# AechPro/rlgym-ppo

Hardware: AMD Instinct MI355X
Metric: ppo_update_samples_per_sec (higher is better)
Workload: dtype f32; 1 GPU; configs[1]: 4096 agents x 128 steps = 524,288-sample buffer, obs 107 f32, 90 discrete actions, 256x3 policy + critic; batch 524,288, minibatch 65,536

## Files before the change

### rlgym_ppo_amd/csrc/api.hip

```cpp
#include "build_id.h"
#include <math.h>
#include <stdarg.h>
#include <string.h>

#include "common.hpp"

namespace rlppo {

static thread_local char g_err[512] = "";

void set_error(const char *fmt, ...) {
    va_list ap;
    va_start(ap, fmt);
    vsnprintf(g_err, sizeof(g_err), fmt, ap);
    va_end(ap);
}

static int64_t padded_width(int64_t d) {
    const int64_t p16 = round_up(d, 16), p64 = round_up(d, 64);
    return (p64 - p16) * 10 >= p64 ? p16 : p64;
}
static int64_t padded_out(int64_t d) {
    if (d <= 32) return 32;
    if (d <= 64) return 64;
    if (d <= 96) return 96;
    return round_up(d, 128);
}

int make_layout(const int32_t *dims, int32_t n_layers, NetLayout *out) {
    RLPPO_CHECK_ARG(dims != nullptr && n_layers >= 1 && n_layers <= RLPPO_MAX_LAYERS, "network: n_layers=%d not in [1,%d]",
                    n_layers, RLPPO_MAX_LAYERS);
    for (int i = 0; i <= n_layers; ++i) RLPPO_CHECK_ARG(dims[i] >= 1, "network: dims[%d]=%d", i, dims[i]);
    out->n_layers = n_layers;
    int64_t off = 0, flat = 0;
    int pin = (int)padded_width(dims[0]);
    for (int l = 0; l < n_layers; ++l) {
        LayerLayout &L = out->L[l];
        L.in = dims[l];
        L.out = dims[l + 1];
        L.pin = pin;
        L.pout = (int)padded_out(dims[l + 1]);
        L.off_w = off;
        off += (int64_t)L.pout * L.pin;
        L.off_wt = off;
        off += (int64_t)L.pin * L.pout;
        L.off_b = off;
        off += L.pout;
        L.off_flat_w = flat;
        flat += (int64_t)L.out * L.in;
        L.off_flat_b = flat;
        flat += L.out;
        pin = L.pout;
    }
    out->packed_floats = off;
    out->flat_floats = flat;
    return 0;
}

static int max_pout(const NetLayout &net) {
    int m = 0;
    for (int l = 0; l < net.n_layers; ++l) m = net.L[l].pout > m ? net.L[l].pout : m;
    return m;
}

struct X3Layout {
    int64_t fwd[RLPPO_MAX_LAYERS], dx[RLPPO_MAX_LAYERS], total;
};
static void x3_layout(const NetLayout &net, X3Layout *o) {
    int64_t off = 0;
    const int last = net.n_layers - 1;
    for (int l = 0; l < net.n_layers; ++l) {
        const LayerLayout &L = net.L[l];
        o->fwd[l] = o->dx[l] = -1;
        if (l >= 1 && l < last && nt_split_ok(L.pout, L.pin)) {
            o->fwd[l] = off;
            off += (int64_t)3 * L.pout * L.pin;
        }
        if (l >= 1 && !(l == last && gemv_head_ok(L.out, L.pin)) && nt_split_ok(L.pin, L.pout)) {
            o->dx[l] = off;
            off += (int64_t)3 * L.pin * L.pout;
        }
    }
    o->total = off;
}

static int g_fold_vhead = 1;

struct RowSource {
    const float *x;
    int64_t ld;
    const unsigned *rowtab = nullptr;
    int64_t src_rows = 0;
};

static int forward(hipStream_t st, const NetLayout &net, const float *packed, const RowSource &in, int64_t n, int out_tanh,
                   float *const *acts, int bf16_operands = 0, unsigned long long *const *bits = nullptr, bool *have_bits = nullptr,
                   bool *head_folded = nullptr, const unsigned short *x3 = nullptr, bool head_prezeroed = false) {
    X3Layout xl;
    if (x3) x3_layout(net, &xl);
    if (have_bits)
        for (int l = 0; l < net.n_layers; ++l) have_bits[l] = false;
    const float *x = in.x;
    int64_t ldx = in.ld;
    const int hl = net.n_layers - 1;
    bool fold = head_folded && g_fold_vhead && hl >= 1 && !out_tanh && !bf16_operands && bits && bits[hl - 1] &&
                gemv_head_ok(net.L[hl].out, net.L[hl].pin) && net.L[hl - 1].pout / 128 <= 2;
    if (x3 && hl >= 1 && xl.fwd[hl - 1] >= 0) fold = false;
    if (head_folded) *head_folded = false;
    for (int l = 0; l < net.n_layers; ++l) {
        const LayerLayout &L = net.L[l];
        const bool last = l == net.n_layers - 1;
        const int epi = last ? (out_tanh ? EPI_BIAS_TANH : EPI_BIAS) : EPI_BIAS_RELU;
        int rc;
        if (last && head_folded && *head_folded) break;
        if (last && !out_tanh && gemv_head_ok(L.out, L.pin))
            rc = launch_gemv_fwd(st, x, ldx, packed + L.off_w, packed + L.off_b, acts[l], L.pout, n, L.pin, L.pout);
        else {
            rc = -1;
            if (!last && bits && bits[l] && x3 && xl.fwd[l] >= 0) {
                rc = launch_gemm_nt_split(st, x, ldx, x3 + xl.fwd[l], packed + L.off_b, acts[l], L.pout, n, L.pout, L.pin, 0, bits[l]);
                if (rc == 0) have_bits[l] = true;
            } else if (!last && bits && bits[l] && !bf16_operands) {
                NtDot dots[2];
                const bool fold_here = fold && l == hl - 1;
                if (fold_here) {
                    if (!head_prezeroed) RLPPO_HIP(hipMemsetAsync(acts[hl], 0, (size_t)n * sizeof(float), st));
                    dots[0].w = packed + net.L[hl].off_w;
                    dots[0].b = packed + net.L[hl].off_b;
                    dots[0].out = acts[hl];
                }
                rc = launch_gemm_nt_bits(st, x, ldx, packed + L.off_w, L.pin, packed + L.off_b, acts[l], L.pout, n, L.pout, L.pin,
                                         EPI_BIAS_RELU, bits[l], l == 0 ? in.rowtab : nullptr, in.src_rows, nullptr, fold_here ? dots : nullptr);
                if (rc == 0) have_bits[l] = true;
                if (fold_here) *head_folded = rc == 0;
            }
            if (l == 0 && in.rowtab && rc != 0) {
                if (rc == -1) set_error("forward: the gathered first layer needs the bitmask form");
                return rc == -1 ? RLPPO_ERR_ARG : rc;
            }
            if (rc == -1)
                rc = launch_gemm_nt(st, x, ldx, packed + L.off_w, L.pin, packed + L.off_b, nullptr, 0, acts[l], L.pout, n, L.pout,
                                    L.pin, epi, bf16_operands);
        }
        if (rc) return rc;
        x = acts[l];
        ldx = L.pout;
    }
    return 0;
}

static bool b16_next_wants_f32(const NetLayout &net, int l) {
    const int nx = l + 1, last = net.n_layers - 1;
    const LayerLayout &N = net.L[nx];
    if (nx == last) {
        const bool fwd_b16 = gemv_head_ok(N.out, N.pin) || nt_b16_ok(N.pout, N.pin, false);
        return !(fwd_b16 && thin_head_ok(N.out, N.pin));
    }
    return !(nt_b16_ok(N.pout, N.pin, true) && tn_b16_ok(N.pout, N.pin));
}
static int forward_b16(hipStream_t st, const NetLayout &net, const float *packed_r, const unsigned short *wb16, const float *x,
                       const unsigned short *xb, int64_t ldx, int64_t n, int out_tanh, float *const *acts,
                       unsigned short *const *actsb, unsigned long long *const *bits, bool *have_bits, bool *f32_valid) {
    for (int l = 0; l < net.n_layers; ++l) have_bits[l] = f32_valid[l] = false;
    int64_t off16 = 0;
    bool x_f32 = true;
    for (int l = 0; l < net.n_layers; ++l) {
        const LayerLayout &L = net.L[l];
        const bool last = l == net.n_layers - 1;
        int rc = 0;
        auto need_x_f32 = [&]() -> int {
            if (x_f32) return 0;
            x_f32 = f32_valid[l - 1] = true;
            return launch_expand_rows(st, actsb[l - 1], acts[l - 1], n * (int64_t)net.L[l - 1].pout);
        };
        if (last) {
            const int epi = out_tanh ? EPI_BIAS_TANH : EPI_BIAS;
            if (!out_tanh && gemv_head_ok(L.out, L.pin))
                rc = launch_gemv_fwd_b16(st, xb, ldx, packed_r + L.off_w, packed_r + L.off_b, acts[l], L.pout, n, L.pin, L.pout);
            else if (nt_b16_ok(L.pout, L.pin, false))
                rc = launch_gemm_nt_b16(st, xb, ldx, wb16 + off16, L.pin, packed_r + L.off_b, acts[l], L.pout, nullptr, 0, n, L.pout,
                                        L.pin, epi, 0, nullptr);
            else {
                rc = need_x_f32();
                if (rc == 0)
                    rc = launch_gemm_nt(st, x, ldx, packed_r + L.off_w, L.pin, packed_r + L.off_b, nullptr, 0, acts[l], L.pout, n,
                                        L.pout, L.pin, epi);
            }
            f32_valid[l] = true;
        } else if (nt_b16_ok(L.pout, L.pin, true) && bits[l]) {
            const bool want = b16_next_wants_f32(net, l);
            rc = launch_gemm_nt_b16(st, xb, ldx, wb16 + off16, L.pin, packed_r + L.off_b, want ? acts[l] : nullptr, L.pout, actsb[l],
                                    L.pout, n, L.pout, L.pin, EPI_BIAS_RELU, 1, bits[l]);
            have_bits[l] = rc == 0;
            f32_valid[l] = want;
        } else {
            rc = need_x_f32();
            if (rc) return rc;
            rc = -1;
            if (bits[l]) {
                rc = launch_gemm_nt_bits(st, x, ldx, packed_r + L.off_w, L.pin, packed_r + L.off_b, acts[l], L.pout, n, L.pout, L.pin,
                                         EPI_BIAS_RELU, bits[l]);
                have_bits[l] = rc == 0;
            }
            if (rc == -1)
                rc = launch_gemm_nt(st, x, ldx, packed_r + L.off_w, L.pin, packed_r + L.off_b, nullptr, 0, acts[l], L.pout, n, L.pout,
                                    L.pin, EPI_BIAS_RELU);
            if (rc == 0) rc = launch_round_rows(st, acts[l], actsb[l], n * (int64_t)L.pout);
            f32_valid[l] = true;
        }
        if (rc) return rc;
        off16 += (int64_t)L.pout * L.pin;
        x = acts[l];
        xb = actsb[l];
        x_f32 = f32_valid[l];
        ldx = L.pout;
    }
    return 0;
}

static size_t forward_ws_floats(const NetLayout &net, int64_t n) { return (size_t)2 * (size_t)n * (size_t)max_pout(net); }

static int forward_pingpong(hipStream_t st, const NetLayout &net, const float *packed, const float *obs, int64_t ld_obs,
                            int64_t n, int out_tanh, void *ws, size_t ws_bytes, float *final_out, const float **out,
                            int64_t *ld_out, int bf16_operands) {
    if (ws_bytes < forward_ws_floats(net, n) * sizeof(float)) {
        set_error("forward: workspace %zu < %zu bytes", ws_bytes, forward_ws_floats(net, n) * sizeof(float));
        return RLPPO_ERR_WORKSPACE;
    }
    RLPPO_CHECK_ARG(ld_obs >= net.L[0].pin && ld_obs % 4 == 0, "forward: ld_obs=%ld must be >= %d (zero padded rows)",
                    (long)ld_obs, net.L[0].pin);
    float *b0 = reinterpret_cast<float *>(ws);
    float *b1 = b0 + (size_t)n * max_pout(net);
    float *acts[RLPPO_MAX_LAYERS];
    for (int l = 0; l < net.n_layers; ++l) acts[l] = (l & 1) ? b1 : b0;
    if (final_out) acts[net.n_layers - 1] = final_out;
    int rc = forward(st, net, packed, RowSource{obs, ld_obs}, n, out_tanh, acts, bf16_operands);
    if (rc) return rc;
    *out = acts[net.n_layers - 1];
    *ld_out = net.L[net.n_layers - 1].pout;
    return 0;
}

}

using namespace rlppo;

static int g_fused_act = 1;
static std::atomic<long long> g_cnt_fused_act{0}, g_cnt_act_chain{0}, g_cnt_paired_pass{0}, g_cnt_gather_fused_pass{0}, g_cnt_pass{0}, g_cnt_group_dw{0}, g_cnt_md_nvec{0};
constexpr int64_t FUSED_ACT_MAX_ROWS = 8192;

struct ActCtx {
    int bf16 = 0;
    unsigned *done = nullptr;
    unsigned done_value = 0;
    unsigned *noise_ctl = nullptr;
    const unsigned *mask = nullptr;
    int mask_words = 0;
};
static int act_ctx(const rlppo_act_opts *o, ActCtx *c, bool late_noise = false, const char *mask_for = nullptr) {
    c->bf16 = get_infer_bf16();
    if (!o) return 0;
    RLPPO_CHECK_ARG(o->precision == RLPPO_PRECISION_DEFAULT || o->precision == RLPPO_PRECISION_FP32 || o->precision == RLPPO_PRECISION_BF16,
                    "act options: inference precision %d (0 = process default, 1 = fp32, 2 = bf16 operands)", o->precision);
    if (o->precision != RLPPO_PRECISION_DEFAULT) c->bf16 = o->precision == RLPPO_PRECISION_BF16;
    c->done = o->done_words;
    c->done_value = o->done_value;
    c->noise_ctl = o->noise_ctl;
    c->mask = o->action_mask;
    c->mask_words = o->mask_words;
    RLPPO_CHECK_ARG(!o->action_mask || !mask_for, "act options: action_mask is an option of the discrete head, not of %s", mask_for ? mask_for : "");
    RLPPO_CHECK_ARG(!o->noise_ctl || late_noise, "act options: noise_ctl is an option of rlppo_discrete_step");
    RLPPO_CHECK_ARG(!o->noise_ctl || (o->done_words && !(o->done_value & 0x80000000u)),
                    "act options: noise_ctl needs done_words (a kernel that gives up on the noise reports it there) and done_value < 2^31");
    return 0;
}
static int act_mask_check(const ActCtx &c, int n_actions) {
    RLPPO_CHECK_ARG(!c.mask || c.mask_words == (n_actions + 31) / 32, "act options: mask_words=%d, but n_actions=%d needs %d words per row",
                    c.mask_words, n_actions, (n_actions + 31) / 32);
    return 0;
}
static int act_done(hipStream_t st, const ActCtx &c, int64_t n) {
    return c.done ? launch_signal_words(st, c.done, (int)rlppo_act_done_words(n), c.done_value) : 0;
}

extern "C" {

int rlppo_abi_version(void) { return RLPPO_ABI_VERSION; }
const char *rlppo_build_id(void) { return RLPPO_BUILD_ID; }
const char *rlppo_last_error(void) { return g_err; }

int64_t rlppo_padded_width(int64_t d) { return padded_width(d); }
int64_t rlppo_padded_out(int64_t d) { return padded_out(d); }

int64_t rlppo_packed_floats(const int32_t *dims, int32_t n_layers) {
    NetLayout net;
    if (make_layout(dims, n_layers, &net)) return -1;
    return net.packed_floats;
}
int64_t rlppo_flat_floats(const int32_t *dims, int32_t n_layers) {
    NetLayout net;
    if (make_layout(dims, n_layers, &net)) return -1;
    return net.flat_floats;
}

int rlppo_net_pack(void *stream, const int32_t *dims, int32_t n_layers, const float *flat, float *packed) {
    NetLayout net;
    int rc = make_layout(dims, n_layers, &net);
    if (rc) return rc;
    RLPPO_CHECK_ARG(flat && packed, "net_pack: null pointer");
    return launch_pack((hipStream_t)stream, net, flat, packed);
}

int rlppo_pad_rows(void *stream, const void *src, int32_t src_is_f64, int64_t n, int64_t d, int64_t ld_src, float *dst,
                   int64_t ld_dst, int32_t standardize, float mean0, float std0) {
    RLPPO_CHECK_ARG(n >= 0 && d >= 1 && ld_src >= d && ld_dst >= d, "pad_rows: n=%ld d=%ld ld_src=%ld ld_dst=%ld", (long)n,
                    (long)d, (long)ld_src, (long)ld_dst);
    RLPPO_CHECK_ARG(n == 0 || (src && dst), "pad_rows: null pointer");
    return launch_pad_rows((hipStream_t)stream, src, src_is_f64, n, d, ld_src, dst, ld_dst, standardize, mean0, std0);
}

int rlppo_pad_rows_per_feature(void *stream, const void *src, int32_t src_is_f64, int64_t n, int64_t d, int64_t ld_src,
                               float *dst, int64_t ld_dst, const float *mean, const float *stdv) {
    RLPPO_CHECK_ARG(n >= 0 && d >= 1 && ld_src >= d && ld_dst >= d, "pad_rows_per_feature: n=%ld d=%ld ld_src=%ld ld_dst=%ld",
                    (long)n, (long)d, (long)ld_src, (long)ld_dst);
    RLPPO_CHECK_ARG(n == 0 || (src && dst && mean && stdv), "pad_rows_per_feature: null pointer");
    return launch_pad_rows_vec((hipStream_t)stream, src, src_is_f64, n, d, ld_src, dst, ld_dst, mean, stdv);
}

size_t rlppo_forward_workspace_bytes(const int32_t *dims, int32_t n_layers, int64_t n) {
    NetLayout net;
    if (make_layout(dims, n_layers, &net)) return 0;
    return forward_ws_floats(net, n > 0 ? n : 0) * sizeof(float) + 256;
}

int rlppo_mlp_forward(void *stream, const int32_t *dims, int32_t n_layers, const float *packed, const float *obs,
                      int64_t ld_obs, int64_t n, int32_t out_tanh, float *out, int64_t ld_out, void *workspace,
                      size_t ws_bytes, const rlppo_act_opts *opts) {
    NetLayout net;
    int rc = make_layout(dims, n_layers, &net);
    if (rc) return rc;
    ActCtx cx;
    rc = act_ctx(opts, &cx, false, "rlppo_mlp_forward");
    if (rc) return rc;
    if (n == 0) return 0;
    RLPPO_CHECK_ARG(n > 0 && packed && obs && out && workspace, "mlp_forward: bad argument");
    RLPPO_CHECK_ARG(ld_out == net.L[n_layers - 1].pout, "mlp_forward: ld_out=%ld must equal the padded output width %d",
                    (long)ld_out, net.L[n_layers - 1].pout);
    const float *o;
    int64_t ldo;
    rc = forward_pingpong((hipStream_t)stream, net, packed, obs, ld_obs, n, out_tanh, workspace, ws_bytes, out, &o, &ldo, cx.bf16);
    return rc ? rc : act_done((hipStream_t)stream, cx, n);
}

int rlppo_discrete_act(void *stream, const int32_t *dims, int32_t n_layers, const float *packed, const float *obs,
                       int64_t ld_obs, int64_t n, const float *noise_q, int64_t *actions, float *logp, float *probs_out,
                       void *workspace, size_t ws_bytes, const rlppo_act_opts *opts) {
    NetLayout net;
    int rc = make_layout(dims, n_layers, &net);
    if (rc) return rc;
    ActCtx cx;
    rc = act_ctx(opts, &cx);
    if (rc) return rc;
    if (n == 0) return 0;
    RLPPO_CHECK_ARG(n > 0 && packed && obs && noise_q && actions && logp && workspace, "discrete_act: bad argument");
    rc = act_mask_check(cx, dims[n_layers]);
    if (rc) return rc;
    if (g_fused_act && !cx.bf16 && fused_act_ok(net) && n <= FUSED_ACT_MAX_ROWS && ld_obs >= net.L[0].pin && ld_obs % 4 == 0 &&
        (reinterpret_cast<uintptr_t>(obs) & 15) == 0) {
        FusedActIO io;
        io.rows = obs;
        io.ld_rows = ld_obs;
        io.noise = noise_q;
        io.actions = actions;
        io.logp = logp;
        io.probs_out = probs_out;
        io.done_words = cx.done;
        io.done_value = cx.done_value;
        io.mask = cx.mask;
        io.mask_words = cx.mask_words;
        ++g_cnt_fused_act;
        return launch_discrete_act_fused((hipStream_t)stream, net, packed, io, n);
    }
    ++g_cnt_act_chain;
    const float *o;
    int64_t ldo;
    rc = forward_pingpong((hipStream_t)stream, net, packed, obs, ld_obs, n, 0, workspace, ws_bytes, nullptr, &o, &ldo, cx.bf16);
    if (rc) return rc;
    rc = launch_discrete_sample_logits((hipStream_t)stream, o, ldo, n, dims[n_layers], noise_q, actions, logp, probs_out, cx.mask, cx.mask_words);
    return rc ? rc : act_done((hipStream_t)stream, cx, n);
}

size_t rlppo_discrete_step_workspace_bytes(const int32_t *dims, int32_t n_layers, int64_t n) {
    NetLayout net;
    if (make_layout(dims, n_layers, &net)) return 0;
    n = n > 0 ? n : 0;
    return forward_ws_floats(net, n) * sizeof(float) + ((size_t)n * net.L[0].pin * sizeof(float) + 255) / 256 * 256 + 512;
}

static int g_window_mode = 0;
int rlppo_host_window_alloc(size_t bytes, void **ptr) {
    RLPPO_CHECK_ARG(ptr && bytes > 0, "host_window_alloc: bad argument");
// ... 384 lines not shown
                    float *const *dx, float *grad, float *tn_ws, unsigned long long *const *bits, const bool *have_bits,
                    bool head_folded = false, const unsigned short *x3 = nullptr, DwList *defer = nullptr) {
    const int last = net.n_layers - 1;
    int rc = 0;
    X3Layout xl;
    if (x3) x3_layout(net, &xl);
    for (int l = last; l >= 0; --l) {
        const LayerLayout &L = net.L[l];
        const float *dY = l == last ? acts[last] : dx[l];
        const int64_t ld_hy = head_folded ? 1 : L.pout;
        const RowSource X = l > 0 ? RowSource{acts[l - 1], net.L[l - 1].pout} : in;
        const bool gemv = l == last && l > 0 && gemv_head_ok(L.out, L.pin);
        const size_t floats = tn_layer_floats(net, l, mb, 0);
        if (gemv)
            rc = launch_gemv_dw(st, dY, ld_hy, X.x, X.ld, grad + L.off_flat_w, grad + L.off_flat_b, L.in, L.pin, mb, tn_ws, floats);
        else if (defer)
            defer->add(L, dY, X, grad);
        else
            rc = launch_gemm_tn(st, dY, L.pout, L.pout, X.x, X.ld, L.pin, grad + L.off_flat_w, grad + L.off_flat_b, L.out, L.in, mb,
                                tn_ws, floats, X.rowtab, X.src_rows);
        if (rc) return rc;
        if (l == 0) break;
        rc = -1;
        if (gemv) {
            if (have_bits[l - 1]) rc = launch_gemv_dx_bits(st, dY, ld_hy, packed + L.off_w, bits[l - 1], dx[l - 1], L.pin, L.pin, mb);
            if (rc == -1) rc = launch_gemv_dx(st, dY, ld_hy, packed + L.off_w, acts[l - 1], L.pin, dx[l - 1], L.pin, L.pin, mb);
        } else {
            if (have_bits[l - 1] && x3 && xl.dx[l] >= 0)
                rc = launch_gemm_nt_split(st, dY, L.pout, x3 + xl.dx[l], nullptr, dx[l - 1], L.pin, mb, L.pin, L.pout, 1, bits[l - 1]);
            else if (have_bits[l - 1])
                rc = launch_gemm_nt_bits(st, dY, L.pout, packed + L.off_wt, L.pout, nullptr, dx[l - 1], L.pin, mb, L.pin, L.pout,
                                         EPI_MASK, bits[l - 1]);
            if (rc == -1)
                rc = launch_gemm_nt(st, dY, L.pout, packed + L.off_wt, L.pout, nullptr, acts[l - 1], L.pin, dx[l - 1], L.pin, mb,
                                    L.pin, L.pout, EPI_MASK);
        }
        if (rc) return rc;
    }
    return rc;
}

static int backward_b16(hipStream_t st, const NetLayout &net, const float *packed_r, const unsigned short *wb16, const float *states,
                        const unsigned short *states_b, int64_t ld_states, int64_t mb, float *const *acts,
                        unsigned short *const *actsb, float *const *dx, unsigned short *const *dxb, float *grad, float *tn_ws,
                        size_t tn_floats, unsigned long long *const *bits, const bool *have_bits, bool *f32_valid) {
    const int last = net.n_layers - 1;
    int64_t first[RLPPO_MAX_LAYERS], total = 0;
    for (int l = 0; l < net.n_layers; ++l) {
        first[l] = total;
        total += (int64_t)net.L[l].pout * net.L[l].pin;
    }
    bool dx_f32[RLPPO_MAX_LAYERS] = {};
    int rc = 0;
    auto act_f32 = [&](int l) -> int {
        if (l < 0 || f32_valid[l]) return 0;
        f32_valid[l] = true;
        return launch_expand_rows(st, actsb[l], acts[l], mb * (int64_t)net.L[l].pout);
    };
    auto grad_f32 = [&](int l) -> int {
        if (dx_f32[l]) return 0;
        dx_f32[l] = true;
        return launch_expand_rows(st, dxb[l], dx[l], mb * (int64_t)net.L[l].pout);
    };
    for (int l = last; l >= 0; --l) {
        const LayerLayout &L = net.L[l];
        const float *X = l > 0 ? acts[l - 1] : states;
        const unsigned short *Xb = l > 0 ? actsb[l - 1] : states_b;
        const int64_t ldx = l > 0 ? net.L[l - 1].pout : ld_states;
        const bool gemv = l == last && l > 0 && gemv_head_ok(L.out, L.pin);
        if (l == last) {
            rc = l > 0 ? launch_thin_dw_b16(st, acts[last], L.pout, Xb, ldx, grad + L.off_flat_w, grad + L.off_flat_b, L.out, L.in,
                                            L.pin, mb, tn_ws, tn_floats)
                       : -1;
            if (rc == -1) {
                rc = act_f32(l - 1);
                if (rc) return rc;
                if (gemv)
                    rc = launch_gemv_dw(st, acts[last], L.pout, X, ldx, grad + L.off_flat_w, grad + L.off_flat_b, L.in, L.pin, mb,
                                        tn_ws, tn_floats);
                else
                    rc = launch_gemm_tn(st, acts[last], L.pout, L.pout, X, ldx, L.pin, grad + L.off_flat_w, grad + L.off_flat_b,
                                        L.out, L.in, mb, tn_ws, tn_floats);
            }
        } else if (tn_b16_ok(L.pout, L.pin) && ldx % 8 == 0) {
            rc = launch_gemm_tn_b16(st, dxb[l], L.pout, Xb, ldx, grad + L.off_flat_w, grad + L.off_flat_b, L.pout, L.pin, L.out, L.in,
                                    mb, tn_ws, tn_floats);
        } else {
            rc = grad_f32(l);
            if (rc == 0) rc = act_f32(l - 1);
            if (rc) return rc;
            rc = launch_gemm_tn(st, dx[l], L.pout, L.pout, X, ldx, L.pin, grad + L.off_flat_w, grad + L.off_flat_b, L.out, L.in, mb,
                                tn_ws, tn_floats);
        }
        if (rc) return rc;
        if (l == 0) break;
        if (l < last && have_bits[l - 1] && nt_b16_ok(L.pin, L.pout, true)) {
            rc = launch_gemm_nt_b16(st, dxb[l], L.pout, wb16 + total + first[l], L.pout, nullptr, nullptr, 0, dxb[l - 1], L.pin, mb,
                                    L.pin, L.pout, EPI_MASK, 2, bits[l - 1]);
            if (rc) return rc;
            continue;
        }
        if (l == last && have_bits[l - 1]) {
            rc = launch_thin_dx_b16(st, acts[last], L.pout, L.out, packed_r + L.off_w, L.pin, bits[l - 1], dxb[l - 1], L.pin, L.pin, mb);
            if (rc == 0) continue;
            if (rc != -1) return rc;
        }
        const float *dY = acts[last];
        if (l < last) {
            rc = grad_f32(l);
            if (rc) return rc;
            dY = dx[l];
        }
        rc = -1;
        if (gemv) {
            if (have_bits[l - 1]) rc = launch_gemv_dx_bits(st, dY, L.pout, packed_r + L.off_w, bits[l - 1], dx[l - 1], L.pin, L.pin, mb);
            if (rc == -1) {
                rc = act_f32(l - 1);
                if (rc) return rc;
                rc = launch_gemv_dx(st, dY, L.pout, packed_r + L.off_w, acts[l - 1], L.pin, dx[l - 1], L.pin, L.pin, mb);
            }
        } else {
            if (have_bits[l - 1])
                rc = launch_gemm_nt_bits(st, dY, L.pout, packed_r + L.off_wt, L.pout, nullptr, dx[l - 1], L.pin, mb, L.pin, L.pout,
                                         EPI_MASK, bits[l - 1]);
            if (rc == -1) {
                rc = act_f32(l - 1);
                if (rc) return rc;
                rc = launch_gemm_nt(st, dY, L.pout, packed_r + L.off_wt, L.pout, nullptr, acts[l - 1], L.pin, dx[l - 1], L.pin, mb,
                                    L.pin, L.pout, EPI_MASK);
            }
        }
        if (rc) return rc;
        rc = launch_round_rows(st, dx[l - 1], dxb[l - 1], mb * (int64_t)L.pin);
        if (rc) return rc;
        dx_f32[l - 1] = true;
    }
    return rc;
}

static int g_head_order = 1;
static int g_paired = 1;
constexpr int64_t PAIRED_MIN_ROWS = 262144;
static bool twin_ok(const NetLayout &p, const NetLayout &v, int64_t mb) {
    if (p.n_layers != v.n_layers || p.n_layers < 2) return false;
    for (int l = 0; l + 1 < p.n_layers; ++l) {
        const LayerLayout &a = p.L[l], &b = v.L[l];
        if (a.in != b.in || a.out != b.out || a.pin != b.pin || a.pout != b.pout) return false;
        if (a.pout % 128 != 0 || a.pin % 16 != 0 || nt_bits_floats(mb, a.pout) == 0) return false;
    }
    return true;
}

static int head_forward(hipStream_t st, const NetLayout &net, const float *packed, const float *x, int64_t ldx, int64_t n, int out_tanh,
                        float *out) {
    const LayerLayout &L = net.L[net.n_layers - 1];
    if (!out_tanh && gemv_head_ok(L.out, L.pin)) return launch_gemv_fwd(st, x, ldx, packed + L.off_w, packed + L.off_b, out, L.pout, n, L.pin, L.pout);
    return launch_gemm_nt(st, x, ldx, packed + L.off_w, L.pin, packed + L.off_b, nullptr, 0, out, L.pout, n, L.pout, L.pin,
                          out_tanh ? EPI_BIAS_TANH : EPI_BIAS);
}
static int head_backward(hipStream_t st, const NetLayout &net, const float *packed, const float *dY, const float *X, int64_t mb,
                         float *dx_prev, float *grad, float *tn_ws, const unsigned long long *bits_prev, int64_t ld_dy = 0,
                         DwList *defer = nullptr) {
    const int last = net.n_layers - 1;
    const LayerLayout &L = net.L[last];
    const int64_t ldx = net.L[last - 1].pout;
    const bool gemv = gemv_head_ok(L.out, L.pin);
    const size_t floats = tn_layer_floats(net, last, mb, 0);
    if (!ld_dy) ld_dy = L.pout;
    int rc = 0;
    if (gemv) rc = launch_gemv_dw(st, dY, ld_dy, X, ldx, grad + L.off_flat_w, grad + L.off_flat_b, L.in, L.pin, mb, tn_ws, floats);
    else if (defer) defer->add(L, dY, RowSource{X, ldx}, grad);
    else rc = launch_gemm_tn(st, dY, L.pout, L.pout, X, ldx, L.pin, grad + L.off_flat_w, grad + L.off_flat_b, L.out, L.in, mb, tn_ws, floats);
    if (rc) return rc;
    if (gemv) return launch_gemv_dx_bits(st, dY, ld_dy, packed + L.off_w, bits_prev, dx_prev, L.pin, L.pin, mb);
    rc = launch_gemm_nt_bits(st, dY, L.pout, packed + L.off_wt, L.pout, nullptr, dx_prev, L.pin, mb, L.pin, L.pout, EPI_MASK,
                             const_cast<unsigned long long *>(bits_prev));
    if (rc == -1) {
        set_error("paired pass: the output layer's dX needs the bitmask form");
        return RLPPO_ERR_ARG;
    }
    return rc;
}

constexpr int64_t FUSED_GATHER_MIN_ROWS = 262144;
static RowSource first_layer_rows(const rlppo_minibatch_args &a, const NetLayout &pol, const NetLayout &val, int prec, const WsPlan &w) {
    const int64_t src_rows = a.ring_cap > 0 ? a.ring_cap : a.n_rows;
    auto gather_form = [&](const NetLayout &n) {
        return n.n_layers > 1 && nt_gather_ok(a.ld_states, src_rows, n.L[0].pout, n.L[0].pin) && tn_gather_ok(a.ld_states, src_rows) &&
               !(n.L[0].out > 64 && n.L[0].out <= 96 && !(n.L[0].in > 96 && n.L[0].in <= 112));
    };
    if (prec != 1 && (g_fused_gather == 2 || (g_fused_gather == 1 && a.mb >= FUSED_GATHER_MIN_ROWS)) && src_rows > 0 &&
        gather_form(pol) && gather_form(val))
        return RowSource{a.states, a.ld_states, w.rowtab, src_rows};
    return RowSource{w.states, pol.L[0].pin};
}

struct Pass {
    const rlppo_minibatch_args *a;
    NetLayout pol, val;
    int64_t mb;
    int prec;
    int64_t ring_base, ring_cap;
    WsPlan w;
    RowSource rows;
    LossCfg cfg;
    MdSpec md;
    bool md_general = false;
    const float *pol_w, *val_w;
    hipStream_t st, side;
    DwList *defer;
};

static LossCfg loss_cfg(const rlppo_minibatch_args &a) {
    LossCfg c;
    c.clip = a.clip_range;
    c.clip_lo = (float)(1.0 - (double)a.clip_range);
    c.clip_hi = (float)(1.0 + (double)a.clip_range);
    c.ent_coef = a.ent_coef;
    c.mb_ratio = a.mb_ratio;
    c.inv_mb = 1.0f / (float)a.mb;
    c.var_m = a.var_m;
    c.var_b = a.var_b;
    c.adv_norm = a.adv_norm;
    c.vclip = a.value_clip;
    c.kl_slots = a.kl_slots;
    c.stop_word = a.stop_word;
    return c;
}

static int policy_loss(hipStream_t st, const Pass &p) {
    const rlppo_minibatch_args &a = *p.a;
    const int last = p.pol.n_layers - 1;
    const LayerLayout &L = p.pol.L[last];
    const WsPlan &w = p.w;
    if (a.head == RLPPO_HEAD_DISCRETE) {
        MaskRows mr;
        mr.mask = a.action_mask;
        mr.W = a.mask_words;
        mr.idx = a.idx;
        mr.ring_base = p.ring_base;
        mr.ring_cap = p.ring_cap;
        return launch_discrete_loss(st, w.pol.act[last], L.pout, L.out, w.g_act, w.g_old, w.g_adv, p.mb, p.cfg, a.stats, a.action_mask ? &mr : nullptr);
    }
    if (a.head == RLPPO_HEAD_GAUSSIAN)
        return launch_gaussian_loss(st, w.pol.act[last], L.pout, L.out / 2, w.g_act, w.g_old, w.g_adv, p.mb, p.cfg, a.stats);
    if (p.md_general) {
        ++g_cnt_md_nvec;
        return launch_multidiscrete_nvec_loss(st, w.pol.act[last], L.pout, w.g_act, w.g_old, w.g_adv, p.mb, p.cfg, a.stats, p.md);
    }
    return launch_multidiscrete_loss(st, w.pol.act[last], L.pout, w.g_act, w.g_old, w.g_adv, p.mb, p.cfg, a.stats);
}

static int gather(const Pass &p) {
    const rlppo_minibatch_args &a = *p.a;
    const WsPlan &w = p.w;
    const int width = p.pol.L[0].pin;
    float *const vout = w.val.act[p.val.n_layers - 1];
    if (p.prec == 1) {
        auto lean0 = [](const NetLayout &n) {
            return n.n_layers > 1 && nt_b16_ok(n.L[0].pout, n.L[0].pin, true) && tn_b16_ok(n.L[0].pout, n.L[0].pin);
        };
        const int rc = launch_gather_rows_round(p.st, a.states, a.ld_states, a.idx, lean0(p.pol) && lean0(p.val) ? nullptr : w.states,
                                                w.states_b, width, p.mb, p.ring_base, p.ring_cap);
        if (rc) return rc;
    } else if (!p.rows.rowtab) {
        GatherMeta gm;
        gm.actions = a.actions; gm.old_logp = a.old_logp; gm.adv = a.advantages; gm.targets = a.targets;
        gm.g_old = w.g_old; gm.g_adv = w.g_adv; gm.g_tgt = w.g_tgt; gm.g_act = w.g_act;
        gm.zero_n = vout;
        gm.act_dim = a.act_dim;
        return launch_gather_rows(p.st, a.states, a.ld_states, a.idx, w.states, width, p.mb, p.ring_base, p.ring_cap, &gm);
    }
    return launch_gather_meta(p.st, a.idx, a.actions, a.act_dim, a.old_logp, a.advantages, a.targets, w.g_act, w.g_old, w.g_adv, w.g_tgt,
                              p.mb, p.ring_base, p.ring_cap, p.rows.rowtab ? w.rowtab : nullptr, vout);
}

static int paired_pass(const Pass &p, SlotBank &bk, int slot) {
    const rlppo_minibatch_args &a = *p.a;
    const NetLayout &pol = p.pol, &val = p.val;
    const WsPlan &w = p.w;
    const int64_t mb = p.mb;
    const hipStream_t st = p.st, hs = p.side;
    const int H = pol.n_layers - 1;
    int rc;
    const LayerLayout &Lvh = val.L[H];
    const bool fold_v = g_fold_vhead && gemv_head_ok(Lvh.out, Lvh.pin) && val.L[H - 1].pout / 128 <= 2;
    float *vout = w.val.act[H], *pout = w.pol.act[H];
    const int64_t ldv = fold_v ? 1 : Lvh.pout;
    const float *xp = p.rows.x, *xv = xp;
    int64_t ldx = p.rows.ld;
    for (int l = 0; l < H; ++l) {
        const LayerLayout &Lp = pol.L[l], &Lv = val.L[l];
        NtAlt alt;
        alt.A = xv;
        alt.B = p.val_w + Lv.off_w;
        alt.bias = p.val_w + Lv.off_b;
        alt.C = w.val.act[l];
        alt.bits = w.val.bits[l];
        NtDot dots[2];
        const bool fold_here = fold_v && l == H - 1;
        if (fold_here) {
            dots[1].w = p.val_w + Lvh.off_w;
            dots[1].out = vout;
            dots[1].b = p.val_w + Lvh.off_b;
        }
        rc = launch_gemm_nt_bits(st, xp, ldx, p.pol_w + Lp.off_w, Lp.pin, p.pol_w + Lp.off_b, w.pol.act[l], Lp.pout, mb, Lp.pout, Lp.pin,
                                 EPI_BIAS_RELU, w.pol.bits[l], l == 0 ? p.rows.rowtab : nullptr, p.rows.src_rows, &alt,
                                 fold_here ? dots : nullptr);
        if (rc) {
            if (rc == -1) set_error("paired pass: a hidden layer does not have the bitmask form");
            return rc == -1 ? RLPPO_ERR_ARG : rc;
        }
        xp = w.pol.act[l];
        xv = w.val.act[l];
        ldx = Lp.pout;
    }
    if (hs != st) {
        rc = order_after(hs, st, bk.ev_fork[slot]);
        if (rc) return rc;
    }
    if (!fold_v) {
        rc = head_forward(hs, val, p.val_w, xv, ldx, mb, 0, vout);
        if (rc) return rc;
    }
    rc = launch_value_loss(hs, vout, ldv, w.g_tgt, w.g_adv, mb, p.cfg, a.stats);
    if (rc) return rc;
    const bool ordered = g_head_order && hs != st;
    if (!ordered) {
        rc = head_backward(hs, val, p.val_w, vout, xv, mb, w.val.dx[H - 1], a.val_grad, w.val.tn, w.val.bits[H - 1], ldv, p.defer);
        if (rc) return rc;
    }
    rc = head_forward(st, pol, p.pol_w, xp, ldx, mb, a.head == RLPPO_HEAD_GAUSSIAN, pout);
    if (rc) return rc;
    rc = policy_loss(st, p);
    if (rc) return rc;
    if (ordered) {
        rc = order_after(hs, st, bk.ev_mid[slot]);
        if (rc) return rc;
        rc = head_backward(hs, val, p.val_w, vout, xv, mb, w.val.dx[H - 1], a.val_grad, w.val.tn, w.val.bits[H - 1], ldv, p.defer);
        if (rc) return rc;
    }
    rc = head_backward(st, pol, p.pol_w, pout, xp, mb, w.pol.dx[H - 1], a.pol_grad, w.pol.tn, w.pol.bits[H - 1], 0, p.defer);
    if (rc) return rc;
    if (hs != st) {
        rc = order_after(st, hs, bk.ev_join[slot]);
        if (rc) return rc;
    }
    for (int l = H - 1; l >= 0; --l) {
        const LayerLayout &Lp = pol.L[l], &Lv = val.L[l];
        const RowSource Xp = l > 0 ? RowSource{w.pol.act[l - 1], pol.L[l - 1].pout} : p.rows;
        const RowSource Xv = l > 0 ? RowSource{w.val.act[l - 1], val.L[l - 1].pout} : p.rows;
        if (p.defer) {
            p.defer->add(Lp, w.pol.dx[l], Xp, a.pol_grad);
            p.defer->add(Lv, w.val.dx[l], Xv, a.val_grad);
        } else {
            TnPair pr;
            pr.dY = w.val.dx[l];
            pr.X = Xv.x;
            pr.dW = a.val_grad + Lv.off_flat_w;
            pr.db = a.val_grad + Lv.off_flat_b;
            pr.ws = w.val.tn;
            rc = launch_gemm_tn(st, w.pol.dx[l], Lp.pout, Lp.pout, Xp.x, Xp.ld, Lp.pin, a.pol_grad + Lp.off_flat_w, a.pol_grad + Lp.off_flat_b,
                                Lp.out, Lp.in, mb, w.pol.tn, tn_layer_floats(pol, l, mb, 0), Xp.rowtab, Xp.src_rows, &pr);
            if (rc) return rc;
        }
        if (l == 0) break;
        NtAlt alt;
        alt.A = w.val.dx[l];
        alt.B = p.val_w + Lv.off_wt;
        alt.C = w.val.dx[l - 1];
        alt.bits = w.val.bits[l - 1];
        rc = launch_gemm_nt_bits(st, w.pol.dx[l], Lp.pout, p.pol_w + Lp.off_wt, Lp.pout, nullptr, w.pol.dx[l - 1], Lp.pin, mb, Lp.pin,
                                 Lp.pout, EPI_MASK, w.pol.bits[l - 1], nullptr, 0, &alt);
        if (rc) return rc == -1 ? RLPPO_ERR_ARG : rc;
    }
    return 0;
}

static int two_chain_pass(const Pass &p) {
    const rlppo_minibatch_args &a = *p.a;
    const NetLayout &pol = p.pol, &val = p.val;
    const WsPlan &w = p.w;
    const int64_t mb = p.mb;
    const bool b16 = p.prec == 1;
    const unsigned short *pol_wb16 = reinterpret_cast<const unsigned short *>(a.pol_wb16);
    const unsigned short *val_wb16 = reinterpret_cast<const unsigned short *>(a.val_wb16);
    const unsigned short *pol_x3 = p.prec == 2 ? pol_wb16 : nullptr, *val_x3 = p.prec == 2 ? val_wb16 : nullptr;
    bool phave[RLPPO_MAX_LAYERS] = {}, vhave[RLPPO_MAX_LAYERS] = {};
    bool pf32[RLPPO_MAX_LAYERS] = {}, vf32[RLPPO_MAX_LAYERS] = {};
    bool v_folded = false;
    int rc;
    if (b16) {
        rc = forward_b16(p.side, val, p.val_w, val_wb16, p.rows.x, w.states_b, p.rows.ld, mb, 0, w.val.act, w.val.actb, w.val.bits, vhave,
                         vf32);
        if (rc) return rc;
        rc = forward_b16(p.st, pol, p.pol_w, pol_wb16, p.rows.x, w.states_b, p.rows.ld, mb, a.head == RLPPO_HEAD_GAUSSIAN, w.pol.act,
                         w.pol.actb, w.pol.bits, phave, pf32);
    } else {
        rc = forward(p.side, val, p.val_w, p.rows, mb, 0, w.val.act, 0, w.val.bits, vhave, &v_folded, val_x3, true);
        if (rc) return rc;
        rc = forward(p.st, pol, p.pol_w, p.rows, mb, a.head == RLPPO_HEAD_GAUSSIAN, w.pol.act, 0, w.pol.bits, phave, nullptr, pol_x3);
    }
    if (rc) return rc;
    const int64_t ldv = v_folded ? 1 : val.L[val.n_layers - 1].pout;
    rc = launch_value_loss(p.side, w.val.act[val.n_layers - 1], ldv, w.g_tgt, w.g_adv, mb, p.cfg, a.stats);
    if (rc) return rc;
    rc = policy_loss(p.st, p);
    if (rc) return rc;
    if (b16) {
        rc = backward_b16(p.side, val, p.val_w, val_wb16, p.rows.x, w.states_b, p.rows.ld, mb, w.val.act, w.val.actb, w.val.dx, w.val.dxb,
                          a.val_grad, w.val.tn, tn_ws_floats(val, mb, p.prec), w.val.bits, vhave, vf32);
        if (rc) return rc;
        return backward_b16(p.st, pol, p.pol_w, pol_wb16, p.rows.x, w.states_b, p.rows.ld, mb, w.pol.act, w.pol.actb, w.pol.dx, w.pol.dxb,
                            a.pol_grad, w.pol.tn, tn_ws_floats(pol, mb, p.prec), w.pol.bits, phave, pf32);
    }
    rc = backward(p.side, val, p.val_w, p.rows, mb, w.val.act, w.val.dx, a.val_grad, w.val.tn, w.val.bits, vhave, v_folded, val_x3, p.defer);
    if (rc) return rc;
    return backward(p.st, pol, p.pol_w, p.rows, mb, w.pol.act, w.pol.dx, a.pol_grad, w.pol.tn, w.pol.bits, phave, false, pol_x3, p.defer);
}

static int ppo_minibatch(void *stream, const rlppo_minibatch_args *a, const int32_t *md_nvec, int32_t md_heads) {
    RLPPO_CHECK_ARG(a != nullptr, "ppo_minibatch: null args");
    Pass p;
    p.a = a;
    int rc = make_layout(a->pol_dims, a->pol_layers, &p.pol);
    if (rc) return rc;
    rc = make_layout(a->val_dims, a->val_layers, &p.val);
    if (rc) return rc;
    const NetLayout &pol = p.pol, &val = p.val;
    const int64_t mb = p.mb = a->mb;
    if (mb == 0) return 0;
    rc = resolve_precision(a->precision, &p.prec);
    if (rc) return rc;
    RLPPO_CHECK_ARG(mb > 0 && a->pol_packed && a->val_packed && a->pol_grad && a->val_grad && a->states && a->actions &&
                        a->old_logp && a->targets && a->advantages && a->idx && a->stats && a->workspace,
                    "ppo_minibatch: null pointer");
    RLPPO_CHECK_ARG(val.L[val.n_layers - 1].out == 1, "ppo_minibatch: critic must have one output");
    RLPPO_CHECK_ARG(a->value_clip >= 0.f && a->value_clip < INFINITY, "ppo_minibatch: value_clip=%g", (double)a->value_clip);
    RLPPO_CHECK_ARG(pol.L[0].in == val.L[0].in, "ppo_minibatch: policy and critic observe different sizes");
    RLPPO_CHECK_ARG(a->ld_states >= pol.L[0].pin && a->ld_states % 4 == 0, "ppo_minibatch: ld_states=%ld < %d",
                    (long)a->ld_states, pol.L[0].pin);
    const size_t ws_bytes = plan_workspace(pol, val, mb, p.prec, a->workspace, &p.w) * sizeof(float);
    if (a->ws_bytes < ws_bytes) {
        set_error("ppo_minibatch: workspace %zu < %zu bytes", a->ws_bytes, ws_bytes);
        return RLPPO_ERR_WORKSPACE;
    }
    const int n_out = pol.L[pol.n_layers - 1].out;
    RLPPO_CHECK_ARG(a->head == RLPPO_HEAD_DISCRETE || a->head == RLPPO_HEAD_GAUSSIAN || a->head == RLPPO_HEAD_MULTIDISCRETE,
                    "ppo_minibatch: unknown head %d", a->head);
    RLPPO_CHECK_ARG(!a->action_mask || a->head == RLPPO_HEAD_DISCRETE, "ppo_minibatch: action_mask is an option of the discrete head, not of the %s head",
                    a->head == RLPPO_HEAD_GAUSSIAN ? "Gaussian" : "multi-discrete");
    RLPPO_CHECK_ARG(!a->action_mask || a->mask_words == (n_out + 31) / 32, "ppo_minibatch: mask_words=%d, but n_actions=%d needs %d words per row",
                    a->mask_words, n_out, (n_out + 31) / 32);
    if (a->head == RLPPO_HEAD_DISCRETE) {
        RLPPO_CHECK_ARG(a->act_dim == 1, "discrete head: act_dim must be 1");
        RLPPO_CHECK_ARG(pol.L[pol.n_layers - 1].pout <= DISCRETE_LOSS_MAX_LD, "discrete head: padded width %ld too large",
                        (long)pol.L[pol.n_layers - 1].pout);
    }
    if (a->head == RLPPO_HEAD_GAUSSIAN)
        RLPPO_CHECK_ARG(n_out % 2 == 0 && a->act_dim == n_out / 2, "gaussian head: act_dim=%d, outputs=%d", a->act_dim, n_out);
    RLPPO_CHECK_ARG(!md_nvec || a->head == RLPPO_HEAD_MULTIDISCRETE, "ppo_minibatch: md_nvec is an option of the multi-discrete head, not of the %s head",
                    a->head == RLPPO_HEAD_GAUSSIAN ? "Gaussian" : "discrete");
    if (a->head == RLPPO_HEAD_MULTIDISCRETE && md_nvec) {
        rc = md_spec_make(md_nvec, md_heads, "multi-discrete head: md_nvec / md_heads", &p.md);
        if (rc) return rc;
        p.md_general = true;
        RLPPO_CHECK_ARG(p.md.S == n_out, "multi-discrete head: md_nvec sums to %d, but the policy has %d outputs", p.md.S, n_out);
        RLPPO_CHECK_ARG(a->act_dim == p.md.H, "multi-discrete head: act_dim=%d, but md_heads=%d", a->act_dim, p.md.H);
    } else if (a->head == RLPPO_HEAD_MULTIDISCRETE)
        RLPPO_CHECK_ARG(n_out == 21 && a->act_dim == 8, "multi-discrete head: needs 21 outputs and act_dim 8");
    RLPPO_CHECK_ARG(p.prec != 1 || (a->pol_packed_r && a->val_packed_r && a->pol_wb16 && a->val_wb16),
                    "ppo_minibatch: the bf16 update precision needs the rlppo_net_pack_bf16 images of both networks (pol_packed_r / val_packed_r / pol_wb16 / val_wb16)");
    RLPPO_CHECK_ARG(p.prec != 2 || (a->pol_wb16 && a->val_wb16),
                    "ppo_minibatch: the split-bf16 update precision needs the rlppo_net_pack_x3 images of both networks (pol_wb16 / val_wb16)");
    p.ring_cap = a->ring_cap > 0 ? a->ring_cap : INT64_MAX;
    p.ring_base = a->ring_cap > 0 ? a->ring_base : 0;
    RLPPO_CHECK_ARG(p.ring_base >= 0 && p.ring_base < p.ring_cap, "ppo_minibatch: ring_base=%ld not in [0, ring_cap=%ld)",
                    (long)a->ring_base, (long)a->ring_cap);
    const int slot = a->slot;
    RLPPO_CHECK_ARG(slot >= 0 && slot < RLPPO_MAX_SLOTS, "ppo_minibatch: slot %d not in [0, %d)", slot, RLPPO_MAX_SLOTS);

    p.rows = first_layer_rows(*a, pol, val, p.prec, p.w);
    const bool twin = p.prec == 0 && (g_paired == 2 || (g_paired == 1 && mb >= PAIRED_MIN_ROWS)) && twin_ok(pol, val, mb);
    p.cfg = loss_cfg(*a);
    p.pol_w = p.prec == 1 ? a->pol_packed_r : a->pol_packed;
    p.val_w = p.prec == 1 ? a->val_packed_r : a->val_packed;
    DwList dws;
    p.defer = (g_group_dw && p.prec != 1) ? &dws : nullptr;

    SlotBank *bank = nullptr;
    rc = slot_bank(&bank);
    if (rc) return rc;
    SlotBank &bk = *bank;
    rc = ensure_slot(bk, slot);
    if (rc) return rc;
    const hipStream_t caller = (hipStream_t)stream;
    p.st = caller;
    if (slot > 0) {
        p.st = bk.main[slot];
        rc = order_after(p.st, caller, bk.ev_slot[slot]);
        if (rc) return rc;
        bk.pending[slot] = true;
    }
    rc = gather(p);
    if (rc) return rc;
    p.side = p.st;
    if (g_two_streams) {
        p.side = bk.side[slot];
        rc = order_after(p.side, p.st, bk.ev_fork[slot]);
        if (rc) return rc;
    }
    ++g_cnt_pass;
    if (twin) ++g_cnt_paired_pass;
    if (p.rows.rowtab) ++g_cnt_gather_fused_pass;
    rc = twin ? paired_pass(p, bk, slot) : two_chain_pass(p);
    if (rc) return rc;
    if (!twin && p.side != p.st) {
        rc = order_after(p.st, p.side, bk.ev_join[slot]);
        if (rc) return rc;
    }
    if (p.defer && dws.n) {
        ++g_cnt_group_dw;
        rc = launch_gemm_tn_group(p.st, dws.p, dws.n, mb, p.w.pol.tn, p.w.tn_floats);
    }
    return rc;
}

int rlppo_ppo_minibatch(void *stream, const rlppo_minibatch_args *a) { return ppo_minibatch(stream, a, nullptr, 0); }
int rlppo_ppo_minibatch_nvec(void *stream, const rlppo_minibatch_args *a, const int32_t *md_nvec, int32_t md_heads) {
    return ppo_minibatch(stream, a, md_nvec, md_heads);
}

int rlppo_ppo_join(void *stream) {
    SlotBank *bank = nullptr;
    int rc = slot_bank(&bank);
    if (rc) return rc;
    SlotBank &bk = *bank;
    for (int s = 1; s < RLPPO_MAX_SLOTS; ++s)
        if (bk.pending[s]) {
            rc = order_after((hipStream_t)stream, bk.main[s], bk.ev_slot[s]);
            if (rc) return rc;
            bk.pending[s] = false;
        }
    return 0;
}

int rlppo_clip_adam(void *stream, float *params, float *grads, float *exp_avg, float *exp_avg_sq, int64_t n,
                    double max_norm, double lr, double beta1, double beta2, double eps, int64_t step, double *gnorm2) {
    if (n == 0) return 0;
    RLPPO_CHECK_ARG(n > 0 && params && grads && exp_avg && exp_avg_sq && gnorm2 && step >= 1, "clip_adam: bad argument");
    const double bc1 = 1.0 - pow(beta1, (double)step);
    const double bc2 = 1.0 - pow(beta2, (double)step);
    const float step_size = (float)(lr / bc1);
    const float bc2_sqrt = (float)sqrt(bc2);
    return launch_clip_adam((hipStream_t)stream, params, grads, exp_avg, exp_avg_sq, n, (float)max_norm, step_size, bc2_sqrt,
                            (float)(1.0 - beta1), (float)beta2, (float)(1.0 - beta2), (float)eps, gnorm2);
}

int rlppo_clip_adam_pack2(void *stream, const rlppo_opt_net *a, const rlppo_opt_net *b, void *sync_ws) {
    RLPPO_CHECK_ARG(a && b, "clip_adam_pack2: null descriptor");
// ... 9 lines not shown
        int rc = make_layout(d[k]->dims, d[k]->n_layers, &nets[k]);
        if (rc) return rc;
        RLPPO_CHECK_ARG(d[k]->params && d[k]->grads && d[k]->exp_avg && d[k]->exp_avg_sq && d[k]->packed && d[k]->gnorm2 &&
                            d[k]->step >= 1, "clip_adam_pack2: bad argument (net %d)", k);
        const double bc1 = 1.0 - pow(d[k]->beta1, (double)d[k]->step);
        const double bc2 = 1.0 - pow(d[k]->beta2, (double)d[k]->step);
        p[k] = d[k]->params; g[k] = d[k]->grads; m[k] = d[k]->exp_avg; v[k] = d[k]->exp_avg_sq; packed[k] = d[k]->packed;
        gn[k] = d[k]->gnorm2;
        const LayerLayout &last = nets[k].L[nets[k].n_layers - 1];
        n[k] = last.off_flat_b + last.out;
        max_norm[k] = (float)d[k]->max_norm; step_size[k] = (float)(d[k]->lr / bc1); bc2_sqrt[k] = (float)sqrt(bc2);
        omb1[k] = (float)(1.0 - d[k]->beta1); beta2[k] = (float)d[k]->beta2; omb2[k] = (float)(1.0 - d[k]->beta2);
        eps[k] = (float)d[k]->eps;
    }
    return launch_clip_adam_pack2((hipStream_t)stream, nets, p, g, m, v, packed, gn, n, max_norm, step_size, bc2_sqrt, omb1, beta2,
                                  omb2, eps, sync_ws, skip);
}

int64_t rlppo_kl_slots_doubles(int64_t mb) { return kl_slots_doubles(mb); }

int rlppo_adv_stats(void *stream, const int64_t *idx, int64_t n, const float *advantages, int64_t ring_base, int64_t ring_cap,
                    float *out, void *ws) {
    RLPPO_CHECK_ARG(n >= 1 && idx && advantages && out && ws, "adv_stats: bad argument");
    const int64_t cap = ring_cap > 0 ? ring_cap : INT64_MAX, base = ring_cap > 0 ? ring_base : 0;
    RLPPO_CHECK_ARG(base >= 0 && base < cap, "adv_stats: ring_base=%ld not in [0, ring_cap=%ld)", (long)ring_base, (long)ring_cap);
    return launch_adv_stats((hipStream_t)stream, idx, n, advantages, base, cap, out, ws);
}

int rlppo_kl_gate(void *stream, const rlppo_kl_gate_args *a) {
    RLPPO_CHECK_ARG(a && a->kl_slots && a->n_passes >= 0 && a->slot_stride >= 3 && a->phase >= 0 && a->phase <= 2 && a->stop_word,
                    "kl_gate: bad argument");
    RLPPO_CHECK_ARG(a->phase == 0 || a->exchange, "kl_gate: phases 1 and 2 need the exchange words");
    RLPPO_CHECK_ARG(a->phase == 1 || a->host_words, "kl_gate: host_words missing");
    return launch_kl_gate((hipStream_t)stream, *a);
}

int rlppo_learn_report(void *stream, const rlppo_report_args *a) {
    RLPPO_CHECK_ARG(a != nullptr, "learn_report: null args");
    RLPPO_CHECK_ARG(a->n_pol >= 0 && a->n_val >= 0 && (a->n_pol == 0 || (a->pol_before && a->pol_now)) && (a->n_val == 0 || (a->val_before && a->val_now)),
                    "learn_report: parameter vectors missing");
    RLPPO_CHECK_ARG(a->stats && a->out && a->done_word && a->ws, "learn_report: null pointer (stats / out / done_word / ws)");
    RLPPO_CHECK_ARG((reinterpret_cast<uintptr_t>(a->ws) & 15) == 0, "learn_report: ws must be 16-byte aligned");
    return launch_learn_report((hipStream_t)stream, *a);
}

}

extern "C" {
int rlppo_gather_rows(void *stream, const float *src, int64_t ld_src, const int64_t *idx, float *dst, int32_t width, int64_t n) {
    if (n == 0) return 0;
    RLPPO_CHECK_ARG(n > 0 && src && idx && dst, "gather_rows: null pointer");
    return launch_gather_rows((hipStream_t)stream, src, ld_src, idx, dst, width, n);
}
int rlppo_welford_increment(void *stream, const float *samples, int64_t ld, int64_t n, int32_t d, void *mean, void *m2,
                            int64_t count, int32_t state_is_f64) {
    if (n == 0) return 0;
    RLPPO_CHECK_ARG(n > 0 && d > 0 && ld >= d && count >= 0 && samples && mean && m2, "welford_increment: bad argument");
    return launch_welford((hipStream_t)stream, samples, ld, n, d, mean, m2, (long long)count, state_is_f64 != 0);
}
int rlppo_welford_merge(void *stream, int32_t d, void *mean, void *m2, int64_t count, const float *other_mean,
                        const float *other_m2, int64_t other_count, int32_t state_is_f64) {
    if (other_count == 0) return 0;
    RLPPO_CHECK_ARG(d > 0 && count >= 0 && other_count > 0 && mean && m2 && other_mean && other_m2, "welford_merge: bad argument");
    return launch_welford_merge((hipStream_t)stream, d, mean, m2, (long long)count, other_mean, other_m2, (long long)other_count,
                                state_is_f64 != 0);
}
int64_t rlppo_wb16_elems(const int32_t *dims, int32_t n_layers) {
    NetLayout net;
    if (make_layout(dims, n_layers, &net)) return -1;
    int64_t n = 0;
    for (int l = 0; l < net.n_layers; ++l) n += (int64_t)net.L[l].pout * net.L[l].pin;
    return 2 * n;
}
int rlppo_net_pack_bf16(void *stream, const int32_t *dims, int32_t n_layers, const float *flat, float *packed_r, void *wb16) {
    NetLayout net;
    int rc = make_layout(dims, n_layers, &net);
    if (rc) return rc;
    RLPPO_CHECK_ARG(flat && packed_r && wb16, "net_pack_bf16: null pointer");
    return launch_pack_bf16((hipStream_t)stream, net, flat, packed_r, reinterpret_cast<unsigned short *>(wb16));
}
int64_t rlppo_x3_elems(const int32_t *dims, int32_t n_layers) {
    NetLayout net;
    if (make_layout(dims, n_layers, &net)) return -1;
    X3Layout xl;
    x3_layout(net, &xl);
    return xl.total;
}
int rlppo_net_pack_x3(void *stream, const int32_t *dims, int32_t n_layers, const float *packed, void *planes) {
    NetLayout net;
    int rc = make_layout(dims, n_layers, &net);
    if (rc) return rc;
    X3Layout xl;
    x3_layout(net, &xl);
    if (xl.total == 0) return 0;
    RLPPO_CHECK_ARG(packed && planes, "net_pack_x3: null pointer");
    unsigned short *pl = reinterpret_cast<unsigned short *>(planes);
    for (int l = 0; l < net.n_layers; ++l) {
        const LayerLayout &L = net.L[l];
        if (xl.fwd[l] >= 0) {
            rc = launch_pack_split((hipStream_t)stream, packed + L.off_w, L.pin, L.pout, L.pin, pl + xl.fwd[l]);
            if (rc) return rc;
        }
        if (xl.dx[l] >= 0) {
            rc = launch_pack_split((hipStream_t)stream, packed + L.off_wt, L.pout, L.pin, L.pout, pl + xl.dx[l]);
            if (rc) return rc;
        }
    }
    return 0;
}
int rlppo_dbg_pack_x3(void *stream, const float *S, int64_t ld, int32_t R, int32_t C, void *planes) {
    return launch_pack_split((hipStream_t)stream, S, ld, R, C, reinterpret_cast<unsigned short *>(planes));
}
int rlppo_dbg_gemm_nt_x3(void *stream, const float *A, int64_t lda, const void *planes, const float *bias, float *C, int64_t ldc, int64_t M,
                         int32_t N, int32_t K, int32_t mode, void *bits) {
    return launch_gemm_nt_split((hipStream_t)stream, A, lda, reinterpret_cast<const unsigned short *>(planes), bias, C, ldc, M, N, K, mode,
                                reinterpret_cast<unsigned long long *>(bits));
}
static int64_t g_selection_epoch = 0;
int rlppo_set_update_precision(int32_t mode) {
    RLPPO_CHECK_ARG(mode >= 0 && mode <= 2, "set_update_precision: mode %d (0 = fp32, 1 = bf16 mixed precision, 2 = split-bf16 products)", mode);
    g_update_bf16 = mode;
    ++g_selection_epoch;
    return 0;
}
int rlppo_get_update_precision(void) { return g_update_bf16; }
int rlppo_set_inference_precision(int32_t mode) {
    RLPPO_CHECK_ARG(mode == 0 || mode == 1, "set_inference_precision: mode %d (0 = fp32, 1 = bf16 operands)", mode);
    set_infer_bf16(mode);
    ++g_selection_epoch;
    return 0;
}
int rlppo_dbg_set(int32_t key, int32_t value) {
    ++g_selection_epoch;
    switch (key) {
        case 1: set_gae_algo(value); return 0;
        case 4: g_two_streams = value; return 0;
        case 21: set_gae_spin_limit(value); return 0;
        case 22: set_gae_oversubscribe(value); return 0;
        case 34: set_fused_spin_limit(value); return 0;
        case 35: set_fused_test_hold(value); return 0;
        case 36: set_split_persistent(value); return 0;
        case 23: set_b16_wide_tiles(value); return 0;
        case 24: set_exp_fast_transform(value); return 0;
        case 26: g_fused_gather = value; return 0;
        case 27: g_fused_act = value; return 0;
        case 29: g_paired = value; return 0;
        case 31: g_head_order = value; return 0;
        case 32: g_fold_vhead = value; return 0;
        case 33: set_pair_interleave(value); return 0;
        case 37: g_group_dw = value; return 0;
        case 38: set_tn_group_budget(value); return 0;
        case 40: set_nt_skinny(value); return 0;
        case 41: g_window_mode = value; return 0;
        default: break;
    }
    set_error("dbg_set: unknown key %d", key);
    return RLPPO_ERR_ARG;
}
int64_t rlppo_selection_epoch(void) { return g_selection_epoch; }
const int64_t *rlppo_selection_epoch_ptr(void) { return &g_selection_epoch; }
int64_t rlppo_dbg_counter(int32_t key) {
    switch (key) {
        case 0: return g_cnt_fused_act;
        case 1: return g_cnt_act_chain;
        case 2: return g_cnt_pass;
        case 3: return g_cnt_paired_pass;
        case 4: return g_cnt_gather_fused_pass;
        case 5: return g_cnt_group_dw;
        case 6: return g_cnt_md_nvec;
        default: return -1;
    }
}
size_t rlppo_dbg_gemm_nt_bits_bytes(int64_t M, int32_t N) { return nt_bits_floats(M, N) * sizeof(float); }
int rlppo_dbg_gemm_nt_bits(void *stream, const float *A, int64_t lda, const float *B, int64_t ldb, const float *bias, float *C,
                           int64_t ldc, int64_t M, int32_t N, int32_t K, int32_t epilogue, void *bits) {
    const int rc = launch_gemm_nt_bits((hipStream_t)stream, A, lda, B, ldb, bias, C, ldc, M, N, K, epilogue,
                                       reinterpret_cast<unsigned long long *>(bits));
    if (rc == -1) {
        set_error("dbg_gemm_nt_bits: the bitmask form does not apply to this call");
        return RLPPO_ERR_ARG;
    }
    return rc;
}
int rlppo_dbg_gemm_nt(void *stream, const float *A, int64_t lda, const float *B, int64_t ldb, const float *bias,
                      const float *mask_src, int64_t ld_mask, float *C, int64_t ldc, int64_t M, int32_t N, int32_t K,
                      int32_t epilogue) {
    return launch_gemm_nt((hipStream_t)stream, A, lda, B, ldb, bias, mask_src, ld_mask, C, ldc, M, N, K, epilogue);
}
int rlppo_dbg_gemm_nt_b16(void *stream, const void *A, int64_t lda, const void *W, int64_t ldw, const float *bias, float *C,
                          int64_t ldc, void *Cb, int64_t ldcb, int64_t M, int32_t N, int32_t K, int32_t epilogue, int32_t hidden,
                          void *bits) {
    return launch_gemm_nt_b16((hipStream_t)stream, reinterpret_cast<const unsigned short *>(A), lda,
                              reinterpret_cast<const unsigned short *>(W), ldw, bias, C, ldc, reinterpret_cast<unsigned short *>(Cb),
                              ldcb, M, N, K, epilogue, hidden, reinterpret_cast<unsigned long long *>(bits));
}
int rlppo_dbg_gemm_tn_b16(void *stream, const void *dY, int64_t ldy, const void *X, int64_t ldx, float *dW, float *db, int32_t pout,
                          int32_t pin, int32_t out, int32_t in, int64_t M, void *ws, size_t ws_bytes) {
    return launch_gemm_tn_b16((hipStream_t)stream, reinterpret_cast<const unsigned short *>(dY), ldy,
                              reinterpret_cast<const unsigned short *>(X), ldx, dW, db, pout, pin, out, in, M, (float *)ws,
                              ws_bytes / sizeof(float));
}
size_t rlppo_dbg_thin_head_workspace_bytes(int32_t out, int32_t kp, int64_t M) { return thin_dw_ws_floats(out, kp, M) * sizeof(float); }
int rlppo_dbg_thin_head_b16(void *stream, const float *dY, int64_t ldy, int32_t out, const float *W, int64_t ldw, const void *bits,
                            const void *hb, int64_t ldh, void *dxb, float *dW, float *db, int32_t in, int32_t kp, int64_t M, void *ws,
                            size_t ws_bytes) {
    int rc = launch_thin_dx_b16((hipStream_t)stream, dY, ldy, out, W, ldw, reinterpret_cast<const unsigned long long *>(bits),
                                reinterpret_cast<unsigned short *>(dxb), kp, kp, M);
    if (rc) return rc == -1 ? RLPPO_ERR_ARG : rc;
    rc = launch_thin_dw_b16((hipStream_t)stream, dY, ldy, reinterpret_cast<const unsigned short *>(hb), ldh, dW, db, out, in, kp, M,
                            (float *)ws, ws_bytes / sizeof(float));
    return rc == -1 ? RLPPO_ERR_ARG : rc;
}
static int tn_products(const rlppo_tn_product *p, int32_t n, TnProduct *q) {
    RLPPO_CHECK_ARG(p && n > 0 && n <= 2 * RLPPO_MAX_LAYERS, "gemm_tn_group: %d products (1..%d)", n, 2 * RLPPO_MAX_LAYERS);
    for (int i = 0; i < n; ++i) {
        q[i].dY = p[i].dY; q[i].ldy = p[i].ldy; q[i].ny_valid = p[i].ny_valid; q[i].X = p[i].X; q[i].ldx = p[i].ldx;
        q[i].kx_valid = p[i].kx_valid; q[i].dW = p[i].dW; q[i].db = p[i].db; q[i].out = p[i].out; q[i].in = p[i].in;
        q[i].rowtab = p[i].rowtab; q[i].src_rows = p[i].src_rows;
    }
    return 0;
}
size_t rlppo_dbg_gemm_tn_group_workspace_bytes(const rlppo_tn_product *p, int32_t n, int64_t M) {
    if (!p || n <= 0 || n > 2 * RLPPO_MAX_LAYERS) return 0;
    int outs[2 * RLPPO_MAX_LAYERS], ins[2 * RLPPO_MAX_LAYERS];
    for (int i = 0; i < n; ++i) {
        outs[i] = p[i].out;
        ins[i] = p[i].in;
    }
    return tn_group_floats(outs, ins, n, M) * sizeof(float);
}
int rlppo_dbg_gemm_tn_group(void *stream, const rlppo_tn_product *p, int32_t n, int64_t M, void *ws, size_t ws_bytes) {
    TnProduct q[2 * RLPPO_MAX_LAYERS];
    const int rc = tn_products(p, n, q);
    if (rc) return rc;
    return launch_gemm_tn_group((hipStream_t)stream, q, n, M, (float *)ws, ws_bytes / sizeof(float));
}
size_t rlppo_dbg_gemm_tn_workspace_bytes(int32_t out, int32_t in, int64_t M) { return tn_partial_floats(out, in, M) * sizeof(float); }
int rlppo_dbg_gemm_tn(void *stream, const float *dY, int64_t ldy, int32_t ny_valid, const float *X, int64_t ldx,
                      int32_t kx_valid, float *dW, float *db, int32_t out, int32_t in, int64_t M, void *ws, size_t ws_bytes) {
    return launch_gemm_tn((hipStream_t)stream, dY, ldy, ny_valid, X, ldx, kx_valid, dW, db, out, in, M, (float *)ws,
                          ws_bytes / sizeof(float));
}
}
```

### rlgym_ppo_amd/csrc/common.hpp

```cpp
#pragma once
#include <hip/hip_runtime.h>
#include <stdint.h>
#include <stdio.h>

#include <atomic>

#include "../../include/rlppo.h"

namespace rlppo {

void set_error(const char *fmt, ...);

#define RLPPO_CHECK_ARG(cond, ...)                \
    do {                                          \
        if (!(cond)) {                            \
            rlppo::set_error(__VA_ARGS__);        \
            return RLPPO_ERR_ARG;                 \
        }                                         \
    } while (0)

#define RLPPO_HIP(expr)                                                                         \
    do {                                                                                        \
        hipError_t e_ = (expr);                                                                 \
        if (e_ != hipSuccess) {                                                                 \
            rlppo::set_error("%s failed: %s (%s:%d)", #expr, hipGetErrorString(e_), __FILE__, __LINE__); \
            return (int)e_;                                                                     \
        }                                                                                       \
    } while (0)

#define RLPPO_LAUNCH_CHECK() RLPPO_HIP(hipGetLastError())

struct PerDeviceOnce {
    std::atomic<unsigned long long> done{0};
};
inline int set_dynamic_lds_once(const void *fn, int bytes, PerDeviceOnce &once) {
    int dev = 0;
    RLPPO_HIP(hipGetDevice(&dev));
    const unsigned long long bit = 1ull << (dev & 63);
    if (!(once.done.load(std::memory_order_acquire) & bit)) {
        RLPPO_HIP(hipFuncSetAttribute(fn, hipFuncAttributeMaxDynamicSharedMemorySize, bytes));
        once.done.fetch_or(bit, std::memory_order_release);
    }
    return 0;
}
inline int device_cu_count(int *cus) {
    static std::atomic<int> by_dev[64];
    int dev = 0;
    RLPPO_HIP(hipGetDevice(&dev));
    int n = by_dev[dev & 63].load(std::memory_order_relaxed);
    if (n == 0) {
        RLPPO_HIP(hipDeviceGetAttribute(&n, hipDeviceAttributeMultiprocessorCount, dev));
        by_dev[dev & 63].store(n, std::memory_order_relaxed);
    }
    *cus = n;
    return 0;
}
#undef hipLaunchKernelGGL
#define hipLaunchKernelGGL(kernel, grid, block, shmem, stream, ...)        \
    do {                                                                   \
        (void)hipGetLastError();                                           \
        kernel<<<(grid), (block), (shmem), (stream)>>>(__VA_ARGS__);       \
    } while (0)

static inline int64_t round_up(int64_t x, int64_t m) { return (x + m - 1) / m * m; }
static inline int64_t cdiv(int64_t a, int64_t b) { return (a + b - 1) / b; }

struct LayerLayout {
    int in, out;
    int pin, pout;
    int64_t off_w, off_wt, off_b;
    int64_t off_flat_w, off_flat_b;
};

struct NetLayout {
    int n_layers;
    LayerLayout L[RLPPO_MAX_LAYERS];
    int64_t packed_floats;
    int64_t flat_floats;
};

int make_layout(const int32_t *dims, int32_t n_layers, NetLayout *out);

enum Epilogue { EPI_BIAS = 0, EPI_BIAS_RELU = 1, EPI_BIAS_TANH = 2, EPI_MASK = 3 };

int launch_gemm_nt(hipStream_t st, const float *A, int64_t lda, const float *B, int64_t ldb, const float *bias,
                   const float *mask_src, int64_t ld_mask, float *C, int64_t ldc, int64_t M, int N, int K, int epi,
                   int bf16_operands = 0);
size_t nt_bits_floats(int64_t M, int N);
struct NtAlt {
    const float *A = nullptr, *B = nullptr, *bias = nullptr;
    float *C = nullptr;
    unsigned long long *bits = nullptr;
    int interleave = 0;
};
struct NtDot {
    const float *w = nullptr, *b = nullptr;
    float *out = nullptr;
};
struct TnPair {
    const float *dY = nullptr, *X = nullptr;
    float *dW = nullptr, *db = nullptr, *ws = nullptr;
};
int launch_gemm_nt_bits(hipStream_t st, const float *A, int64_t lda, const float *B, int64_t ldb, const float *bias, float *C,
                        int64_t ldc, int64_t M, int N, int K, int epi, unsigned long long *bits, const unsigned *rowtab = nullptr,
                        int64_t src_rows = 0, const NtAlt *alt = nullptr, const NtDot *dot = nullptr );
bool nt_gather_ok(int64_t lda, int64_t src_rows, int N, int K);
int launch_gemm_nt_bf16(hipStream_t st, const float *A, int64_t lda, const float *B, int64_t ldb, const float *bias, float *C,
                        int64_t ldc, int64_t M, int N, int nb, int K, int epi);
void set_infer_bf16(int v);
void set_pair_interleave(int v);
void set_nt_skinny(int on);
int get_infer_bf16();
size_t tn_partial_floats(int out, int in, int64_t M);
int launch_gemm_tn(hipStream_t st, const float *dY, int64_t ldy, int ny_valid, const float *X, int64_t ldx, int kx_valid,
                   float *dW, float *db, int out, int in, int64_t M, float *ws, size_t ws_floats, const unsigned *rowtab = nullptr,
                   int64_t src_rows = 0, const TnPair *pair = nullptr);
bool tn_gather_ok(int64_t ldx, int64_t src_rows);
struct TnProduct {
    const float *dY = nullptr;
    int64_t ldy = 0;
    int ny_valid = 0;
    const float *X = nullptr;
    int64_t ldx = 0;
    int kx_valid = 0;
    float *dW = nullptr, *db = nullptr;
    int out = 0, in = 0;
    const unsigned *rowtab = nullptr;
    int64_t src_rows = 0;
};
constexpr int TN_GROUP_MAX = 2 * RLPPO_MAX_LAYERS;
size_t tn_group_floats(const int *outs, const int *ins, int n, int64_t M);
int launch_gemm_tn_group(hipStream_t st, const TnProduct *prods, int n, int64_t M, float *ws, size_t ws_floats);
void set_tn_group_budget(int workgroups);

bool nt_b16_ok(int N, int K, bool hidden);
bool nt_split_ok(int N, int K);
void set_split_persistent(int v);
int launch_pack_split(hipStream_t st, const float *S, int64_t ld, int R, int Cc, unsigned short *planes);
int launch_gemm_nt_split(hipStream_t st, const float *A, int64_t lda, const unsigned short *planes, const float *bias, float *C, int64_t ldc,
                         int64_t M, int N, int K, int mode, unsigned long long *bits);
int launch_gemm_nt_b16(hipStream_t st, const unsigned short *A, int64_t lda, const unsigned short *B, int64_t ldb, const float *bias,
                       float *C, int64_t ldc, unsigned short *Cb, int64_t ldcb, int64_t M, int N, int K, int epi, int mode,
                       unsigned long long *bits);
void set_b16_wide_tiles(int on);
bool tn_b16_ok(int pout, int pin);
int launch_gemm_tn_b16(hipStream_t st, const unsigned short *dY, int64_t ldy, const unsigned short *X, int64_t ldx, float *dW,
                       float *db, int pout, int pin, int out, int in, int64_t M, float *ws, size_t ws_floats);

void set_exp_fast_transform(int on);

bool gemv_head_ok(int out, int kp);
int launch_gemv_fwd(hipStream_t st, const float *x, int64_t ldx, const float *w, const float *b, float *y, int64_t ldy, int64_t n, int kp, int pout);
int launch_gemv_fwd_b16(hipStream_t st, const unsigned short *x, int64_t ldx, const float *w, const float *b, float *y, int64_t ldy,
                        int64_t n, int kp, int pout);
bool thin_head_ok(int out, int kp);
size_t thin_dw_ws_floats(int out, int kp, int64_t n);
int launch_thin_dx_b16(hipStream_t st, const float *dy, int64_t ldy, int out, const float *w, int64_t ldw,
                       const unsigned long long *bits, unsigned short *dxb, int64_t ldc, int kp, int64_t n);
int launch_thin_dw_b16(hipStream_t st, const float *dy, int64_t ldy, const unsigned short *xb, int64_t ldx, float *dw, float *db,
                       int out, int in, int kp, int64_t n, float *ws, size_t ws_floats);
int launch_gemv_dx(hipStream_t st, const float *dy, int64_t ldy, const float *w, const float *mask, int64_t ldm, float *dx, int64_t ldc, int kp, int64_t n);
int launch_gemv_dx_bits(hipStream_t st, const float *dy, int64_t ldy, const float *w, const unsigned long long *bits, float *dx,
                        int64_t ldc, int kp, int64_t n);
int launch_gemv_dw(hipStream_t st, const float *dy, int64_t ldy, const float *x, int64_t ldx, float *dw, float *db, int in, int kp, int64_t n,
                   float *ws = nullptr, size_t ws_floats = 0);

struct LossCfg {
    float clip, clip_lo, clip_hi, ent_coef, mb_ratio, inv_mb;
    float var_m, var_b;
    const float *adv_norm = nullptr;
    float vclip = 0.f;
    double *kl_slots = nullptr;
    const unsigned *stop_word = nullptr;
};
__host__ __device__ __forceinline__ int64_t ring_row(int64_t i, int64_t base, int64_t cap) {
    const int64_t r = i + base;
    return r >= cap ? r - cap : r;
}
int launch_discrete_sample_logits(hipStream_t, const float *, int64_t, int64_t, int, const float *, int64_t *, float *, float *,
                                  const unsigned *mask = nullptr, int mask_words = 0);
int launch_discrete_probs(hipStream_t st, const float *logits, int64_t ld, int64_t n, int A, int clamp, float *probs,
                          int64_t ld_p, int64_t *flat_argmax, const unsigned *mask = nullptr, int mask_words = 0);
struct MaskRows {
    const unsigned *mask = nullptr;
    int W = 0;
    const int64_t *idx = nullptr;
    int64_t ring_base = 0, ring_cap = INT64_MAX;
};
int launch_categorical_select(hipStream_t, const float *, int64_t, int64_t, int, const float *, int64_t *, float *);
int launch_gaussian_sample(hipStream_t, const float *, int64_t, int64_t, int, const float *, float, float, float *, float *,
                           unsigned *done_words = nullptr, unsigned done_value = 0);
int launch_multidiscrete_sample(hipStream_t, const float *, int64_t, int64_t, const float *, int64_t *, float *,
                                unsigned *done_words = nullptr, unsigned done_value = 0);
int launch_value_loss(hipStream_t st, float *vout, int64_t ldv, const float *targets, const float *adv, int64_t mb, const LossCfg &cfg,
                      double *stats);
int64_t kl_slots_doubles(int64_t mb);
constexpr int64_t DISCRETE_LOSS_MAX_LD = 64 * 32;
int launch_discrete_loss(hipStream_t, float *, int64_t, int, const float *, const float *, const float *, int64_t, const LossCfg &, double *,
                         const MaskRows *mask_rows = nullptr);
int launch_gaussian_loss(hipStream_t, float *, int64_t, int, const float *, const float *, const float *, int64_t, const LossCfg &, double *);
int launch_multidiscrete_loss(hipStream_t, float *, int64_t, const float *, const float *, const float *, int64_t, const LossCfg &, double *);
struct MdSpec {
    int H, B, S;
    unsigned char b[RLPPO_MD_MAX_HEADS];
};
int md_spec_make(const int32_t *nvec, int n_heads, const char *who, MdSpec *spec);
int launch_multidiscrete_nvec_sample(hipStream_t, const float *, int64_t, int64_t, const float *, int64_t *, float *, const MdSpec &,
                                     unsigned *done_words = nullptr, unsigned done_value = 0);
int launch_multidiscrete_nvec_loss(hipStream_t, float *, int64_t, const float *, const float *, const float *, int64_t, const LossCfg &, double *,
                                   const MdSpec &);

struct FusedActIO {
    const float *rows = nullptr;
    int64_t ld_rows = 0;
    const void *raw = nullptr;
    int raw_is_f64 = 0, standardize = 0;
    int64_t ld_raw = 0;
    float mean0 = 0.f, std0 = 1.f;
    const float *mean_v = nullptr, *std_v = nullptr;
    float *rows_out = nullptr;
    int64_t ld_rows_out = 0;
    const float *noise = nullptr;
    int64_t *actions = nullptr;
    float *actions_f32 = nullptr;
    float *logp = nullptr, *probs_out = nullptr;
    unsigned *done_words = nullptr;
    unsigned done_value = 0;
    unsigned *noise_ctl = nullptr;
    const unsigned *mask = nullptr;
    int mask_words = 0;
};
bool fused_act_ok(const NetLayout &net);
}
void host_window_register(void *base, size_t bytes, unsigned *hdp_flush);
void host_window_unregister(void *base);
namespace rlppo {
int launch_discrete_act_fused(hipStream_t st, const NetLayout &net, const float *packed, const FusedActIO &io, int64_t n);

size_t gae_workspace_bytes(int64_t n);
void set_gae_algo(int algo);
void set_gae_spin_limit(int v);
void set_gae_oversubscribe(int v);
void set_fused_spin_limit(int v);
void set_fused_test_hold(int v);
int launch_gae(hipStream_t, const float *, const float *, const float *, const float *, const float *, int64_t, double, double, float,
               float *, float *, float *, void *, size_t);

int launch_pack(hipStream_t, const NetLayout &, const float *, float *);
int launch_pack_bf16(hipStream_t st, const NetLayout &net, const float *flat, float *packed_r, unsigned short *wb16);
int launch_round_rows(hipStream_t st, float *x, unsigned short *xb, int64_t n_elems);
int launch_expand_rows(hipStream_t st, const unsigned short *xb, float *x, int64_t n_elems);
int launch_gather_rows_round(hipStream_t st, const float *src, int64_t ld_src, const int64_t *idx, float *dst, unsigned short *dstb,
                             int width, int64_t n, int64_t ring_base, int64_t ring_cap);
int launch_clip_adam(hipStream_t, float *p, float *g, float *m, float *v, int64_t n, float max_norm, float step_size,
                     float bc2_sqrt, float one_minus_beta1, float beta2, float one_minus_beta2, float eps, double *gnorm2);
int launch_clip_adam_pack2(hipStream_t st, const NetLayout *nets, float *const *p, float *const *g, float *const *m, float *const *v,
                           float *const *packed, double *const *gnorm2, const int64_t *n, const float *max_norm,
                           const float *step_size, const float *bc2_sqrt, const float *omb1, const float *beta2, const float *omb2,
                           const float *eps, void *sync_ws = nullptr, const unsigned *const *skip = nullptr);
int launch_adv_stats(hipStream_t st, const int64_t *idx, int64_t n, const float *adv, int64_t ring_base, int64_t ring_cap, float *out,
                     void *ws);
int launch_kl_gate(hipStream_t st, const rlppo_kl_gate_args &a);
int launch_welford(hipStream_t st, const float *x, int64_t ld, int64_t n, int d, void *mean, void *m2, long long count0, int state_f64);
int launch_welford_merge(hipStream_t st, int d, void *mean, void *m2, long long count, const float *omean, const float *om2,
                         long long ocount, int state_f64);
struct GatherMeta {
    const float *actions = nullptr, *old_logp = nullptr, *adv = nullptr, *targets = nullptr;
    float *g_act = nullptr, *g_old = nullptr, *g_adv = nullptr, *g_tgt = nullptr, *zero_n = nullptr;
    int act_dim = 0;
};
int launch_gather_rows(hipStream_t st, const float *src, int64_t ld_src, const int64_t *idx, float *dst, int width, int64_t n,
                       int64_t ring_base = 0, int64_t ring_cap = INT64_MAX, const GatherMeta *meta = nullptr);
int launch_gather_meta(hipStream_t st, const int64_t *idx, const float *actions, int act_dim, const float *old_logp,
                       const float *adv, const float *targets, float *g_act, float *g_old, float *g_adv, float *g_tgt, int64_t n,
                       int64_t ring_base, int64_t ring_cap, unsigned *rowtab = nullptr, float *zero_n = nullptr);
int launch_i64_to_f32(hipStream_t st, const int64_t *src, float *dst, int64_t n);
int launch_learn_report(hipStream_t st, const rlppo_report_args &r);
int launch_signal_words(hipStream_t st, unsigned *words, int count, unsigned value);
int launch_pad_rows(hipStream_t, const void *, int, int64_t, int64_t, int64_t, float *, int64_t, int, float, float);
int launch_pad_rows_vec(hipStream_t, const void *, int, int64_t, int64_t, int64_t, float *, int64_t, const float *, const float *);

}
```

### rlgym_ppo_amd/csrc/gemm.hip

```cpp
#include "gemm_detail.hpp"

namespace rlppo {

template <int NB, int EPI, int BKT, bool BITS = false, bool GATHER = false>
__global__ __launch_bounds__(256, BKT == 16 ? 4 : 2) void gemm_nt_dma_kernel(const float *__restrict__ A, unsigned lda_b,
                                                                              const float *__restrict__ B, unsigned ldb_b,
                                                                              const float *__restrict__ bias,
                                                                              const float *__restrict__ mask_src,
                                                                              unsigned ldm_b, float *__restrict__ C,
                                                                              unsigned ldc_b, int64_t M, int K,
                                                                              unsigned long long *__restrict__ bits = nullptr,
                                                                              const unsigned *__restrict__ rowtab = nullptr,
                                                                              unsigned src_rows = 0, NtAlt alt = NtAlt{},
                                                                              NtDot dot = NtDot{}, NtDot dot_alt = NtDot{}) {
    constexpr int BN = NB * 16;
    constexpr int CPR = BKT / 4;
    constexpr int RPW = 64 / CPR;
    constexpr int RPP = 4 * RPW;
    constexpr int A_IT = SBM / RPP, B_IT = BN / RPP;
    constexpr int B_REM = BN % RPP;
    static_assert(B_REM % RPW == 0, "the ragged staging pass must be whole wave instructions");
    __shared__ __attribute__((aligned(16))) float lds[2 * SBM * BKT + 2 * BN * BKT];
    float *As = lds;
    float *Bs = lds + 2 * SBM * BKT;

    const int tid = threadIdx.x;
    const int lane = tid & 63, wave = tid >> 6;
    const int wave_u = __builtin_amdgcn_readfirstlane(wave);
    const int r16 = lane & 15, q = lane >> 4;
    int row_tile, col_tile;
    xcd_tile(row_tile, col_tile);
    int nct = gridDim.y;
    bool second = blockIdx.z != 0;
    if (alt.interleave) {
        nct >>= 1;
        second = col_tile >= nct;
        if (second) col_tile -= nct;
    }
    if (second) {
        A = alt.A;
        B = alt.B;
        bias = alt.bias;
        C = alt.C;
        bits = alt.bits;
        dot = dot_alt;
    }
    const int64_t m0 = (int64_t)row_tile * SBM;
    const int n0 = col_tile * BN;
    const int rows_here = (int)((M - m0) < SBM ? (M - m0) : SBM);
    unsigned long long *const bit_word = BITS ? bits + ((size_t)row_tile * nct + col_tile) * 256 + tid : nullptr;
    unsigned long long mask_word = 0;
    if (BITS && EPI == EPI_MASK) mask_word = *bit_word;

    const __amdgpu_buffer_rsrc_t a_rs = GATHER ? __builtin_amdgcn_make_buffer_rsrc(const_cast<float *>(A), (short)lda_b, src_rows, 0x00020000)
                                               : make_rsrc(reinterpret_cast<const char *>(A) + m0 * lda_b,
                                                           (unsigned)(rows_here - 1) * lda_b + (unsigned)K * 4);
    const __amdgpu_buffer_rsrc_t b_rs = make_rsrc(reinterpret_cast<const char *>(B) + (int64_t)n0 * ldb_b,
                                                  (unsigned)(BN - 1) * ldb_b + (unsigned)K * 4);
    const int row_p = wave * RPW + lane / CPR, pch = lane % CPR;
    const int lch = BKT == 32 ? (pch ^ (row_p & 7)) : (pch ^ ((0 - (row_p >> 2)) & 3));
    const unsigned a_off = GATHER ? (unsigned)lch * 16 : (unsigned)row_p * lda_b + lch * 16;
    const unsigned b_off = (unsigned)row_p * ldb_b + lch * 16;
    const unsigned a_step = (unsigned)RPP * lda_b, b_step = (unsigned)RPP * ldb_b;
    unsigned a_row[4];
    static_assert(A_IT <= 4, "a_row");
    if (GATHER) {
        const __amdgpu_buffer_rsrc_t t_rs = make_rsrc(rowtab + m0, (unsigned)rows_here * 4);
#pragma unroll
        for (int i = 0; i < A_IT; ++i) a_row[i] = __builtin_amdgcn_raw_buffer_load_b32(t_rs, (unsigned)(row_p + i * RPP) * 4, 0, 0);
    }

    f32x4 acc[2][NB];
    if (EPI == EPI_MASK) {
#pragma unroll
        for (int i = 0; i < 2; ++i)
#pragma unroll
            for (int j = 0; j < NB; ++j) acc[i][j] = f32x4{0.f, 0.f, 0.f, 0.f};
    } else {
        const __amdgpu_buffer_rsrc_t bias_rs = make_rsrc(bias + n0, BN * 4);
#pragma unroll
        for (int j = 0; j < NB; ++j) {
            acc[0][j] = ldb(bias_rs, (unsigned)(q * 16), j * 64);
            acc[1][j] = acc[0][j];
        }
    }

    auto issue_tile = [&](int buf, unsigned kb) {
        float *Ad = As + buf * SBM * BKT + wave_u * RPW * BKT;
        float *Bd = Bs + buf * BN * BKT + wave_u * RPW * BKT;
#pragma unroll
        for (int i = 0; i < A_IT; ++i) {
            if (GATHER)
                __builtin_amdgcn_struct_ptr_buffer_load_lds(a_rs, Ad + i * RPP * BKT, 16, a_row[i], a_off, kb, 0, 0);
            else
                __builtin_amdgcn_raw_ptr_buffer_load_lds(a_rs, Ad + i * RPP * BKT, 16, a_off, kb + i * a_step, 0, 0);
        }
#pragma unroll
        for (int i = 0; i < B_IT; ++i)
            __builtin_amdgcn_raw_ptr_buffer_load_lds(b_rs, Bd + i * RPP * BKT, 16, b_off, kb + i * b_step, 0, 0);
        if (B_REM != 0 && wave_u * RPW < B_REM)
            __builtin_amdgcn_raw_ptr_buffer_load_lds(b_rs, Bd + B_IT * RPP * BKT, 16, b_off, kb + B_IT * b_step, 0, 0);
    };

    const int nk = K / BKT;
    if (GATHER) asm volatile("s_waitcnt vmcnt(0)" ::: "memory");
    issue_tile(0, 0);
    asm volatile("s_waitcnt vmcnt(0)" ::: "memory");
    __syncthreads();
    for (int kt = 0; kt < nk; ++kt) {
        const int cur = kt & 1;
        if ((kt + 1) < nk) issue_tile(cur ^ 1, (unsigned)(kt + 1) * (BKT * 4));
        const float *Ac = As + cur * SBM * BKT + (wave * 32) * BKT;
        const float *Bc = Bs + cur * BN * BKT;
#pragma unroll
        for (int kc = 0; kc < BKT / 16; ++kc) {
            f32x4 fa[2], fb[NB];
#pragma unroll
            for (int i = 0; i < 2; ++i) fa[i] = *reinterpret_cast<const f32x4 *>(&Ac[dswz<BKT>(i * 16 + r16, kc * 4 + q)]);
#pragma unroll
            for (int j = 0; j < NB; ++j) fb[j] = *reinterpret_cast<const f32x4 *>(&Bc[dswz<BKT>(j * 16 + r16, kc * 4 + q)]);
#pragma unroll
            for (int s = 0; s < 4; ++s)
#pragma unroll
                for (int i = 0; i < 2; ++i)
#pragma unroll
                    for (int j = 0; j < NB; ++j) acc[i][j] = MFMA16(fb[j][s], fa[i][s], acc[i][j]);
        }
        __builtin_amdgcn_sched_barrier(0);
        asm volatile("s_waitcnt vmcnt(0)" ::: "memory");
        __syncthreads();
    }
    char *const park = reinterpret_cast<char *>(lds) + wave_u * 8192;
    if (BITS && EPI == EPI_MASK) {
        apply_bits<NB>(acc, mask_word);
        nt_epilogue<NB, EPI_NONE>(acc, nullptr, 0, C, ldc_b, m0, n0, rows_here, wave, r16, q, park);
    } else if (BITS && EPI == EPI_BIAS_RELU) {
#pragma unroll
        for (int i = 0; i < 2; ++i)
#pragma unroll
            for (int j = 0; j < NB; ++j)
#pragma unroll
                for (int e = 0; e < 4; ++e) acc[i][j][e] = relu1(acc[i][j][e]);
        *bit_word = relu_bits<NB>(acc);
        if (dot.w) {
            const __amdgpu_buffer_rsrc_t w_rs = make_rsrc(dot.w + n0, BN * 4);
            float s0 = 0.f, s1 = 0.f;
#pragma unroll
            for (int j = 0; j < NB; ++j) {
                const f32x4 wv = ldb(w_rs, (unsigned)(q * 16), j * 64);
#pragma unroll
                for (int e = 0; e < 4; ++e) {
                    s0 += acc[0][j][e] * wv[e];
                    s1 += acc[1][j][e] * wv[e];
                }
            }
            s0 += __shfl_xor(s0, 16);
            s1 += __shfl_xor(s1, 16);
            s0 += __shfl_xor(s0, 32);
            s1 += __shfl_xor(s1, 32);
            if (q == 0) {
                const float b0 = col_tile == 0 ? dot.b[0] : 0.f;
                const int r0 = wave * 32 + r16;
                if (r0 < rows_here) atomicAdd(dot.out + m0 + r0, s0 + b0);
                if (r0 + 16 < rows_here) atomicAdd(dot.out + m0 + r0 + 16, s1 + b0);
            }
        }
        nt_epilogue<NB, EPI_NONE>(acc, nullptr, 0, C, ldc_b, m0, n0, rows_here, wave, r16, q, park);
    } else {
        nt_epilogue<NB, EPI>(acc, mask_src, ldm_b, C, ldc_b, m0, n0, rows_here, wave, r16, q, park);
    }
}

__device__ __forceinline__ bf16x8 to_bf16x8(const float *lo, const float *hi) {
    const f32x4 a = *reinterpret_cast<const f32x4 *>(lo), b = *reinterpret_cast<const f32x4 *>(hi);
    bf16x8 r;
#pragma unroll
    for (int e = 0; e < 4; ++e) {
        r[e] = (__bf16)a[e];
        r[4 + e] = (__bf16)b[e];
    }
    return r;
}

template <int NB, int EPI>
__global__ __launch_bounds__(256, 2) void gemm_nt_bf16_kernel(const float *__restrict__ A, unsigned lda_b,
                                                                              const float *__restrict__ B, unsigned ldb_b,
                                                                              const float *__restrict__ bias,
                                                                              const float *__restrict__ mask_src,
                                                                              unsigned ldm_b, float *__restrict__ C,
                                                                              unsigned ldc_b, int64_t M, int K) {
    constexpr int BN = NB * 16;
    constexpr int BKT = 32;
    constexpr int CPR = BKT / 4;
    constexpr int RPW = 64 / CPR;
    constexpr int RPP = 4 * RPW;
    constexpr int A_IT = SBM / RPP, B_IT = BN / RPP;
    static_assert(BN % RPP == 0, "column tile must be a whole number of staging passes");
    __shared__ __attribute__((aligned(16))) float lds[2 * SBM * BKT + 2 * BN * BKT];
    float *As = lds;
    float *Bs = lds + 2 * SBM * BKT;

    const int tid = threadIdx.x;
    const int lane = tid & 63, wave = tid >> 6;
    const int wave_u = __builtin_amdgcn_readfirstlane(wave);
    const int r16 = lane & 15, q = lane >> 4;
    int row_tile, col_tile;
    xcd_tile(row_tile, col_tile);
    const int64_t m0 = (int64_t)row_tile * SBM;
    const int n0 = col_tile * BN;
    const int rows_here = (int)((M - m0) < SBM ? (M - m0) : SBM);

    const __amdgpu_buffer_rsrc_t a_rs = make_rsrc(reinterpret_cast<const char *>(A) + m0 * lda_b,
                                                  (unsigned)(rows_here - 1) * lda_b + (unsigned)K * 4);
    const __amdgpu_buffer_rsrc_t b_rs = make_rsrc(reinterpret_cast<const char *>(B) + (int64_t)n0 * ldb_b,
                                                  (unsigned)(BN - 1) * ldb_b + (unsigned)K * 4);
    const int row_p = wave * RPW + lane / CPR, pch = lane % CPR;
    const int lch = BKT == 32 ? (pch ^ (row_p & 7)) : (pch ^ ((0 - (row_p >> 2)) & 3));
    const unsigned a_off = (unsigned)row_p * lda_b + lch * 16;
    const unsigned b_off = (unsigned)row_p * ldb_b + lch * 16;
    const unsigned a_step = (unsigned)RPP * lda_b, b_step = (unsigned)RPP * ldb_b;

    f32x4 acc[2][NB];
    if (EPI == EPI_MASK) {
#pragma unroll
        for (int i = 0; i < 2; ++i)
#pragma unroll
            for (int j = 0; j < NB; ++j) acc[i][j] = f32x4{0.f, 0.f, 0.f, 0.f};
    } else {
        const __amdgpu_buffer_rsrc_t bias_rs = make_rsrc(bias + n0, BN * 4);
#pragma unroll
        for (int j = 0; j < NB; ++j) {
            acc[0][j] = ldb(bias_rs, (unsigned)(q * 16), j * 64);
            acc[1][j] = acc[0][j];
        }
    }

    auto issue_tile = [&](int buf, unsigned kb) {
        float *Ad = As + buf * SBM * BKT + wave_u * RPW * BKT;
        float *Bd = Bs + buf * BN * BKT + wave_u * RPW * BKT;
#pragma unroll
        for (int i = 0; i < A_IT; ++i)
            __builtin_amdgcn_raw_ptr_buffer_load_lds(a_rs, Ad + i * RPP * BKT, 16, a_off, kb + i * a_step, 0, 0);
#pragma unroll
        for (int i = 0; i < B_IT; ++i)
            __builtin_amdgcn_raw_ptr_buffer_load_lds(b_rs, Bd + i * RPP * BKT, 16, b_off, kb + i * b_step, 0, 0);
    };

    const int nk = K / BKT;
    issue_tile(0, 0);
    asm volatile("s_waitcnt vmcnt(0)" ::: "memory");
    __syncthreads();
    for (int kt = 0; kt < nk; ++kt) {
        const int cur = kt & 1;
        if ((kt + 1) < nk) issue_tile(cur ^ 1, (unsigned)(kt + 1) * (BKT * 4));
        const float *Ac = As + cur * SBM * BKT + (wave * 32) * BKT;
        const float *Bc = Bs + cur * BN * BKT;
        bf16x8 fa[2], fb[NB];
#pragma unroll
        for (int i = 0; i < 2; ++i) fa[i] = to_bf16x8(&Ac[dswz<32>(i * 16 + r16, 2 * q)], &Ac[dswz<32>(i * 16 + r16, 2 * q + 1)]);
#pragma unroll
        for (int j = 0; j < NB; ++j) fb[j] = to_bf16x8(&Bc[dswz<32>(j * 16 + r16, 2 * q)], &Bc[dswz<32>(j * 16 + r16, 2 * q + 1)]);
#pragma unroll
        for (int i = 0; i < 2; ++i)
#pragma unroll
            for (int j = 0; j < NB; ++j) acc[i][j] = __builtin_amdgcn_mfma_f32_16x16x32_bf16(fb[j], fa[i], acc[i][j], 0, 0, 0);
        __builtin_amdgcn_sched_barrier(0);
        asm volatile("s_waitcnt vmcnt(0)" ::: "memory");
        __syncthreads();
    }
    nt_epilogue<NB, EPI>(acc, mask_src, ldm_b, C, ldc_b, m0, n0, rows_here, wave, r16, q);
}

template <int NB>
static int launch_nt_1(hipStream_t st, dim3 grid, int epi, const float *A, unsigned lda_b, const float *B, unsigned ldb_b,
                       const float *bias, const float *mask_src, unsigned ldm_b, float *C, unsigned ldc_b, int64_t M,
                       int K) {
    constexpr int BKT = (NB * 16) % 32 == 0 && NB * 16 >= 64 ? 16 : 32;
    if (BKT == 32 && K % 32 != 0) {
        if (epi == EPI_BIAS_RELU || epi == EPI_BIAS || epi == EPI_BIAS_TANH || epi == EPI_MASK) {
#define NT16(E)                                                                                                         \
    case E:                                                                                                            \
        hipLaunchKernelGGL((gemm_nt_dma_kernel<NB, E, 16>), grid, dim3(256), 0, st, A, lda_b, B, ldb_b, bias, mask_src,  \
                           ldm_b, C, ldc_b, M, K);                                                                     \
        break;
            switch (epi) { NT16(EPI_BIAS) NT16(EPI_BIAS_RELU) NT16(EPI_BIAS_TANH) NT16(EPI_MASK) }
// ... 50 lines not shown
    };
    fetch(0, 0);
    for (int kt0 = 0; kt0 < nk; kt0 += 2 * SK_AHEAD) {
        fetch(1, kt0 + SK_AHEAD);
#pragma unroll
        for (int i = 0; i < SK_AHEAD; ++i)
            if (kt0 + i < nk) {
#pragma unroll
                for (int s = 0; s < 4; ++s) acc = MFMA16(fb[0][i][s], fa[0][i][s], acc);
            }
        fetch(0, kt0 + 2 * SK_AHEAD);
#pragma unroll
        for (int i = 0; i < SK_AHEAD; ++i)
            if (kt0 + SK_AHEAD + i < nk) {
#pragma unroll
                for (int s = 0; s < 4; ++s) acc = MFMA16(fb[1][i][s], fa[1][i][s], acc);
            }
    }
#pragma unroll
    for (int e = 0; e < 4; ++e) {
        if (EPI == EPI_BIAS_RELU) acc[e] = relu1(acc[e]);
        if (EPI == EPI_BIAS_TANH) acc[e] = tanhf(acc[e]);
    }
    if (m0 + r16 < M) *reinterpret_cast<f32x4 *>(C + (m0 + r16) * ldc + n0 + q * 4) = acc;
}

static int launch_gemm_nt_skinny(hipStream_t st, const float *A, int64_t lda, const float *B, int64_t ldb, const float *bias, float *C,
                                 int64_t ldc, int64_t M, int N, int K, int epi) {
    dim3 grid((unsigned)cdiv(N, 64), (unsigned)cdiv(M, 16));
#define SK(E)                                                                                                              \
    case E:                                                                                                                \
        hipLaunchKernelGGL((gemm_nt_skinny_kernel<E>), grid, dim3(256), 0, st, A, lda, B, ldb, bias, C, ldc, M, N, K);      \
        break;
    switch (epi) {
        SK(EPI_BIAS) SK(EPI_BIAS_RELU) SK(EPI_BIAS_TANH)
        default:
            set_error("gemm_nt (few rows): bad epilogue %d", epi);
            return RLPPO_ERR_ARG;
    }
#undef SK
    RLPPO_LAUNCH_CHECK();
    return 0;
}

static int g_infer_bf16 = 0;
void set_infer_bf16(int v) { g_infer_bf16 = v; }
int get_infer_bf16() { return g_infer_bf16; }

template <int NB>
static int launch_bf16_1(hipStream_t st, dim3 grid, int epi, const float *A, unsigned lda_b, const float *B, unsigned ldb_b,
                         const float *bias, float *C, unsigned ldc_b, int64_t M, int K) {
#define BF(E)                                                                                                          \
    case E:                                                                                                            \
        hipLaunchKernelGGL((gemm_nt_bf16_kernel<NB, E>), grid, dim3(256), 0, st, A, lda_b, B, ldb_b, bias, nullptr, 0u, C, \
                           ldc_b, M, K);                                                                               \
        break;
    switch (epi) {
        BF(EPI_BIAS) BF(EPI_BIAS_RELU) BF(EPI_BIAS_TANH)
        default:
            set_error("gemm_nt (bf16 operands): epilogue %d is not a forward epilogue", epi);
            return RLPPO_ERR_ARG;
    }
#undef BF
    RLPPO_LAUNCH_CHECK();
    return 0;
}

int launch_gemm_nt_bf16(hipStream_t st, const float *A, int64_t lda, const float *B, int64_t ldb, const float *bias, float *C,
                        int64_t ldc, int64_t M, int N, int nb, int K, int epi) {
    dim3 grid((unsigned)cdiv(M, SBM), (unsigned)(N / (nb * 16)));
    const unsigned la = (unsigned)(lda * 4), lb = (unsigned)(ldb * 4), lc = (unsigned)(ldc * 4);
    switch (nb) {
        case 8: return launch_bf16_1<8>(st, grid, epi, A, la, B, lb, bias, C, lc, M, K);
        case 6: return launch_bf16_1<6>(st, grid, epi, A, la, B, lb, bias, C, lc, M, K);
        case 4: return launch_bf16_1<4>(st, grid, epi, A, la, B, lb, bias, C, lc, M, K);
        default: return launch_bf16_1<2>(st, grid, epi, A, la, B, lb, bias, C, lc, M, K);
    }
}

size_t nt_bits_floats(int64_t M, int N) {
    if (N % 128 != 0 || M <= 0) return 0;
    return (size_t)cdiv(M, SBM) * (size_t)(N / 128) * 256 * 2;
}
static int g_pair_interleave = 1;
void set_pair_interleave(int v) { g_pair_interleave = v; }
bool nt_gather_ok(int64_t lda, int64_t src_rows, int N, int K) {
    return N % 128 == 0 && K % 16 == 0 && lda * 4 < 16384 && lda % 4 == 0 && src_rows > 0 && src_rows < ((int64_t)1 << 32);
}
int launch_gemm_nt_bits(hipStream_t st, const float *A, int64_t lda, const float *B, int64_t ldb, const float *bias, float *C,
                        int64_t ldc, int64_t M, int N, int K, int epi, unsigned long long *bits, const unsigned *rowtab,
                        int64_t src_rows, const NtAlt *alt, const NtDot *dot) {
    if (!bits || N % 128 != 0 || K % 16 != 0 || M <= 0) return -1;
    if (epi != EPI_BIAS_RELU && epi != EPI_MASK) return -1;
    const int64_t lim = (int64_t)1 << 31;
    if ((!rowtab && 129 * lda * 4 >= lim) || 129 * ldb * 4 >= lim || 129 * ldc * 4 >= lim) return -1;
    RLPPO_CHECK_ARG(!alt || (alt->A && alt->B && alt->C && alt->bits), "gemm_nt: incomplete second operand set");
    dim3 grid((unsigned)cdiv(M, SBM), (unsigned)(N / 128), alt ? 2u : 1u);
    NtAlt second = alt ? *alt : NtAlt{};
    if (alt && g_pair_interleave) {
        grid.y *= 2;
        grid.z = 1;
        second.interleave = 1;
    }
    const NtDot d0 = dot ? dot[0] : NtDot{}, d1 = dot && alt ? dot[1] : NtDot{};
    RLPPO_CHECK_ARG(!dot || (epi == EPI_BIAS_RELU && N / 128 <= 2 && (!d0.w || (d0.out && d0.b)) && (!d1.w || (d1.out && d1.b))),
                    "gemm_nt: the folded one-output head needs the ReLU forward form and at most two column tiles");
    const unsigned la = (unsigned)(lda * 4), lb = (unsigned)(ldb * 4), lc = (unsigned)(ldc * 4);
    if (rowtab) {
        RLPPO_CHECK_ARG(epi == EPI_BIAS_RELU && nt_gather_ok(lda, src_rows, N, K), "gemm_nt (gathered rows): unsupported shape");
        hipLaunchKernelGGL((gemm_nt_dma_kernel<8, EPI_BIAS_RELU, 16, true, true>), grid, dim3(256), 0, st, A, la, B, lb, bias, nullptr,
                           0u, C, lc, M, K, bits, rowtab, (unsigned)src_rows, second, d0, d1);
    } else if (epi == EPI_BIAS_RELU)
        hipLaunchKernelGGL((gemm_nt_dma_kernel<8, EPI_BIAS_RELU, 16, true>), grid, dim3(256), 0, st, A, la, B, lb, bias, nullptr,
                           0u, C, lc, M, K, bits, nullptr, 0u, second, d0, d1);
    else
        hipLaunchKernelGGL((gemm_nt_dma_kernel<8, EPI_MASK, 16, true>), grid, dim3(256), 0, st, A, la, B, lb, nullptr, nullptr, 0u,
                           C, lc, M, K, bits, nullptr, 0u, second);
    RLPPO_LAUNCH_CHECK();
    return 0;
}

int launch_gemm_nt(hipStream_t st, const float *A, int64_t lda, const float *B, int64_t ldb, const float *bias,
                   const float *mask_src, int64_t ld_mask, float *C, int64_t ldc, int64_t M, int N, int K, int epi,
                   int bf16_operands) {
    if (M <= 0) return 0;
    RLPPO_CHECK_ARG(K > 0 && K % 16 == 0, "gemm_nt: K=%d must be a positive multiple of 16", K);
    RLPPO_CHECK_ARG(lda % 4 == 0 && ldb % 4 == 0 && ldc % 4 == 0 && lda >= K && ldb >= K && ldc >= N,
                    "gemm_nt: leading dimensions lda=%ld ldb=%ld ldc=%ld incompatible with K=%d N=%d", (long)lda,
                    (long)ldb, (long)ldc, K, N);
    RLPPO_CHECK_ARG(epi != EPI_MASK || (mask_src && ld_mask >= N && ld_mask % 4 == 0), "gemm_nt: mask operand missing");
    RLPPO_CHECK_ARG(epi == EPI_MASK || bias, "gemm_nt: bias operand missing");
    int nb;
    if (N % 128 == 0) nb = 8;
    else if (N == 96) nb = 6;
    else if (N == 64) nb = 4;
    else if (N == 32) nb = 2;
    else {
        set_error("gemm_nt: N=%d is not a padded output width", N);
        return RLPPO_ERR_ARG;
    }
    const int64_t lim = (int64_t)1 << 31;
    RLPPO_CHECK_ARG(129 * lda * 4 < lim && 129 * ldb * 4 < lim && 129 * ldc * 4 < lim && 129 * ld_mask * 4 < lim,
                    "gemm_nt: a leading dimension is too wide for 32-bit tile offsets");
    if (bf16_operands && epi != EPI_MASK && K % 32 == 0) return launch_gemm_nt_bf16(st, A, lda, B, ldb, bias, C, ldc, M, N, nb, K, epi);
    if (g_nt_skinny && M <= SK_MAX_ROWS && epi != EPI_MASK && !bf16_operands) return launch_gemm_nt_skinny(st, A, lda, B, ldb, bias, C, ldc, M, N, K, epi);
    dim3 grid((unsigned)cdiv(M, SBM), (unsigned)(N / (nb * 16)));
    const unsigned la = (unsigned)(lda * 4), lb = (unsigned)(ldb * 4), lc = (unsigned)(ldc * 4), lm = (unsigned)(ld_mask * 4);
    switch (nb) {
        case 8: return launch_nt_1<8>(st, grid, epi, A, la, B, lb, bias, mask_src, lm, C, lc, M, K);
        case 6: return launch_nt_1<6>(st, grid, epi, A, la, B, lb, bias, mask_src, lm, C, lc, M, K);
        case 4: return launch_nt_1<4>(st, grid, epi, A, la, B, lb, bias, mask_src, lm, C, lc, M, K);
        default: return launch_nt_1<2>(st, grid, epi, A, la, B, lb, bias, mask_src, lm, C, lc, M, K);
    }
}

namespace {
constexpr int TM = 32;
constexpr unsigned OOR = 0x80000000u;
}

struct TnGeom {
    int ni, nj, wn;
    __host__ __device__ int bnt() const { return wn * ni * 16; }
    __host__ __device__ int bkx() const { return (4 / wn) * nj * 16; }
    __host__ __device__ int tile_floats() const { return ni * nj * 1024; }
};
static TnGeom tn_geometry(int out, int in) {
    if (in > 96 && in <= 112) return TnGeom{2, 7, 4};
    if (out > 64 && out <= 96) return TnGeom{3, 4, 2};
    return TnGeom{4, 4, 2};
}

constexpr int TN_LDS_FLOATS = 2 * 2 * 32 * 128;
template <int TMT, int NI, int NJ, int WN, bool GATHER>
__device__ __forceinline__ void tn_tile(float *lds, const float *__restrict__ dY, unsigned ldy_b, int ny_valid,
                                        const float *__restrict__ X, unsigned ldx_b, int kx_valid, bool with_db, int out, int64_t M,
                                        int rows_per_wg, float *__restrict__ partial, const unsigned *__restrict__ rowtab,
                                        unsigned src_rows, int bx, int by, int bz, int tiles_x, int tiles_y, int splits_z) {
    constexpr int WK = 4 / WN;
    constexpr int BNT = WN * NI * 16, BKX = WK * NJ * 16, TILE_F = NI * NJ * 1024;
    constexpr int PPW = TMT / 8;
    static_assert(2 * 2 * TMT * 128 <= TN_LDS_FLOATS && 8 * 128 <= TN_LDS_FLOATS, "stage buffers");
    float *Ys = lds;
    float *Xs = lds + 2 * TMT * 128;

    const int tid = threadIdx.x;
    const int lane = tid & 63, wave = tid >> 6;
    const int wave_u = __builtin_amdgcn_readfirstlane(wave);
    const int r16 = lane & 15, q = lane >> 4;
    const int wn = wave / WK, wk = wave % WK;
    const int n0 = bx * BNT, k0 = by * BKX;
    const int64_t mbeg = (int64_t)bz * rows_per_wg;
    const int rows = (int)((M - mbeg) < rows_per_wg ? (M - mbeg) : rows_per_wg);
    const int steps = (rows + TMT - 1) / TMT;
    const int rem = rows - (steps - 1) * TMT;
    const int ny_here = (ny_valid - n0) < BNT ? (ny_valid - n0) : BNT;
    const int kx_here = (kx_valid - k0) < BKX ? (kx_valid - k0) : BKX;

    const __amdgpu_buffer_rsrc_t y_rs = make_rsrc(reinterpret_cast<const char *>(dY) + mbeg * ldy_b + (int64_t)n0 * 4,
                                                  (unsigned)(rows - 1) * ldy_b + (unsigned)ny_here * 4);
    const __amdgpu_buffer_rsrc_t x_rs =
        GATHER ? __builtin_amdgcn_make_buffer_rsrc(const_cast<float *>(X), (short)ldx_b, src_rows, 0x00020000)
               : make_rsrc(reinterpret_cast<const char *>(X) + mbeg * ldx_b + (int64_t)k0 * 4,
                           (unsigned)(rows - 1) * ldx_b + (unsigned)kx_here * 4);
    const int row_l = 2 * wave + (lane >> 5);
    const int lch = (lane & 31) ^ ((row_l & 3) << 2);
    const bool x_col = lch * 4 < kx_here;
    const unsigned y_off = (lch * 4 < ny_here) ? (unsigned)row_l * ldy_b + lch * 16 : OOR;
    const unsigned x_off = GATHER ? (unsigned)(k0 * 4 + lch * 16) : (x_col ? (unsigned)row_l * ldx_b + lch * 16 : OOR);
    const unsigned y_row8 = 8u * ldy_b, x_row8 = 8u * ldx_b, y_stage = TMT * ldy_b, x_stage = TMT * ldx_b;
    unsigned x_row[4];
    static_assert(PPW <= 4, "x_row");
    const __amdgpu_buffer_rsrc_t t_rs = make_rsrc(GATHER ? rowtab + mbeg : nullptr, GATHER ? (unsigned)rows * 4 : 0u);
    auto load_rows = [&](int stage) {
        if (GATHER) {
#pragma unroll
            for (int i = 0; i < PPW; ++i)
                x_row[i] = __builtin_amdgcn_raw_buffer_load_b32(t_rs, (unsigned)row_l * 4, (unsigned)(stage * TMT + 8 * i) * 4, 0);
        }
    };

    auto issue_stage = [&](int buf, int stage) {
        float *Yd = Ys + (buf * TMT + 2 * wave_u) * 128, *Xd = Xs + (buf * TMT + 2 * wave_u) * 128;
#pragma unroll
        for (int i = 0; i < PPW; ++i) {
            __builtin_amdgcn_raw_ptr_buffer_load_lds(y_rs, Yd + 8 * i * 128, 16, y_off, (unsigned)stage * y_stage + i * y_row8, 0, 0);
            if (GATHER) {
                if (x_col) __builtin_amdgcn_struct_ptr_buffer_load_lds(x_rs, Xd + 8 * i * 128, 16, x_row[i], x_off, 0, 0, 0);
            } else {
                __builtin_amdgcn_raw_ptr_buffer_load_lds(x_rs, Xd + 8 * i * 128, 16, x_off, (unsigned)stage * x_stage + i * x_row8, 0, 0);
            }
        }
    };
    const int zr = tid >> 5, zc = (tid & 31) * 4;
    auto clear_tail = [&](int buf) {
        const f32x4 z = f32x4{0.f, 0.f, 0.f, 0.f};
        for (int r = rem + zr; r < TMT; r += 8) {
            *reinterpret_cast<f32x4 *>(&Ys[(buf * TMT + r) * 128 + zc]) = z;
            *reinterpret_cast<f32x4 *>(&Xs[(buf * TMT + r) * 128 + zc]) = z;
        }
    };

    f32x4 acc[NI][NJ], acc2[NI][NJ];
#pragma unroll
    for (int i = 0; i < NI; ++i)
#pragma unroll
        for (int j = 0; j < NJ; ++j) acc[i][j] = acc2[i][j] = f32x4{0.f, 0.f, 0.f, 0.f};
    f32x4 bs4 = f32x4{0.f, 0.f, 0.f, 0.f};
    const bool want_db = with_db && by == 0;

    load_rows(0);
    if (GATHER) asm volatile("s_waitcnt vmcnt(0)" ::: "memory");
    issue_stage(0, 0);
    if (steps > 1) load_rows(1);
    asm volatile("s_waitcnt vmcnt(0)" ::: "memory");
    if (steps == 1 && rem < TMT) clear_tail(0);
    __syncthreads();
    int fy[NI], fx[NJ];
#pragma unroll
    for (int i = 0; i < NI; ++i) {
        const int g = wn * NI + i;
        fy[i] = q * 128 + (((g & ~3) | ((g & 3) ^ q)) << 4) + r16;
    }
#pragma unroll
    for (int j = 0; j < NJ; ++j) {
        const int g = wk * NJ + j;
        fx[j] = q * 128 + (((g & ~3) | ((g & 3) ^ q)) << 4) + r16;
    }
    const int db_off = zr * 128 + zc;
    for (int st = 0; st < steps; ++st) {
        const int cur = st & 1;
        const bool more = (st + 1) < steps;
        if (more) {
            issue_stage(cur ^ 1, st + 1);
            if ((st + 2) < steps) load_rows(st + 2);
        }
        const float *Yc = Ys + cur * TMT * 128;
        const float *Xc = Xs + cur * TMT * 128;
        if (want_db) {
#pragma unroll
            for (int i = 0; i < PPW; ++i) bs4 += *reinterpret_cast<const f32x4 *>(&Yc[db_off + 8 * i * 128]);
        }
#pragma unroll
        for (int c = 0; c < TMT / 16; ++c) {
#pragma unroll
            for (int s = 0; s < 4; ++s) {
                const int m = c * 16 + s * 4;
                float fa[NI], fb[NJ];
#pragma unroll
                for (int i = 0; i < NI; ++i) fa[i] = Yc[m * 128 + fy[i]];
#pragma unroll
                for (int j = 0; j < NJ; ++j) fb[j] = Xc[m * 128 + fx[j]];
#pragma unroll
                for (int i = 0; i < NI; ++i)
#pragma unroll
                    for (int j = 0; j < NJ; ++j) {
                        if (c & 1) acc2[i][j] = MFMA16(fa[i], fb[j], acc2[i][j]);
                        else acc[i][j] = MFMA16(fa[i], fb[j], acc[i][j]);
                    }
            }
        }
        __builtin_amdgcn_sched_barrier(0);
        asm volatile("s_waitcnt vmcnt(0)" ::: "memory");
        if (more && (st + 2) == steps && rem < TMT) clear_tail(cur ^ 1);
        __syncthreads();
    }
// ... 451 lines not shown
```

### rlgym_ppo_amd/csrc/gemm_detail.hpp

```cpp
#pragma once
#include "common.hpp"

namespace rlppo {


typedef float f32x4 __attribute__((ext_vector_type(4)));
#define MFMA16(a, b, c) __builtin_amdgcn_mfma_f32_16x16x4f32((a), (b), (c), 0, 0, 0)

namespace {
constexpr int SBM = 128;
constexpr int EPI_NONE = 99;
typedef unsigned int u32x4 __attribute__((ext_vector_type(4)));
__device__ __forceinline__ __amdgpu_buffer_rsrc_t make_rsrc(const void *base, unsigned bytes) {
    return __builtin_amdgcn_make_buffer_rsrc(const_cast<void *>(base), 0, bytes, 0x00020000);
}
__device__ __forceinline__ f32x4 ldb(__amdgpu_buffer_rsrc_t r, unsigned voff, unsigned soff) {
    return __builtin_bit_cast(f32x4, __builtin_amdgcn_raw_buffer_load_b128(r, voff, soff, 0));
}
__device__ __forceinline__ void stb(__amdgpu_buffer_rsrc_t r, unsigned voff, unsigned soff, f32x4 v) {
    __builtin_amdgcn_raw_buffer_store_b128(__builtin_bit_cast(u32x4, v), r, voff, soff, 0);
}
__device__ __forceinline__ float relu1(float x) { return __builtin_amdgcn_fmed3f(x, 0.f, __builtin_inff()); }
}

__device__ __forceinline__ void nt_store_parked(f32x4 (&acc)[2][8], char *park, float *C, unsigned ldc_b, int64_t m0, int n0, int rows_here,
                                                int wave, int lane) {
#ifndef NT_ABL
#define NT_ABL 0
#endif
    const __amdgpu_buffer_rsrc_t c_rs = make_rsrc(reinterpret_cast<char *>(C) + m0 * ldc_b + (int64_t)n0 * 4, (NT_ABL & 16) ? 0u : (unsigned)(rows_here - 1) * ldc_b + 128 * 4);
    const int r16 = lane & 15, q = lane >> 4, rr = lane >> 5, c32 = lane & 31;
#pragma unroll
    for (int i = 0; i < 2; ++i) {
        if (i) asm volatile("s_waitcnt lgkmcnt(0)" ::: "memory");
#pragma unroll
        for (int j = 0; j < 8; ++j) *reinterpret_cast<f32x4 *>(park + r16 * 512 + (((j * 4 + q) ^ r16) * 16)) = acc[i][j];
        f32x4 v[8];
#pragma unroll
        for (int t = 0; t < 8; ++t) {
            const int r = 2 * t + rr;
            v[t] = *reinterpret_cast<const f32x4 *>(park + r * 512 + ((c32 ^ r) * 16));
        }
        const unsigned c_off = (unsigned)(wave * 32 + i * 16 + rr) * ldc_b + c32 * 16;
#pragma unroll
        for (int t = 0; t < 8; ++t) stb(c_rs, c_off, 2 * t * ldc_b, v[t]);
    }
}

template <int NB, int EPI>
__device__ __forceinline__ void nt_epilogue(f32x4 (&acc)[2][NB], const float *mask_src, unsigned ldm_b, float *C, unsigned ldc_b,
                                            int64_t m0, int n0, int rows_here, int wave, int r16, int q, char *park = nullptr) {
    constexpr int BN = NB * 16;
    const int row_l = wave * 32 + r16;
    const __amdgpu_buffer_rsrc_t c_rs = make_rsrc(reinterpret_cast<char *>(C) + m0 * ldc_b + (int64_t)n0 * 4,
                                                  (unsigned)(rows_here - 1) * ldc_b + BN * 4);
    const unsigned c_off = (unsigned)row_l * ldc_b + q * 16;
    if (EPI == EPI_MASK) {
        const __amdgpu_buffer_rsrc_t m_rs = make_rsrc(reinterpret_cast<const char *>(mask_src) + m0 * ldm_b + (int64_t)n0 * 4,
                                                      (unsigned)(rows_here - 1) * ldm_b + BN * 4);
        const unsigned m_off = (unsigned)row_l * ldm_b + q * 16;
#pragma unroll
        for (int i = 0; i < 2; ++i)
#pragma unroll
            for (int j = 0; j < NB; ++j) {
                const f32x4 h = ldb(m_rs, m_off, 16 * i * ldm_b + j * 64);
#pragma unroll
                for (int e = 0; e < 4; ++e) acc[i][j][e] = h[e] > 0.f ? acc[i][j][e] : 0.f;
            }
    } else if (EPI != EPI_BIAS && EPI != EPI_NONE) {
#pragma unroll
        for (int i = 0; i < 2; ++i)
#pragma unroll
            for (int j = 0; j < NB; ++j)
#pragma unroll
                for (int e = 0; e < 4; ++e) {
                    if (EPI == EPI_BIAS_RELU) acc[i][j][e] = relu1(acc[i][j][e]);
                    if (EPI == EPI_BIAS_TANH) acc[i][j][e] = tanhf(acc[i][j][e]);
                }
    }
    __builtin_amdgcn_sched_barrier(0);
    if constexpr (NB == 8) {
        if (park) {
            nt_store_parked(acc, park, C, ldc_b, m0, n0, rows_here, wave, q * 16 + r16);
            return;
        }
    }
#pragma unroll
    for (int i = 0; i < 2; ++i)
#pragma unroll
        for (int j = 0; j < NB; ++j) stb(c_rs, c_off, 16 * i * ldc_b + j * 64, acc[i][j]);
}

template <int NB>
__device__ __forceinline__ unsigned long long relu_bits(const f32x4 (&acc)[2][NB]) {
    unsigned lo = 0, hi = 0;
#pragma unroll
    for (int i = 0; i < 2; ++i)
#pragma unroll
        for (int j = 0; j < NB; ++j)
#pragma unroll
            for (int e = 0; e < 4; ++e) {
                const int b = (i * NB + j) * 4 + e;
                const unsigned v = acc[i][j][e] > 0.f ? 1u : 0u;
                if (b < 32) lo |= v << b;
                else hi |= v << (b - 32);
            }
    return ((unsigned long long)hi << 32) | lo;
}
template <int NB>
__device__ __forceinline__ void apply_bits(f32x4 (&acc)[2][NB], unsigned long long w) {
    const unsigned lo = (unsigned)w, hi = (unsigned)(w >> 32);
#pragma unroll
    for (int i = 0; i < 2; ++i)
#pragma unroll
        for (int j = 0; j < NB; ++j)
#pragma unroll
            for (int e = 0; e < 4; ++e) {
                const int b = (i * NB + j) * 4 + e;
                const unsigned m = 0u - (((b < 32 ? lo : hi) >> (b & 31)) & 1u);
                const float x = acc[i][j][e];
                acc[i][j][e] = __uint_as_float(__float_as_uint(x) & m);
            }
}

__device__ __forceinline__ void xcd_tile(int &row_tile, int &col_tile) {
    const int nr = gridDim.x, nc = gridDim.y;
    row_tile = blockIdx.x;
    col_tile = blockIdx.y;
    if (nc > 1 && nr >= 8) {
        const int id = blockIdx.y * nr + blockIdx.x, full = nr & ~7, grouped = full * nc;
        if (id < grouped) {
            const int g = id % (8 * nc);
            row_tile = (id / (8 * nc)) * 8 + (g & 7);
            col_tile = g >> 3;
        } else {
            const int t = id - grouped, r = nr - full;
            row_tile = full + t % r;
            col_tile = t / r;
        }
    }
}

template <int BKT>
__device__ __forceinline__ int dswz(int row, int chunk) {
    if (BKT == 32) return row * 32 + ((chunk ^ (row & 7)) << 2);
    return row * 16 + ((chunk ^ ((0 - (row >> 2)) & 3)) << 2);
}

typedef __bf16 bf16x8 __attribute__((ext_vector_type(8)));
typedef unsigned int u32x2 __attribute__((ext_vector_type(2)));

int64_t tn_partial_rows(int out, int in, int64_t M);
int64_t tn_partial_rows_wide(int pout, int pin, int64_t M);
struct TnAlt {
    const float *dY, *X;
    float *partial;
    int interleave;
};
struct TnRedAlt {
    const float *partial;
    float *dW, *db;
};
int launch_tn_reduce(hipStream_t st, const float *partial, int splits, int tiles_x, int tiles_y, float *dW, float *db, int out, int in,
                     int ni = 4, int nj = 4, int wn = 2, const TnRedAlt *alt = nullptr);
}
```

### rlgym_ppo_amd/csrc/heads.hip

```cpp
#include "common.hpp"

namespace rlppo {

constexpr float PROB_MIN = 1e-11f;

__device__ __forceinline__ float wave_max(float v) {
#pragma unroll
    for (int o = 32; o > 0; o >>= 1) v = fmaxf(v, __shfl_xor(v, o));
    return v;
}
__device__ __forceinline__ float wave_sum(float v) {
#pragma unroll
    for (int o = 32; o > 0; o >>= 1) v += __shfl_xor(v, o);
    return v;
}

template <int EPL>
__device__ __forceinline__ unsigned row_valid_bits(const unsigned *__restrict__ words, int A, int lane) {
    unsigned bits = 0, in_row = 0;
#pragma unroll
    for (int e = 0; e < EPL; ++e) {
        const int c = lane + 64 * e;
        if (c < A) {
            in_row |= 1u << e;
            bits |= ((words[(lane >> 5) + 2 * e] >> (lane & 31)) & 1u) << e;
        }
    }
    return __ballot(bits != 0) ? bits : in_row;
}

template <int EPL, bool MASKED = false>
__device__ __forceinline__ void row_softmax(const float *__restrict__ z, int A, int lane, float (&p)[EPL],
                                            float (&pc)[EPL], unsigned valid = 0) {
    float mx = -INFINITY;
#pragma unroll
    for (int e = 0; e < EPL; ++e) {
        const int c = lane + 64 * e;
        const bool in = MASKED ? ((valid >> e) & 1u) != 0 : c < A;
        p[e] = in ? z[c] : -INFINITY;
        mx = fmaxf(mx, p[e]);
    }
    mx = wave_max(mx);
    float s = 0.f;
#pragma unroll
    for (int e = 0; e < EPL; ++e) {
        const int c = lane + 64 * e;
        const bool in = MASKED ? ((valid >> e) & 1u) != 0 : c < A;
        p[e] = in ? expf(p[e] - mx) : 0.f;
        s += p[e];
    }
    s = wave_sum(s);
#pragma unroll
    for (int e = 0; e < EPL; ++e) {
        p[e] = p[e] / s;
        pc[e] = fminf(fmaxf(p[e], PROB_MIN), 1.0f);
    }
}

template <int EPL, bool FROM_PROBS, bool MASKED = false>
__global__ __launch_bounds__(256) void discrete_sample_kernel(const float *__restrict__ src, int64_t ld, int64_t n,
                                                               int A, const float *__restrict__ noise,
                                                               int64_t *__restrict__ actions, float *__restrict__ logp,
                                                               float *__restrict__ probs_out,
                                                               const unsigned *__restrict__ mask = nullptr, int W = 0) {
    const int lane = threadIdx.x & 63;
    const int64_t row = (int64_t)blockIdx.x * 4 + (threadIdx.x >> 6);
    if (row >= n) return;
    float p[EPL], pc[EPL];
    const float *z = src + row * ld;
    unsigned valid = 0;
    if (MASKED) valid = row_valid_bits<EPL>(mask + row * W, A, lane);
    if (MASKED) {
        row_softmax<EPL, true>(z, A, lane, p, pc, valid);
    } else if (FROM_PROBS) {
#pragma unroll
        for (int e = 0; e < EPL; ++e) {
            const int c = lane + 64 * e;
            pc[e] = c < A ? z[c] : 0.f;
        }
    } else {
        row_softmax<EPL>(z, A, lane, p, pc);
    }
    float best = -INFINITY;
    int besti = 0x7fffffff;
    float bestp = 1.f;
#pragma unroll
    for (int e = 0; e < EPL; ++e) {
        const int c = lane + 64 * e;
        if (MASKED) {
            if ((valid >> e) & 1u) {
                const float v = pc[e] / noise[row * A + c];
                if (v > best) {
                    best = v;
                    besti = c;
                    bestp = pc[e];
                }
            }
            if (probs_out && c < A) probs_out[row * A + c] = ((valid >> e) & 1u) ? pc[e] : 0.f;
        } else if (c < A) {
            const float v = pc[e] / noise[row * A + c];
            if (v > best) {
                best = v;
                besti = c;
                bestp = pc[e];
            }
            if (probs_out) probs_out[row * A + c] = pc[e];
        }
    }
#pragma unroll
    for (int o = 32; o > 0; o >>= 1) {
        const float ov = __shfl_xor(best, o);
        const int oi = __shfl_xor(besti, o);
        const float op = __shfl_xor(bestp, o);
        if (ov > best || (ov == best && oi < besti)) {
            best = ov;
            besti = oi;
            bestp = op;
        }
    }
    if (lane == 0) {
        actions[row] = besti;
        logp[row] = logf(bestp);
    }
}

template <bool FROM_PROBS>
static int launch_discrete_sample(hipStream_t st, const float *src, int64_t ld, int64_t n, int A, const float *noise,
                                  int64_t *actions, float *logp, float *probs_out, const unsigned *mask = nullptr, int W = 0) {
    if (n <= 0) return 0;
    dim3 grid((unsigned)cdiv(n, 4)), block(256);
    if (!FROM_PROBS && mask) {
        RLPPO_CHECK_ARG(W == (A + 31) / 32, "discrete head: mask_words=%d, n_actions=%d needs %d", W, A, (A + 31) / 32);
        if (A <= 128)
            hipLaunchKernelGGL((discrete_sample_kernel<2, false, true>), grid, block, 0, st, src, ld, n, A, noise, actions, logp, probs_out, mask, W);
        else if (A <= 512)
            hipLaunchKernelGGL((discrete_sample_kernel<8, false, true>), grid, block, 0, st, src, ld, n, A, noise, actions, logp, probs_out, mask, W);
        else if (A <= 2048)
            hipLaunchKernelGGL((discrete_sample_kernel<32, false, true>), grid, block, 0, st, src, ld, n, A, noise, actions, logp, probs_out, mask, W);
        else {
            set_error("discrete head: n_actions=%d > 2048 unsupported", A);
            return RLPPO_ERR_ARG;
        }
        RLPPO_LAUNCH_CHECK();
        return 0;
    }
    if (A <= 128)
        hipLaunchKernelGGL((discrete_sample_kernel<2, FROM_PROBS>), grid, block, 0, st, src, ld, n, A, noise, actions, logp, probs_out);
    else if (A <= 512)
        hipLaunchKernelGGL((discrete_sample_kernel<8, FROM_PROBS>), grid, block, 0, st, src, ld, n, A, noise, actions, logp, probs_out);
    else if (A <= 2048)
        hipLaunchKernelGGL((discrete_sample_kernel<32, FROM_PROBS>), grid, block, 0, st, src, ld, n, A, noise, actions, logp, probs_out);
    else {
        set_error("discrete head: n_actions=%d > 2048 unsupported", A);
        return RLPPO_ERR_ARG;
    }
    RLPPO_LAUNCH_CHECK();
    return 0;
}

int launch_discrete_sample_logits(hipStream_t st, const float *logits, int64_t ld, int64_t n, int A, const float *noise,
                                  int64_t *actions, float *logp, float *probs_out, const unsigned *mask, int mask_words) {
    return launch_discrete_sample<false>(st, logits, ld, n, A, noise, actions, logp, probs_out, mask, mask_words);
}
int launch_categorical_select(hipStream_t st, const float *probs, int64_t ld, int64_t n, int A, const float *noise,
                              int64_t *actions, float *logp) {
    return launch_discrete_sample<true>(st, probs, ld, n, A, noise, actions, logp, nullptr);
}

template <int EPL, bool MASKED = false>
__global__ __launch_bounds__(256) void discrete_probs_kernel(const float *__restrict__ logits, int64_t ld, int64_t n, int A,
                                                              int clamp, float *__restrict__ probs, int64_t ld_p,
                                                              unsigned long long *__restrict__ key,
                                                              const unsigned *__restrict__ mask = nullptr, int W = 0) {
    const int lane = threadIdx.x & 63;
    const int64_t row = (int64_t)blockIdx.x * 4 + (threadIdx.x >> 6);
    if (row >= n) return;
    float p[EPL], pc[EPL];
    unsigned valid = 0;
    if (MASKED) {
        valid = row_valid_bits<EPL>(mask + row * W, A, lane);
        row_softmax<EPL, true>(logits + row * ld, A, lane, p, pc, valid);
    } else {
        row_softmax<EPL>(logits + row * ld, A, lane, p, pc);
    }
    float best = -1.f;
    int besti = 0x7fffffff;
#pragma unroll
    for (int e = 0; e < EPL; ++e) {
        const int c = lane + 64 * e;
        if (MASKED) {
            const bool ok = ((valid >> e) & 1u) != 0;
            if (probs && c < A) probs[row * ld_p + c] = ok ? (clamp ? pc[e] : p[e]) : 0.f;
            if (ok && pc[e] > best) {
                best = pc[e];
                besti = c;
            }
        } else if (c < A) {
            if (probs) probs[row * ld_p + c] = clamp ? pc[e] : p[e];
            if (pc[e] > best) {
                best = pc[e];
                besti = c;
            }
        }
    }
    if (!key) return;
#pragma unroll
    for (int o = 32; o > 0; o >>= 1) {
        const float ov = __shfl_xor(best, o);
        const int oi = __shfl_xor(besti, o);
        if (ov > best || (ov == best && oi < besti)) {
            best = ov;
            besti = oi;
        }
    }
    if (lane == 0) {
        const unsigned long long flat = (unsigned long long)(row * A + besti);
        atomicMax(key, ((unsigned long long)__float_as_uint(best) << 32) | (0xffffffffull - flat));
    }
}
__global__ void decode_flat_argmax_kernel(unsigned long long *key) {
    *(long long *)key = (long long)(0xffffffffull - (*key & 0xffffffffull));
}

int launch_discrete_probs(hipStream_t st, const float *logits, int64_t ld, int64_t n, int A, int clamp, float *probs,
                          int64_t ld_p, int64_t *flat_argmax, const unsigned *mask, int W) {
    if (n <= 0) return 0;
    RLPPO_CHECK_ARG(!mask || W == (A + 31) / 32, "discrete head: mask_words=%d, n_actions=%d needs %d", W, A, (A + 31) / 32);
    if (flat_argmax && (unsigned long long)n * (unsigned long long)A > 0xffffffffull) {
        set_error("discrete_probs: n * n_actions exceeds the 32-bit flat index of the arg-max key");
        return RLPPO_ERR_ARG;
    }
    unsigned long long *key = (unsigned long long *)flat_argmax;
    if (key) RLPPO_HIP(hipMemsetAsync(key, 0, sizeof(*key), st));
    dim3 grid((unsigned)cdiv(n, 4)), block(256);
    if (mask && A <= 128)
        hipLaunchKernelGGL((discrete_probs_kernel<2, true>), grid, block, 0, st, logits, ld, n, A, clamp, probs, ld_p, key, mask, W);
    else if (mask && A <= 512)
        hipLaunchKernelGGL((discrete_probs_kernel<8, true>), grid, block, 0, st, logits, ld, n, A, clamp, probs, ld_p, key, mask, W);
    else if (mask && A <= 2048)
        hipLaunchKernelGGL((discrete_probs_kernel<32, true>), grid, block, 0, st, logits, ld, n, A, clamp, probs, ld_p, key, mask, W);
    else if (A <= 128)
        hipLaunchKernelGGL((discrete_probs_kernel<2>), grid, block, 0, st, logits, ld, n, A, clamp, probs, ld_p, key);
    else if (A <= 512)
        hipLaunchKernelGGL((discrete_probs_kernel<8>), grid, block, 0, st, logits, ld, n, A, clamp, probs, ld_p, key);
    else if (A <= 2048)
        hipLaunchKernelGGL((discrete_probs_kernel<32>), grid, block, 0, st, logits, ld, n, A, clamp, probs, ld_p, key);
    else {
        set_error("discrete head: n_actions=%d > 2048 unsupported", A);
        return RLPPO_ERR_ARG;
    }
    RLPPO_LAUNCH_CHECK();
    if (key) {
        hipLaunchKernelGGL(decode_flat_argmax_kernel, dim3(1), dim3(1), 0, st, key);
        RLPPO_LAUNCH_CHECK();
    }
    return 0;
}

__device__ __forceinline__ float surrogate_weight(float ratio, float adv, const LossCfg &c, float &s_min) {
    const float s1 = ratio * adv;
    const float cl = fminf(fmaxf(ratio, c.clip_lo), c.clip_hi);
    const float s2 = cl * adv;
    const float inr = (ratio >= c.clip_lo && ratio <= c.clip_hi) ? 1.f : 0.f;
    s_min = fminf(s1, s2);
    return s1 < s2 ? 1.f : (s1 > s2 ? inr : 0.5f + 0.5f * inr);
}

__device__ __forceinline__ void block_stats_add(double *stats, const float (&v)[5], bool active, const LossCfg &c,
                                                double *kl_slots = nullptr) {
    __shared__ float red[5][4];
    const int lane = threadIdx.x & 63, wave = threadIdx.x >> 6;
#pragma unroll
    for (int k = 0; k < 5; ++k) {
        float x = wave_sum(active ? v[k] : 0.f);
        if (lane == 0) red[k][wave] = x;
    }
    __syncthreads();
    if (threadIdx.x < 5) {
        const int k = threadIdx.x;
        const double s = (double)red[k][0] + (double)red[k][1] + (double)red[k][2] + (double)red[k][3];
        if (k == RLPPO_STAT_KL && kl_slots) {
            kl_slots[2 + blockIdx.x] = s;
            if (blockIdx.x == 0) {
                kl_slots[0] = (double)gridDim.x;
                kl_slots[1] = (double)c.mb_ratio;
            }
        }
        if (!(c.stop_word && *c.stop_word)) atomicAdd(stats + k, s);
    }
}

__device__ __forceinline__ float surrogate_adv(float adv, const LossCfg &c) { return c.adv_norm ? (adv - c.adv_norm[0]) * c.adv_norm[1] : adv; }

__device__ __forceinline__ float value_row(float *vout_row, float target, float adv, const LossCfg &c) {
    const float v = vout_row[0];
    if (c.vclip > 0.f) {
        const float v_old = target - adv;
        const float dv = v - v_old;
        const float d = (v_old + fminf(fmaxf(dv, -c.vclip), c.vclip)) - target;
        vout_row[0] = fabsf(dv) <= c.vclip ? c.mb_ratio * (2.f * d * c.inv_mb) : 0.f;
        return d * d;
    }
    const float d = v - target;
    vout_row[0] = c.mb_ratio * (2.f * d * c.inv_mb);
    return d * d;
}

template <int EPL, bool MASKED = false>
__global__ __launch_bounds__(256) void discrete_loss_kernel(float *__restrict__ logits, int64_t ld, int A,
                                                             const float *__restrict__ actions,
                                                             const float *__restrict__ old_logp,
                                                             const float *__restrict__ advantages, int64_t mb,
                                                             LossCfg cfg, double *__restrict__ stats, MaskRows mr = MaskRows{}) {
    const int lane = threadIdx.x & 63;
    float st[5] = {0.f, 0.f, 0.f, 0.f, 0.f};
    for (int64_t row = (int64_t)blockIdx.x * 4 + (threadIdx.x >> 6); row < mb; row += (int64_t)gridDim.x * 4) {
        float *z = logits + row * ld;
        float p[EPL], pc[EPL], lp[EPL];
        unsigned valid = 0;
        if (MASKED) {
            valid = row_valid_bits<EPL>(mr.mask + ring_row(mr.idx[row], mr.ring_base, mr.ring_cap) * mr.W, A, lane);
            row_softmax<EPL, true>(z, A, lane, p, pc, valid);
        } else {
            row_softmax<EPL>(z, A, lane, p, pc);
        }
        const int a = (int)actions[row];
        float ent = 0.f, lpa = 0.f, pca = 0.f;
#pragma unroll
        for (int e = 0; e < EPL; ++e) {
            const int c = lane + 64 * e;
            const bool in = MASKED ? ((valid >> e) & 1u) != 0 : c < A;
            lp[e] = in ? logf(pc[e]) : 0.f;
            if (in) ent -= lp[e] * pc[e];
            if (c == a) {
                lpa = MASKED && !in ? logf(pc[e]) : lp[e];
                pca = pc[e];
            }
        }
        ent = wave_sum(ent);
        lpa = wave_sum(lpa);
        pca = wave_sum(pca);
        const float old = old_logp[row], adv = surrogate_adv(advantages[row], cfg);
        const float lr = lpa - old;
        const float ratio = expf(lr);
        float smin;
        const float w = surrogate_weight(ratio, adv, cfg, smin);
        const float g_logp = cfg.mb_ratio * (-(adv * w * ratio) * cfg.inv_mb);
        const float g_ent = cfg.mb_ratio * (cfg.ent_coef * cfg.inv_mb);
        float gp[EPL];
        float dot = 0.f;
#pragma unroll
        for (int e = 0; e < EPL; ++e) {
            const int c = lane + 64 * e;
            const bool in = MASKED ? ((valid >> e) & 1u) != 0 : c < A;
            float g = 0.f;
            if (in) {
                g = g_ent * (lp[e] + 1.f);
                if (c == a) g += g_logp / pca;
                if (!(p[e] >= PROB_MIN)) g = 0.f;
            }
            gp[e] = g;
            dot += g * p[e];
        }
        dot = wave_sum(dot);
#pragma unroll
        for (int e = 0; e < EPL; ++e) {
            const int c = lane + 64 * e;
            const bool in = MASKED ? ((valid >> e) & 1u) != 0 : c < A;
            if (c < ld) z[c] = in ? p[e] * (gp[e] - dot) : 0.f;
        }
        if (lane == 0) {
            st[RLPPO_STAT_ENTROPY] += ent * cfg.inv_mb;
            st[RLPPO_STAT_KL] += ((ratio - 1.f) - lr) * cfg.inv_mb;
            st[RLPPO_STAT_CLIPFRAC] += (fabsf(ratio - 1.f) > cfg.clip ? 1.f : 0.f) * cfg.inv_mb;
            st[RLPPO_STAT_PLOSS] += -smin * cfg.inv_mb;
        }
    }
    block_stats_add(stats, st, true, cfg, cfg.kl_slots);
}

template <int CTRL>
__device__ __forceinline__ float dpp_mov(float v) {
    return __builtin_bit_cast(float, __builtin_amdgcn_update_dpp(0, __builtin_bit_cast(int, v), CTRL, 0xF, 0xF, true));
}
__device__ __forceinline__ float row16_sum(float v) {
    v += dpp_mov<0xB1>(v);
    v += dpp_mov<0x4E>(v);
    v += dpp_mov<0x141>(v);
    v += dpp_mov<0x140>(v);
    return v;
}
__device__ __forceinline__ float row16_max(float v) {
    v = fmaxf(v, dpp_mov<0xB1>(v));
    v = fmaxf(v, dpp_mov<0x4E>(v));
    v = fmaxf(v, dpp_mov<0x141>(v));
    v = fmaxf(v, dpp_mov<0x140>(v));
    return v;
}

template <bool MASKED = false>
__global__ __launch_bounds__(256) void discrete_loss16_kernel(float *__restrict__ logits, int64_t ld, int A,
                                                               const float *__restrict__ actions,
                                                               const float *__restrict__ old_logp,
                                                               const float *__restrict__ advantages, int64_t mb,
                                                               LossCfg cfg, double *__restrict__ stats, MaskRows mr = MaskRows{}) {
    typedef float f32x4 __attribute__((ext_vector_type(4)));
    const int l16 = threadIdx.x & 15, grp = threadIdx.x >> 4;
    const int c0 = l16 * 8;
    const bool in_row = c0 < ld;
    float st[5] = {0.f, 0.f, 0.f, 0.f, 0.f};
    for (int64_t base = (int64_t)blockIdx.x * 16; base < mb; base += (int64_t)gridDim.x * 16) {
        const bool live = base + grp < mb;
        const int64_t row = live ? base + grp : mb - 1;
        float *z = logits + row * ld + c0;
        float p[8], pc[8], lp[8];
        if (in_row) {
            const f32x4 z0 = *reinterpret_cast<const f32x4 *>(z), z1 = *reinterpret_cast<const f32x4 *>(z + 4);
#pragma unroll
            for (int e = 0; e < 4; ++e) {
                p[e] = z0[e];
                p[4 + e] = z1[e];
            }
        }
        const float old = old_logp[row], adv = surrogate_adv(advantages[row], cfg);
        const int a = (int)actions[row];
        unsigned valid = 0;
        if (MASKED) {
            const unsigned in_bits = c0 + 8 <= A ? 0xffu : (c0 < A ? (1u << (A - c0)) - 1u : 0u);
            if (in_bits)
                valid = reinterpret_cast<const unsigned char *>(mr.mask + ring_row(mr.idx[row], mr.ring_base, mr.ring_cap) * mr.W)[l16] & in_bits;
            if (!(row16_max(valid ? 1.f : 0.f) > 0.f)) valid = in_bits;
        }
        float mx = -INFINITY;
#pragma unroll
        for (int e = 0; e < 8; ++e) {
            const bool in = MASKED ? ((valid >> e) & 1u) != 0 : (in_row && c0 + e < A);
            if (!in) p[e] = -INFINITY;
            mx = fmaxf(mx, p[e]);
        }
        mx = row16_max(mx);
        float s = 0.f;
#pragma unroll
        for (int e = 0; e < 8; ++e) {
            const bool in = MASKED ? ((valid >> e) & 1u) != 0 : (c0 + e < A);
            p[e] = in ? expf(p[e] - mx) : 0.f;
            s += p[e];
        }
        s = row16_sum(s);
        float ent = 0.f, lpa = 0.f, pca = 0.f;
#pragma unroll
        for (int e = 0; e < 8; ++e) {
            const int c = c0 + e;
            const bool in = MASKED ? ((valid >> e) & 1u) != 0 : c < A;
            p[e] = p[e] / s;
            pc[e] = fminf(fmaxf(p[e], PROB_MIN), 1.0f);
            lp[e] = in ? logf(pc[e]) : 0.f;
            if (in) ent -= lp[e] * pc[e];
            if (c == a) {
                lpa = MASKED && !in ? logf(pc[e]) : lp[e];
                pca = pc[e];
            }
        }
        ent = row16_sum(ent);
        lpa = row16_sum(lpa);
        pca = row16_sum(pca);
        const float lr = lpa - old;
        const float ratio = expf(lr);
        float smin;
        const float w = surrogate_weight(ratio, adv, cfg, smin);
        const float g_logp = cfg.mb_ratio * (-(adv * w * ratio) * cfg.inv_mb);
        const float g_ent = cfg.mb_ratio * (cfg.ent_coef * cfg.inv_mb);
        float gp[8];
        float dot = 0.f;
#pragma unroll
        for (int e = 0; e < 8; ++e) {
            const int c = c0 + e;
            const bool in = MASKED ? ((valid >> e) & 1u) != 0 : c < A;
            float g = 0.f;
            if (in) {
                g = g_ent * (lp[e] + 1.f);
                if (c == a) g += g_logp / pca;
                if (!(p[e] >= PROB_MIN)) g = 0.f;
            }
            gp[e] = g;
            dot += g * p[e];
        }
        dot = row16_sum(dot);
        if (live && in_row) {
            f32x4 o0, o1;
#pragma unroll
            for (int e = 0; e < 4; ++e) {
                const bool in0 = MASKED ? ((valid >> e) & 1u) != 0 : (c0 + e < A);
                const bool in1 = MASKED ? ((valid >> (4 + e)) & 1u) != 0 : (c0 + 4 + e < A);
                o0[e] = in0 ? p[e] * (gp[e] - dot) : 0.f;
                o1[e] = in1 ? p[4 + e] * (gp[4 + e] - dot) : 0.f;
            }
            *reinterpret_cast<f32x4 *>(z) = o0;
            *reinterpret_cast<f32x4 *>(z + 4) = o1;
        }
        if (live && l16 == 0) {
            st[RLPPO_STAT_ENTROPY] += ent * cfg.inv_mb;
            st[RLPPO_STAT_KL] += ((ratio - 1.f) - lr) * cfg.inv_mb;
            st[RLPPO_STAT_CLIPFRAC] += (fabsf(ratio - 1.f) > cfg.clip ? 1.f : 0.f) * cfg.inv_mb;
            st[RLPPO_STAT_PLOSS] += -smin * cfg.inv_mb;
        }
    }
    block_stats_add(stats, st, true, cfg, cfg.kl_slots);
}

__global__ __launch_bounds__(256) void value_loss_kernel(float *__restrict__ vout, int64_t ldv, const float *__restrict__ targets,
                                                         const float *__restrict__ advantages, int64_t mb, LossCfg cfg,
                                                         double *__restrict__ stats) {
    float st[5] = {0.f, 0.f, 0.f, 0.f, 0.f};
    for (int64_t row = (int64_t)blockIdx.x * 256 + threadIdx.x; row < mb; row += (int64_t)gridDim.x * 256)
        st[RLPPO_STAT_VLOSS] += value_row(vout + row * ldv, targets[row], cfg.vclip > 0.f ? advantages[row] : 0.f, cfg) * cfg.inv_mb;
    block_stats_add(stats, st, true, cfg);
}

int launch_value_loss(hipStream_t st, float *vout, int64_t ldv, const float *targets, const float *adv, int64_t mb, const LossCfg &cfg,
                      double *stats) {
    if (mb <= 0) return 0;
    RLPPO_CHECK_ARG(!(cfg.vclip > 0.f) || adv, "value loss: clipping needs the advantages");
    dim3 grid((unsigned)(cdiv(mb, 256) < 1024 ? cdiv(mb, 256) : 1024));
    hipLaunchKernelGGL(value_loss_kernel, grid, dim3(256), 0, st, vout, ldv, targets, adv, mb, cfg, stats);
    RLPPO_LAUNCH_CHECK();
    return 0;
}

int64_t kl_slots_doubles(int64_t mb) {
    const int64_t g = cdiv(mb > 0 ? mb : 1, 256);
    return 2 + (g > 2048 ? g : 2048);
}

int launch_discrete_loss(hipStream_t st, float *logits, int64_t ld, int A, const float *actions, const float *old_logp, const float *adv,
                         int64_t mb, const LossCfg &cfg, double *stats, const MaskRows *mr) {
    if (mb <= 0) return 0;
    dim3 grid((unsigned)(cdiv(mb, 4) < 2048 ? cdiv(mb, 4) : 2048)), block(256);
    RLPPO_CHECK_ARG(ld <= DISCRETE_LOSS_MAX_LD, "discrete head: padded width %ld too large", (long)ld);
    if (mr && mr->mask) {
        RLPPO_CHECK_ARG(mr->W == (A + 31) / 32 && mr->idx, "discrete head: mask_words=%d, n_actions=%d needs %d", mr->W, A, (A + 31) / 32);
        if (ld <= 128) {
            dim3 grid16((unsigned)(cdiv(mb, 16) < 2048 ? cdiv(mb, 16) : 2048));
            hipLaunchKernelGGL(discrete_loss16_kernel<true>, grid16, block, 0, st, logits, ld, A, actions, old_logp, adv, mb, cfg, stats, *mr);
        } else if (ld <= 512)
            hipLaunchKernelGGL((discrete_loss_kernel<8, true>), grid, block, 0, st, logits, ld, A, actions, old_logp, adv, mb, cfg, stats, *mr);
        else
            hipLaunchKernelGGL((discrete_loss_kernel<32, true>), grid, block, 0, st, logits, ld, A, actions, old_logp, adv, mb, cfg, stats, *mr);
        RLPPO_LAUNCH_CHECK();
        return 0;
    }
    if (ld <= 128) {
        dim3 grid16((unsigned)(cdiv(mb, 16) < 2048 ? cdiv(mb, 16) : 2048));
        hipLaunchKernelGGL(discrete_loss16_kernel<false>, grid16, block, 0, st, logits, ld, A, actions, old_logp, adv, mb, cfg, stats, MaskRows{});
    } else if (ld <= 512)
        hipLaunchKernelGGL((discrete_loss_kernel<8>), grid, block, 0, st, logits, ld, A, actions, old_logp, adv, mb, cfg, stats, MaskRows{});
    else
        hipLaunchKernelGGL((discrete_loss_kernel<32>), grid, block, 0, st, logits, ld, A, actions, old_logp, adv, mb, cfg, stats, MaskRows{});
    RLPPO_LAUNCH_CHECK();
    return 0;
}

constexpr int FLOAT_SUM_K = 32;

__device__ __forceinline__ float gauss_logpdf(float x, float mean, float sd) {
    const float msq = mean * mean, ssq = sd * sd, xsq = x * x;
    const float t1 = -(msq / (2.f * ssq));
    const float t2 = (mean * x) / ssq;
    const float t3 = -(xsq / (2.f * ssq));
    const float t4 = logf(1.f / sqrtf((float)(2.0 * 3.14159265358979323846) * ssq));
    return t1 + t2 + t3 + t4;
}

__device__ __forceinline__ void block_done_words(unsigned *done_words, unsigned done_value, int64_t n) {
    if (!done_words) return;
    __builtin_amdgcn_fence(__ATOMIC_RELEASE, "");
    __syncthreads();
    const int64_t w = (int64_t)blockIdx.x * 16 + threadIdx.x;
    if (threadIdx.x < 16 && w < (n + 15) / 16) __hip_atomic_store(done_words + w, done_value, __ATOMIC_RELEASE, __HIP_MEMORY_SCOPE_SYSTEM);
}

__global__ __launch_bounds__(256) void gaussian_sample_kernel(const float *__restrict__ y, int64_t ld, int64_t n, int k,
                                                               const float *__restrict__ eps, float var_m, float var_b,
                                                               float *__restrict__ actions, float *__restrict__ logp,
                                                               unsigned *done_words, unsigned done_value) {
    const int64_t row = (int64_t)blockIdx.x * blockDim.x + threadIdx.x;
    if (row < n) {
        const float *yr = y + row * ld;
        float lp = 0.f;
        double lpd = 0.0;
        for (int j = 0; j < k; ++j) {
            const float mean = yr[j];
            const float sd = yr[k + j] * var_m + var_b;
            float a = eps[row * k + j] * sd + mean;
            a = fminf(fmaxf(a, -1.f), 1.f);
            actions[row * k + j] = a;
            if (k <= FLOAT_SUM_K)
                lp += gauss_logpdf(a, mean, sd);
            else
                lpd += (double)gauss_logpdf(a, mean, sd);
        }
        logp[row] = k <= FLOAT_SUM_K ? lp : (float)lpd;
    }
    block_done_words(done_words, done_value, n);
}

int launch_gaussian_sample(hipStream_t st, const float *y, int64_t ld, int64_t n, int k, const float *eps, float var_m,
                           float var_b, float *actions, float *logp, unsigned *done_words, unsigned done_value) {
    if (n <= 0) return 0;
    hipLaunchKernelGGL(gaussian_sample_kernel, dim3((unsigned)cdiv(n, 256)), dim3(256), 0, st, y, ld, n, k, eps, var_m,
                       var_b, actions, logp, done_words, done_value);
    RLPPO_LAUNCH_CHECK();
    return 0;
}

__global__ __launch_bounds__(256) void gaussian_loss_kernel(float *__restrict__ y, int64_t ld, int k,
                                                             const float *__restrict__ actions,
                                                             const float *__restrict__ old_logp,
                                                             const float *__restrict__ advantages, int64_t mb,
                                                             LossCfg cfg, double *__restrict__ stats) {
    const int64_t row = (int64_t)blockIdx.x * blockDim.x + threadIdx.x;
    const bool active = row < mb;
    float st[5] = {0.f, 0.f, 0.f, 0.f, 0.f};
    if (active) {
        float *yr = y + row * ld;
        const float *xr = actions + row * k;
        float lp = 0.f, ent = 0.f;
        if (k <= FLOAT_SUM_K) {
#pragma unroll 4
            for (int j = 0; j < k; ++j) {
                const float mean = yr[j], sd = yr[k + j] * cfg.var_m + cfg.var_b;
                lp += gauss_logpdf(xr[j], mean, sd);
                ent += 1.4189385332046727f + logf(sd);
            }
        } else {
            double lpd = 0.0, entd = 0.0;
#pragma unroll 4
            for (int j = 0; j < k; ++j) {
                const float mean = yr[j], sd = yr[k + j] * cfg.var_m + cfg.var_b;
                lpd += (double)gauss_logpdf(xr[j], mean, sd);
                entd += (double)(1.4189385332046727f + logf(sd));
            }
            lp = (float)lpd;
            ent = (float)entd;
        }
        const float old = old_logp[row], adv = surrogate_adv(advantages[row], cfg);
        const float lr = lp - old;
        const float ratio = expf(lr);
        float smin;
        const float w = surrogate_weight(ratio, adv, cfg, smin);
        const float g_logp = cfg.mb_ratio * (-(adv * w * ratio) * cfg.inv_mb);
        const float g_ent = -cfg.mb_ratio * cfg.ent_coef * cfg.inv_mb / (float)k;
#pragma unroll 4
        for (int j = 0; j < k; ++j) {
            const float ym = yr[j], ys = yr[k + j];
            const float sd = ys * cfg.var_m + cfg.var_b;
            const float d = xr[j] - ym;
            const float s2 = sd * sd;
// ... 282 lines not shown
```

Measured before the change: 63.84 million samples/s.

## Fuse discrete policy loss into the policy head GEMM epilogue

Adds an EPI_BIAS_LOSS epilogue to the NT GEMM kernel that computes softmax, PPO surrogate gradient and loss statistics directly from the accumulator tiles. When the discrete-head conditions hold (unmasked, no KL slots, padded width 96 or 128, large minibatch), the policy head forward and the separate policy_loss kernel become one launch. This avoids writing the logits to global memory and reading them back. The shared row loss math moves into a common header. The cost is extra register and LDS pressure in the GEMM kernel, and block-level stats atomics issued from every GEMM block.

```diff
diff --git a/rlgym_ppo_amd/csrc/api.hip b/rlgym_ppo_amd/csrc/api.hip
--- a/rlgym_ppo_amd/csrc/api.hip
+++ b/rlgym_ppo_amd/csrc/api.hip
@@ -95,7 +95,8 @@
 
 static int forward(hipStream_t st, const NetLayout &net, const float *packed, const RowSource &in, int64_t n, int out_tanh,
                    float *const *acts, int bf16_operands = 0, unsigned long long *const *bits = nullptr, bool *have_bits = nullptr,
-                   bool *head_folded = nullptr, const unsigned short *x3 = nullptr, bool head_prezeroed = false) {
+                   bool *head_folded = nullptr, const unsigned short *x3 = nullptr, bool head_prezeroed = false,
+                   const NtLoss *head_loss = nullptr) {
     X3Layout xl;
     if (x3) x3_layout(net, &xl);
     if (have_bits)
@@ -113,7 +114,13 @@
         const int epi = last ? (out_tanh ? EPI_BIAS_TANH : EPI_BIAS) : EPI_BIAS_RELU;
         int rc;
         if (last && head_folded && *head_folded) break;
-        if (last && !out_tanh && gemv_head_ok(L.out, L.pin))
+        if (last && head_loss) {
+            rc = launch_gemm_nt_loss(st, x, ldx, packed + L.off_w, L.pin, packed + L.off_b, acts[l], L.pout, n, L.pout, L.pin, *head_loss);
+            if (rc == -1) {
+                set_error("forward: padded width %d has no loss epilogue", L.pout);
+                return RLPPO_ERR_ARG;
+            }
+        } else if (last && !out_tanh && gemv_head_ok(L.out, L.pin))
             rc = launch_gemv_fwd(st, x, ldx, packed + L.off_w, packed + L.off_b, acts[l], L.pout, n, L.pin, L.pout);
         else {
             rc = -1;
@@ -246,7 +253,7 @@
 using namespace rlppo;
 
 static int g_fused_act = 1;
-static std::atomic<long long> g_cnt_fused_act{0}, g_cnt_act_chain{0}, g_cnt_paired_pass{0}, g_cnt_gather_fused_pass{0}, g_cnt_pass{0}, g_cnt_group_dw{0}, g_cnt_md_nvec{0};
+static std::atomic<long long> g_cnt_fused_act{0}, g_cnt_act_chain{0}, g_cnt_paired_pass{0}, g_cnt_gather_fused_pass{0}, g_cnt_pass{0}, g_cnt_group_dw{0}, g_cnt_md_nvec{0}, g_cnt_head_loss_epi{0};
 constexpr int64_t FUSED_ACT_MAX_ROWS = 8192;
 
 struct ActCtx {
@@ -937,8 +944,13 @@
 }
 
 static int head_forward(hipStream_t st, const NetLayout &net, const float *packed, const float *x, int64_t ldx, int64_t n, int out_tanh,
-                        float *out) {
+                        float *out, const NtLoss *loss = nullptr) {
     const LayerLayout &L = net.L[net.n_layers - 1];
+    if (loss) {
+        const int rc = launch_gemm_nt_loss(st, x, ldx, packed + L.off_w, L.pin, packed + L.off_b, out, L.pout, n, L.pout, L.pin, *loss);
+        if (rc == -1) set_error("head forward: padded width %d has no loss epilogue", L.pout);
+        return rc == -1 ? RLPPO_ERR_ARG : rc;
+    }
     if (!out_tanh && gemv_head_ok(L.out, L.pin)) return launch_gemv_fwd(st, x, ldx, packed + L.off_w, packed + L.off_b, out, L.pout, n, L.pin, L.pout);
     return launch_gemm_nt(st, x, ldx, packed + L.off_w, L.pin, packed + L.off_b, nullptr, 0, out, L.pout, n, L.pout, L.pin,
                           out_tanh ? EPI_BIAS_TANH : EPI_BIAS);
@@ -1011,6 +1023,26 @@
     c.kl_slots = a.kl_slots;
     c.stop_word = a.stop_word;
     return c;
+}
+
+#ifndef HEAD_LOSS_EPI_DEFAULT
+#define HEAD_LOSS_EPI_DEFAULT 1
+#endif
+static int g_head_loss_epi = HEAD_LOSS_EPI_DEFAULT;
+constexpr int64_t HEAD_LOSS_EPI_MIN_ROWS = 50000;
+static bool head_loss_epilogue(const Pass &p, NtLoss *out) {
+    const rlppo_minibatch_args &a = *p.a;
+    const LayerLayout &L = p.pol.L[p.pol.n_layers - 1];
+    if (!(g_head_loss_epi == 2 || (g_head_loss_epi == 1 && p.mb >= HEAD_LOSS_EPI_MIN_ROWS))) return false;
+    if (a.head != RLPPO_HEAD_DISCRETE || a.action_mask || a.kl_slots || p.prec == 1) return false;
+    if (L.pout != 96 && L.pout != 128) return false;
+    out->act = p.w.g_act;
+    out->old_logp = p.w.g_old;
+    out->adv = p.w.g_adv;
+    out->stats = a.stats;
+    out->A = L.out;
+    out->cfg = p.cfg;
+    return true;
 }
 
 static int policy_loss(hipStream_t st, const Pass &p) {
@@ -1115,9 +1147,12 @@
         rc = head_backward(hs, val, p.val_w, vout, xv, mb, w.val.dx[H - 1], a.val_grad, w.val.tn, w.val.bits[H - 1], ldv, p.defer);
         if (rc) return rc;
     }
-    rc = head_forward(st, pol, p.pol_w, xp, ldx, mb, a.head == RLPPO_HEAD_GAUSSIAN, pout);
-    if (rc) return rc;
-    rc = policy_loss(st, p);
+    NtLoss hl;
+    const bool loss_epi = head_loss_epilogue(p, &hl);
+    if (loss_epi) ++g_cnt_head_loss_epi;
+    rc = head_forward(st, pol, p.pol_w, xp, ldx, mb, a.head == RLPPO_HEAD_GAUSSIAN, pout, loss_epi ? &hl : nullptr);
+    if (rc) return rc;
+    if (!loss_epi) rc = policy_loss(st, p);
     if (rc) return rc;
     if (ordered) {
         rc = order_after(hs, st, bk.ev_mid[slot]);
@@ -1174,6 +1209,8 @@
     bool phave[RLPPO_MAX_LAYERS] = {}, vhave[RLPPO_MAX_LAYERS] = {};
     bool pf32[RLPPO_MAX_LAYERS] = {}, vf32[RLPPO_MAX_LAYERS] = {};
     bool v_folded = false;
+    NtLoss hl;
+    const bool loss_epi = !b16 && head_loss_epilogue(p, &hl);
     int rc;
     if (b16) {
         rc = forward_b16(p.side, val, p.val_w, val_wb16, p.rows.x, w.states_b, p.rows.ld, mb, 0, w.val.act, w.val.actb, w.val.bits, vhave,
@@ -1184,13 +1221,15 @@
     } else {
         rc = forward(p.side, val, p.val_w, p.rows, mb, 0, w.val.act, 0, w.val.bits, vhave, &v_folded, val_x3, true);
         if (rc) return rc;
-        rc = forward(p.st, pol, p.pol_w, p.rows, mb, a.head == RLPPO_HEAD_GAUSSIAN, w.pol.act, 0, w.pol.bits, phave, nullptr, pol_x3);
+        if (loss_epi) ++g_cnt_head_loss_epi;
+        rc = forward(p.st, pol, p.pol_w, p.rows, mb, a.head == RLPPO_HEAD_GAUSSIAN, w.pol.act, 0, w.pol.bits, phave, nullptr, pol_x3, false,
+                     loss_epi ? &hl : nullptr);
     }
     if (rc) return rc;
     const int64_t ldv = v_folded ? 1 : val.L[val.n_layers - 1].pout;
     rc = launch_value_loss(p.side, w.val.act[val.n_layers - 1], ldv, w.g_tgt, w.g_adv, mb, p.cfg, a.stats);
     if (rc) return rc;
-    rc = policy_loss(p.st, p);
+    if (!loss_epi) rc = policy_loss(p.st, p);
     if (rc) return rc;
     if (b16) {
         rc = backward_b16(p.side, val, p.val_w, val_wb16, p.rows.x, w.states_b, p.rows.ld, mb, w.val.act, w.val.actb, w.val.dx, w.val.dxb,
@@ -1506,6 +1545,7 @@
         case 38: set_tn_group_budget(value); return 0;
         case 40: set_nt_skinny(value); return 0;
         case 41: g_window_mode = value; return 0;
+        case 42: g_head_loss_epi = value; return 0;
         default: break;
     }
     set_error("dbg_set: unknown key %d", key);
@@ -1522,6 +1562,7 @@
         case 4: return g_cnt_gather_fused_pass;
         case 5: return g_cnt_group_dw;
         case 6: return g_cnt_md_nvec;
+        case 7: return g_cnt_head_loss_epi;
         default: return -1;
     }
 }
diff --git a/rlgym_ppo_amd/csrc/common.hpp b/rlgym_ppo_amd/csrc/common.hpp
--- a/rlgym_ppo_amd/csrc/common.hpp
+++ b/rlgym_ppo_amd/csrc/common.hpp
@@ -81,7 +81,8 @@
 
 int make_layout(const int32_t *dims, int32_t n_layers, NetLayout *out);
 
-enum Epilogue { EPI_BIAS = 0, EPI_BIAS_RELU = 1, EPI_BIAS_TANH = 2, EPI_MASK = 3 };
+enum Epilogue { EPI_BIAS = 0, EPI_BIAS_RELU = 1, EPI_BIAS_TANH = 2, EPI_MASK = 3,
+                EPI_BIAS_LOSS = 4 };
 
 int launch_gemm_nt(hipStream_t st, const float *A, int64_t lda, const float *B, int64_t ldb, const float *bias,
                    const float *mask_src, int64_t ld_mask, float *C, int64_t ldc, int64_t M, int N, int K, int epi,
@@ -173,6 +174,14 @@
     double *kl_slots = nullptr;
     const unsigned *stop_word = nullptr;
 };
+struct NtLoss {
+    const float *act = nullptr, *old_logp = nullptr, *adv = nullptr;
+    double *stats = nullptr;
+    int A = 0;
+    LossCfg cfg;
+};
+int launch_gemm_nt_loss(hipStream_t st, const float *A, int64_t lda, const float *B, int64_t ldb, const float *bias, float *C,
+                        int64_t ldc, int64_t M, int N, int K, const NtLoss &loss);
 __host__ __device__ __forceinline__ int64_t ring_row(int64_t i, int64_t base, int64_t cap) {
     const int64_t r = i + base;
     return r >= cap ? r - cap : r;
diff --git a/rlgym_ppo_amd/csrc/gemm.hip b/rlgym_ppo_amd/csrc/gemm.hip
--- a/rlgym_ppo_amd/csrc/gemm.hip
+++ b/rlgym_ppo_amd/csrc/gemm.hip
@@ -12,7 +12,8 @@
                                                                               unsigned long long *__restrict__ bits = nullptr,
                                                                               const unsigned *__restrict__ rowtab = nullptr,
                                                                               unsigned src_rows = 0, NtAlt alt = NtAlt{},
-                                                                              NtDot dot = NtDot{}, NtDot dot_alt = NtDot{}) {
+                                                                              NtDot dot = NtDot{}, NtDot dot_alt = NtDot{},
+                                                                              NtLoss loss = NtLoss{}) {
     constexpr int BN = NB * 16;
     constexpr int CPR = BKT / 4;
     constexpr int RPW = 64 / CPR;
@@ -51,6 +52,13 @@
     unsigned long long *const bit_word = BITS ? bits + ((size_t)row_tile * nct + col_tile) * 256 + tid : nullptr;
     unsigned long long mask_word = 0;
     if (BITS && EPI == EPI_MASK) mask_word = *bit_word;
+    float r_act = 0.f, r_old = 0.f, r_adv = 0.f;
+    if (EPI == EPI_BIAS_LOSS) {
+        const unsigned r_off = (unsigned)(wave * 32 + (lane & 31)) * 4;
+        r_act = __builtin_bit_cast(float, __builtin_amdgcn_raw_buffer_load_b32(make_rsrc(loss.act + m0, (unsigned)rows_here * 4), r_off, 0, 0));
+        r_old = __builtin_bit_cast(float, __builtin_amdgcn_raw_buffer_load_b32(make_rsrc(loss.old_logp + m0, (unsigned)rows_here * 4), r_off, 0, 0));
+        r_adv = __builtin_bit_cast(float, __builtin_amdgcn_raw_buffer_load_b32(make_rsrc(loss.adv + m0, (unsigned)rows_here * 4), r_off, 0, 0));
+    }
 
     const __amdgpu_buffer_rsrc_t a_rs = GATHER ? __builtin_amdgcn_make_buffer_rsrc(const_cast<float *>(A), (short)lda_b, src_rows, 0x00020000)
                                                : make_rsrc(reinterpret_cast<const char *>(A) + m0 * lda_b,
@@ -131,6 +139,12 @@
         __syncthreads();
     }
     char *const park = reinterpret_cast<char *>(lds) + wave_u * 8192;
+    if constexpr (EPI == EPI_BIAS_LOSS) {
+        static_assert(BKT == 16 && !BITS && !GATHER, "loss epilogue: the head's forward form");
+        nt_loss_epilogue<NB>(acc, reinterpret_cast<char *>(lds) + wave_u * (int)(sizeof(lds) / 4), C, ldc_b, m0, rows_here, wave, lane,
+                             loss, r_act, r_old, r_adv);
+        return;
+    }
     if (BITS && EPI == EPI_MASK) {
         apply_bits<NB>(acc, mask_word);
         nt_epilogue<NB, EPI_NONE>(acc, nullptr, 0, C, ldc_b, m0, n0, rows_here, wave, r16, q, park);
@@ -487,6 +501,29 @@
         case 4: return launch_nt_1<4>(st, grid, epi, A, la, B, lb, bias, mask_src, lm, C, lc, M, K);
         default: return launch_nt_1<2>(st, grid, epi, A, la, B, lb, bias, mask_src, lm, C, lc, M, K);
     }
+}
+
+int launch_gemm_nt_loss(hipStream_t st, const float *A, int64_t lda, const float *B, int64_t ldb, const float *bias, float *C,
+                        int64_t ldc, int64_t M, int N, int K, const NtLoss &loss) {
+    if (N != 96 && N != 128) return -1;
+    if (M <= 0) return 0;
+    RLPPO_CHECK_ARG(K > 0 && K % 16 == 0, "gemm_nt: K=%d must be a positive multiple of 16", K);
+    RLPPO_CHECK_ARG(lda % 4 == 0 && ldb % 4 == 0 && ldc % 4 == 0 && lda >= K && ldb >= K && ldc >= N,
+                    "gemm_nt: leading dimensions lda=%ld ldb=%ld ldc=%ld incompatible with K=%d N=%d", (long)lda, (long)ldb, (long)ldc, K, N);
+    RLPPO_CHECK_ARG(bias && loss.act && loss.old_logp && loss.adv && loss.stats && loss.A > 0 && loss.A <= N && !loss.cfg.kl_slots,
+                    "gemm_nt (loss epilogue): incomplete loss descriptor");
+    const int64_t lim = (int64_t)1 << 31;
+    RLPPO_CHECK_ARG(129 * lda * 4 < lim && 129 * ldb * 4 < lim && 129 * ldc * 4 < lim, "gemm_nt: a leading dimension is too wide for 32-bit tile offsets");
+    dim3 grid((unsigned)cdiv(M, SBM), 1u);
+    const unsigned la = (unsigned)(lda * 4), lb = (unsigned)(ldb * 4), lc = (unsigned)(ldc * 4);
+    if (N == 96)
+        hipLaunchKernelGGL((gemm_nt_dma_kernel<6, EPI_BIAS_LOSS, 16>), grid, dim3(256), 0, st, A, la, B, lb, bias, nullptr, 0u, C, lc, M, K,
+                           nullptr, nullptr, 0u, NtAlt{}, NtDot{}, NtDot{}, loss);
+    else
+        hipLaunchKernelGGL((gemm_nt_dma_kernel<8, EPI_BIAS_LOSS, 16>), grid, dim3(256), 0, st, A, la, B, lb, bias, nullptr, 0u, C, lc, M, K,
+                           nullptr, nullptr, 0u, NtAlt{}, NtDot{}, NtDot{}, loss);
+    RLPPO_LAUNCH_CHECK();
+    return 0;
 }
 
 namespace {
diff --git a/rlgym_ppo_amd/csrc/gemm_detail.hpp b/rlgym_ppo_amd/csrc/gemm_detail.hpp
--- a/rlgym_ppo_amd/csrc/gemm_detail.hpp
+++ b/rlgym_ppo_amd/csrc/gemm_detail.hpp
@@ -1,5 +1,6 @@
 #pragma once
 #include "common.hpp"
+#include "loss_row16.hpp"
 
 namespace rlppo {
 
@@ -89,6 +90,65 @@
     for (int i = 0; i < 2; ++i)
 #pragma unroll
         for (int j = 0; j < NB; ++j) stb(c_rs, c_off, 16 * i * ldc_b + j * 64, acc[i][j]);
+}
+
+template <int NB>
+__device__ __forceinline__ void nt_loss_epilogue(f32x4 (&acc)[2][NB], char *park, float *C, unsigned ldc_b, int64_t m0, int rows_here,
+                                                 int wave, int lane, const NtLoss &ls, float r_act, float r_old, float r_adv) {
+    constexpr int BN = NB * 16, ROWB = BN * 4;
+    static_assert(BN <= 128 && 16 * ROWB <= (2 * SBM * 16 + 2 * BN * 16) * 4 / 4, "a wave parks 16 whole rows in its quarter of the BK = 16 stage buffers");
+    const int r16 = lane & 15, q = lane >> 4;
+    const int c0 = r16 * 8;
+    const bool in_row = c0 < BN;
+    const __amdgpu_buffer_rsrc_t c_rs = make_rsrc(reinterpret_cast<char *>(C) + m0 * ldc_b, (unsigned)(rows_here - 1) * ldc_b + BN * 4);
+    float st[5] = {0.f, 0.f, 0.f, 0.f, 0.f};
+#pragma unroll
+    for (int i = 0; i < 2; ++i) {
+        if (i) asm volatile("s_waitcnt lgkmcnt(0)" ::: "memory");
+#pragma unroll
+        for (int j = 0; j < NB; ++j) *reinterpret_cast<f32x4 *>(park + r16 * ROWB + (((j * 4 + q) ^ (r16 & 7)) * 16)) = acc[i][j];
+#pragma unroll
+        for (int t = 0; t < 4; ++t) {
+            const int R = 4 * t + q;
+            const int rl = wave * 32 + 16 * i + R;
+            const bool live = rl < rows_here;
+            float p[8], g[8], term[4];
+            if (in_row) {
+                const f32x4 z0 = *reinterpret_cast<const f32x4 *>(park + R * ROWB + (((2 * r16) ^ (R & 7)) * 16));
+                const f32x4 z1 = *reinterpret_cast<const f32x4 *>(park + R * ROWB + (((2 * r16 + 1) ^ (R & 7)) * 16));
+#pragma unroll
+                for (int e = 0; e < 4; ++e) {
+                    p[e] = z0[e];
+                    p[4 + e] = z1[e];
+                }
+            } else {
+#pragma unroll
+                for (int e = 0; e < 8; ++e) p[e] = 0.f;
+            }
+            const int src = 16 * i + R;
+            const float old = __shfl(r_old, src), adv = __shfl(r_adv, src);
+            const int a = (int)__shfl(r_act, src);
+            discrete_row16<false>(p, c0, in_row, ls.A, old, adv, a, 0u, ls.cfg, g, term);
+            if (live && in_row) {
+                f32x4 o0, o1;
+#pragma unroll
+                for (int e = 0; e < 4; ++e) {
+                    o0[e] = g[e];
+                    o1[e] = g[4 + e];
+                }
+                const unsigned c_off = (unsigned)rl * ldc_b + (unsigned)c0 * 4;
+                stb(c_rs, c_off, 0, o0);
+                stb(c_rs, c_off + 16, 0, o1);
+            }
+            if (live && r16 == 0) {
+                st[RLPPO_STAT_ENTROPY] += term[0];
+                st[RLPPO_STAT_KL] += term[1];
+                st[RLPPO_STAT_CLIPFRAC] += term[2];
+                st[RLPPO_STAT_PLOSS] += term[3];
+            }
+        }
+    }
+    block_stats_add(ls.stats, st, true, ls.cfg);
 }
 
 template <int NB>
diff --git a/rlgym_ppo_amd/csrc/heads.hip b/rlgym_ppo_amd/csrc/heads.hip
--- a/rlgym_ppo_amd/csrc/heads.hip
+++ b/rlgym_ppo_amd/csrc/heads.hip
@@ -1,17 +1,11 @@
 #include "common.hpp"
+#include "loss_row16.hpp"
 
 namespace rlppo {
 
-constexpr float PROB_MIN = 1e-11f;
-
 __device__ __forceinline__ float wave_max(float v) {
 #pragma unroll
     for (int o = 32; o > 0; o >>= 1) v = fmaxf(v, __shfl_xor(v, o));
-    return v;
-}
-__device__ __forceinline__ float wave_sum(float v) {
-#pragma unroll
-    for (int o = 32; o > 0; o >>= 1) v += __shfl_xor(v, o);
     return v;
 }
 
@@ -257,40 +251,6 @@
     return 0;
 }
 
-__device__ __forceinline__ float surrogate_weight(float ratio, float adv, const LossCfg &c, float &s_min) {
-    const float s1 = ratio * adv;
-    const float cl = fminf(fmaxf(ratio, c.clip_lo), c.clip_hi);
-    const float s2 = cl * adv;
-    const float inr = (ratio >= c.clip_lo && ratio <= c.clip_hi) ? 1.f : 0.f;
-    s_min = fminf(s1, s2);
-    return s1 < s2 ? 1.f : (s1 > s2 ? inr : 0.5f + 0.5f * inr);
-}
-
-__device__ __forceinline__ void block_stats_add(double *stats, const float (&v)[5], bool active, const LossCfg &c,
-                                                double *kl_slots = nullptr) {
-    __shared__ float red[5][4];
-    const int lane = threadIdx.x & 63, wave = threadIdx.x >> 6;
-#pragma unroll
-    for (int k = 0; k < 5; ++k) {
-        float x = wave_sum(active ? v[k] : 0.f);
-        if (lane == 0) red[k][wave] = x;
-    }
-    __syncthreads();
-    if (threadIdx.x < 5) {
-        const int k = threadIdx.x;
-        const double s = (double)red[k][0] + (double)red[k][1] + (double)red[k][2] + (double)red[k][3];
-        if (k == RLPPO_STAT_KL && kl_slots) {
-            kl_slots[2 + blockIdx.x] = s;
-            if (blockIdx.x == 0) {
-                kl_slots[0] = (double)gridDim.x;
-                kl_slots[1] = (double)c.mb_ratio;
-            }
-        }
-        if (!(c.stop_word && *c.stop_word)) atomicAdd(stats + k, s);
-    }
-}
-
-__device__ __forceinline__ float surrogate_adv(float adv, const LossCfg &c) { return c.adv_norm ? (adv - c.adv_norm[0]) * c.adv_norm[1] : adv; }
 
 __device__ __forceinline__ float value_row(float *vout_row, float target, float adv, const LossCfg &c) {
     const float v = vout_row[0];
@@ -379,25 +339,6 @@
     block_stats_add(stats, st, true, cfg, cfg.kl_slots);
 }
 
-template <int CTRL>
-__device__ __forceinline__ float dpp_mov(float v) {
-    return __builtin_bit_cast(float, __builtin_amdgcn_update_dpp(0, __builtin_bit_cast(int, v), CTRL, 0xF, 0xF, true));
-}
-__device__ __forceinline__ float row16_sum(float v) {
-    v += dpp_mov<0xB1>(v);
-    v += dpp_mov<0x4E>(v);
-    v += dpp_mov<0x141>(v);
-    v += dpp_mov<0x140>(v);
-    return v;
-}
-__device__ __forceinline__ float row16_max(float v) {
-    v = fmaxf(v, dpp_mov<0xB1>(v));
-    v = fmaxf(v, dpp_mov<0x4E>(v));
-    v = fmaxf(v, dpp_mov<0x141>(v));
-    v = fmaxf(v, dpp_mov<0x140>(v));
-    return v;
-}
-
 template <bool MASKED = false>
 __global__ __launch_bounds__(256) void discrete_loss16_kernel(float *__restrict__ logits, int64_t ld, int A,
                                                                const float *__restrict__ actions,
@@ -413,7 +354,7 @@
         const bool live = base + grp < mb;
         const int64_t row = live ? base + grp : mb - 1;
         float *z = logits + row * ld + c0;
-        float p[8], pc[8], lp[8];
+        float p[8], g[8], term[4];
         if (in_row) {
             const f32x4 z0 = *reinterpret_cast<const f32x4 *>(z), z1 = *reinterpret_cast<const f32x4 *>(z + 4);
 #pragma unroll
@@ -422,87 +363,27 @@
                 p[4 + e] = z1[e];
             }
         }
-        const float old = old_logp[row], adv = surrogate_adv(advantages[row], cfg);
+        const float old = old_logp[row], adv = advantages[row];
         const int a = (int)actions[row];
-        unsigned valid = 0;
-        if (MASKED) {
-            const unsigned in_bits = c0 + 8 <= A ? 0xffu : (c0 < A ? (1u << (A - c0)) - 1u : 0u);
-            if (in_bits)
-                valid = reinterpret_cast<const unsigned char *>(mr.mask + ring_row(mr.idx[row], mr.ring_base, mr.ring_cap) * mr.W)[l16] & in_bits;
-            if (!(row16_max(valid ? 1.f : 0.f) > 0.f)) valid = in_bits;
-        }
-        float mx = -INFINITY;
-#pragma unroll
-        for (int e = 0; e < 8; ++e) {
-            const bool in = MASKED ? ((valid >> e) & 1u) != 0 : (in_row && c0 + e < A);
-            if (!in) p[e] = -INFINITY;
-            mx = fmaxf(mx, p[e]);
-        }
-        mx = row16_max(mx);
-        float s = 0.f;
-#pragma unroll
-        for (int e = 0; e < 8; ++e) {
-            const bool in = MASKED ? ((valid >> e) & 1u) != 0 : (c0 + e < A);
-            p[e] = in ? expf(p[e] - mx) : 0.f;
-            s += p[e];
-        }
-        s = row16_sum(s);
-        float ent = 0.f, lpa = 0.f, pca = 0.f;
-#pragma unroll
-        for (int e = 0; e < 8; ++e) {
-            const int c = c0 + e;
-            const bool in = MASKED ? ((valid >> e) & 1u) != 0 : c < A;
-            p[e] = p[e] / s;
-            pc[e] = fminf(fmaxf(p[e], PROB_MIN), 1.0f);
-            lp[e] = in ? logf(pc[e]) : 0.f;
-            if (in) ent -= lp[e] * pc[e];
-            if (c == a) {
-                lpa = MASKED && !in ? logf(pc[e]) : lp[e];
-                pca = pc[e];
-            }
-        }
-        ent = row16_sum(ent);
-        lpa = row16_sum(lpa);
-        pca = row16_sum(pca);
-        const float lr = lpa - old;
-        const float ratio = expf(lr);
-        float smin;
-        const float w = surrogate_weight(ratio, adv, cfg, smin);
-        const float g_logp = cfg.mb_ratio * (-(adv * w * ratio) * cfg.inv_mb);
-        const float g_ent = cfg.mb_ratio * (cfg.ent_coef * cfg.inv_mb);
-        float gp[8];
-        float dot = 0.f;
-#pragma unroll
-        for (int e = 0; e < 8; ++e) {
-            const int c = c0 + e;
-            const bool in = MASKED ? ((valid >> e) & 1u) != 0 : c < A;
-            float g = 0.f;
-            if (in) {
-                g = g_ent * (lp[e] + 1.f);
-                if (c == a) g += g_logp / pca;
-                if (!(p[e] >= PROB_MIN)) g = 0.f;
-            }
-            gp[e] = g;
-            dot += g * p[e];
-        }
-        dot = row16_sum(dot);
+        unsigned mask_byte = 0;
+        if (MASKED && row16_in_bits(c0, A))
+            mask_byte = reinterpret_cast<const unsigned char *>(mr.mask + ring_row(mr.idx[row], mr.ring_base, mr.ring_cap) * mr.W)[l16];
+        discrete_row16<MASKED>(p, c0, in_row, A, old, adv, a, mask_byte, cfg, g, term);
         if (live && in_row) {
             f32x4 o0, o1;
 #pragma unroll
             for (int e = 0; e < 4; ++e) {
-                const bool in0 = MASKED ? ((valid >> e) & 1u) != 0 : (c0 + e < A);
-                const bool in1 = MASKED ? ((valid >> (4 + e)) & 1u) != 0 : (c0 + 4 + e < A);
-                o0[e] = in0 ? p[e] * (gp[e] - dot) : 0.f;
-                o1[e] = in1 ? p[4 + e] * (gp[4 + e] - dot) : 0.f;
+                o0[e] = g[e];
+                o1[e] = g[4 + e];
             }
             *reinterpret_cast<f32x4 *>(z) = o0;
             *reinterpret_cast<f32x4 *>(z + 4) = o1;
         }
         if (live && l16 == 0) {
-            st[RLPPO_STAT_ENTROPY] += ent * cfg.inv_mb;
-            st[RLPPO_STAT_KL] += ((ratio - 1.f) - lr) * cfg.inv_mb;
-            st[RLPPO_STAT_CLIPFRAC] += (fabsf(ratio - 1.f) > cfg.clip ? 1.f : 0.f) * cfg.inv_mb;
-            st[RLPPO_STAT_PLOSS] += -smin * cfg.inv_mb;
+            st[RLPPO_STAT_ENTROPY] += term[0];
+            st[RLPPO_STAT_KL] += term[1];
+            st[RLPPO_STAT_CLIPFRAC] += term[2];
+            st[RLPPO_STAT_PLOSS] += term[3];
         }
     }
     block_stats_add(stats, st, true, cfg, cfg.kl_slots);
diff --git a/rlgym_ppo_amd/csrc/loss_row16.hpp b/rlgym_ppo_amd/csrc/loss_row16.hpp
--- /dev/null
+++ b/rlgym_ppo_amd/csrc/loss_row16.hpp
@@ -0,0 +1,147 @@
+#pragma once
+#include "common.hpp"
+
+namespace rlppo {
+
+constexpr float PROB_MIN = 1e-11f;
+
+__device__ __forceinline__ float wave_sum(float v) {
+#pragma unroll
+    for (int o = 32; o > 0; o >>= 1) v += __shfl_xor(v, o);
+    return v;
+}
+
+__device__ __forceinline__ float surrogate_weight(float ratio, float adv, const LossCfg &c, float &s_min) {
+    const float s1 = ratio * adv;
+    const float cl = fminf(fmaxf(ratio, c.clip_lo), c.clip_hi);
+    const float s2 = cl * adv;
+    const float inr = (ratio >= c.clip_lo && ratio <= c.clip_hi) ? 1.f : 0.f;
+    s_min = fminf(s1, s2);
+    return s1 < s2 ? 1.f : (s1 > s2 ? inr : 0.5f + 0.5f * inr);
+}
+
+__device__ __forceinline__ void block_stats_add(double *stats, const float (&v)[5], bool active, const LossCfg &c,
+                                                double *kl_slots = nullptr) {
+    __shared__ float red[5][4];
+    const int lane = threadIdx.x & 63, wave = threadIdx.x >> 6;
+#pragma unroll
+    for (int k = 0; k < 5; ++k) {
+        float x = wave_sum(active ? v[k] : 0.f);
+        if (lane == 0) red[k][wave] = x;
+    }
+    __syncthreads();
+    if (threadIdx.x < 5) {
+        const int k = threadIdx.x;
+        const double s = (double)red[k][0] + (double)red[k][1] + (double)red[k][2] + (double)red[k][3];
+        if (k == RLPPO_STAT_KL && kl_slots) {
+            kl_slots[2 + blockIdx.x] = s;
+            if (blockIdx.x == 0) {
+                kl_slots[0] = (double)gridDim.x;
+                kl_slots[1] = (double)c.mb_ratio;
+            }
+        }
+        if (!(c.stop_word && *c.stop_word)) atomicAdd(stats + k, s);
+    }
+}
+
+__device__ __forceinline__ float surrogate_adv(float adv, const LossCfg &c) { return c.adv_norm ? (adv - c.adv_norm[0]) * c.adv_norm[1] : adv; }
+
+template <int CTRL>
+__device__ __forceinline__ float dpp_mov(float v) {
+    return __builtin_bit_cast(float, __builtin_amdgcn_update_dpp(0, __builtin_bit_cast(int, v), CTRL, 0xF, 0xF, true));
+}
+__device__ __forceinline__ float row16_sum(float v) {
+    v += dpp_mov<0xB1>(v);
+    v += dpp_mov<0x4E>(v);
+    v += dpp_mov<0x141>(v);
+    v += dpp_mov<0x140>(v);
+    return v;
+}
+__device__ __forceinline__ float row16_max(float v) {
+    v = fmaxf(v, dpp_mov<0xB1>(v));
+    v = fmaxf(v, dpp_mov<0x4E>(v));
+    v = fmaxf(v, dpp_mov<0x141>(v));
+    v = fmaxf(v, dpp_mov<0x140>(v));
+    return v;
+}
+
+__device__ __forceinline__ unsigned row16_in_bits(int c0, int A) { return c0 + 8 <= A ? 0xffu : (c0 < A ? (1u << (A - c0)) - 1u : 0u); }
+
+template <bool MASKED>
+__device__ __forceinline__ void discrete_row16(float (&p)[8], int c0, bool in_row, int A, float old, float adv_stored, int a,
+                                               unsigned mask_byte, const LossCfg &cfg, float (&g_out)[8], float (&term)[4]) {
+    float pc[8], lp[8];
+    const float adv = surrogate_adv(adv_stored, cfg);
+    unsigned valid = 0;
+    if (MASKED) {
+        const unsigned in_bits = row16_in_bits(c0, A);
+        valid = mask_byte & in_bits;
+        if (!(row16_max(valid ? 1.f : 0.f) > 0.f)) valid = in_bits;
+    }
+    float mx = -INFINITY;
+#pragma unroll
+    for (int e = 0; e < 8; ++e) {
+        const bool in = MASKED ? ((valid >> e) & 1u) != 0 : (in_row && c0 + e < A);
+        if (!in) p[e] = -INFINITY;
+        mx = fmaxf(mx, p[e]);
+    }
+    mx = row16_max(mx);
+    float s = 0.f;
+#pragma unroll
+    for (int e = 0; e < 8; ++e) {
+        const bool in = MASKED ? ((valid >> e) & 1u) != 0 : (c0 + e < A);
+        p[e] = in ? expf(p[e] - mx) : 0.f;
+        s += p[e];
+    }
+    s = row16_sum(s);
+    float ent = 0.f, lpa = 0.f, pca = 0.f;
+#pragma unroll
+    for (int e = 0; e < 8; ++e) {
+        const int c = c0 + e;
+        const bool in = MASKED ? ((valid >> e) & 1u) != 0 : c < A;
+        p[e] = p[e] / s;
+        pc[e] = fminf(fmaxf(p[e], PROB_MIN), 1.0f);
+        lp[e] = in ? logf(pc[e]) : 0.f;
+        if (in) ent -= lp[e] * pc[e];
+        if (c == a) {
+            lpa = MASKED && !in ? logf(pc[e]) : lp[e];
+            pca = pc[e];
+        }
+    }
+    ent = row16_sum(ent);
+    lpa = row16_sum(lpa);
+    pca = row16_sum(pca);
+    const float lr = lpa - old;
+    const float ratio = expf(lr);
+    float smin;
+    const float w = surrogate_weight(ratio, adv, cfg, smin);
+    const float g_logp = cfg.mb_ratio * (-(adv * w * ratio) * cfg.inv_mb);
+    const float g_ent = cfg.mb_ratio * (cfg.ent_coef * cfg.inv_mb);
+    float gp[8];
+    float dot = 0.f;
+#pragma unroll
+    for (int e = 0; e < 8; ++e) {
+        const int c = c0 + e;
+        const bool in = MASKED ? ((valid >> e) & 1u) != 0 : c < A;
+        float g = 0.f;
+        if (in) {
+            g = g_ent * (lp[e] + 1.f);
+            if (c == a) g += g_logp / pca;
+            if (!(p[e] >= PROB_MIN)) g = 0.f;
+        }
+        gp[e] = g;
+        dot += g * p[e];
+    }
+    dot = row16_sum(dot);
+#pragma unroll
+    for (int e = 0; e < 8; ++e) {
+        const bool in = MASKED ? ((valid >> e) & 1u) != 0 : (c0 + e < A);
+        g_out[e] = in ? p[e] * (gp[e] - dot) : 0.f;
+    }
+    term[0] = ent * cfg.inv_mb;
+    term[1] = ((ratio - 1.f) - lr) * cfg.inv_mb;
+    term[2] = (fabsf(ratio - 1.f) > cfg.clip ? 1.f : 0.f) * cfg.inv_mb;
+    term[3] = -smin * cfg.inv_mb;
+}
+
+}
```

Result: no change. 64.18 million samples/s (median of 6 runs) (+0.5%).
